# burlachenkok/flpytorch

Hardware: AMD Instinct MI355X
Metric: gradient-codec encode+reduce GB/s (device-resident), [N,D] fp32; % HBM peak (higher is better)
Workload: dtype f32; 1 GPU; C3 topk:1% N=1024/GPU D=10000000; codec=topk:1%, clients_per_gpu=1024, clients_total=1024, D=10000000, K=100000, rows_alloc=contiguous, parallelism=client-shard dp1

## Files before the change

flpytorch_amd/csrc/select.hip:

```cpp
#include <stdlib.h>

#include <atomic>
#include <map>
#include <mutex>
#include <vector>

#include "chunks.hpp"
#include "randk_tree.hpp"

namespace flc {

constexpr uint32_t ALL = 0xFFFFFFFFu;
constexpr uint32_t F_OVERFLOW = 1u, F_SHORT = 2u, F_TIES = 4u, F_EXACT = 8u;
constexpr uint32_t F_RESIDENT = 16u;
constexpr uint32_t F_REPAIR = 32u;
constexpr int SMAX = 16384;
constexpr int HBINS = 2048;
constexpr uint32_t TIECAP = HBINS;
constexpr int CS_SH = 64;
constexpr int64_t CS_FEW = 16;
constexpr int CS_ST = 8;
constexpr int CS_LCAP = 2048;
constexpr int RS_U = 16;
#ifndef FLC_RS_NG
#define FLC_RS_NG 4
#endif
constexpr int RS_NG = FLC_RS_NG;
constexpr int RS_NG_MAX = 16;
static_assert(RS_NG >= 1 && RS_NG <= RS_NG_MAX, "FLC_RS_NG: 1..16 groups");
constexpr int RS_GLOB = 0, RS_GEN = 32, RS_GAVE = 64, RS_CCNT = 96, RS_CDONE = 112, RS_GRP = 128;
constexpr int RS_XGRP = RS_GRP + 32 * RS_NG_MAX;
constexpr int RS_ABV = RS_XGRP + 32 * RS_NG_MAX;
constexpr int RS_CAP = 2048;
constexpr int RS_SS = 8192;
#ifndef FLC_RS_SR
#define FLC_RS_SR 1
#endif
constexpr int RS_SR = FLC_RS_SR;
#ifndef FLC_RS_STPOL
#define FLC_RS_STPOL 2
#endif
#ifndef FLC_RS_GACQ
#define FLC_RS_GACQ 1
#endif
#ifndef FLC_RS_POLLAB
#define FLC_RS_POLLAB 1
#endif
#ifndef FLC_RS_DONE
#define FLC_RS_DONE 1
#endif
#ifndef FLC_RS_RANKFIRST
#define FLC_RS_RANKFIRST 0
#endif
#ifndef FLC_RS_PROBE_NOCOUNT
#define FLC_RS_PROBE_NOCOUNT 0
#endif
#ifndef FLC_RS_G0REL
#define FLC_RS_G0REL 1
#endif
#ifndef FLC_RS_FENCE
#define FLC_RS_FENCE 0
#endif
#ifndef FLC_RS_SPEC
#define FLC_RS_SPEC 1
#endif
constexpr int RS_HREP = RS_ABV + 32 * RS_NG_MAX;
constexpr int RS_HSPEC = RS_HREP + 3 * RS_NG * HBINS;
constexpr int RS_CLIST = RS_HSPEC + 3 * RS_NG * HBINS;
constexpr int RS_TCNT = RS_CLIST + 2 * RS_CAP;
constexpr int RS_GMAX = 1024;
constexpr int RS_CS = 4;
constexpr int RS_CNUM = RS_TCNT + 2 * RS_GMAX;
constexpr int RS_CREG = RS_CNUM + RS_GMAX;
#ifdef FLC_RS_PRINT
constexpr int RS_PROBE = RS_CREG + 2 * RS_CS * RS_GMAX;
constexpr int RS_CTL = RS_PROBE + 4096;
#else
constexpr int RS_CTL = RS_CREG + 2 * RS_CS * RS_GMAX;
#endif
#ifndef FLC_RS_SPECST
#define FLC_RS_SPECST 0
#endif
#ifndef FLC_CS_LIST
#define FLC_CS_LIST 1
#endif
#ifndef FLC_CS_TWO_MAXD
#define FLC_CS_TWO_MAXD (int64_t(64) << 20)
#endif

struct SelWs {
    uint2* tab;
    uint32_t* ent_idx;
    float* ent_val;
    uint32_t* rowcnt;
    uint32_t* flags;
    uint32_t* thr;
    uint32_t* prefix;
    uint32_t* krem;
    uint32_t* tieprefix;
    uint32_t* tiecut;
    uint32_t* hist;
    uint32_t* worklist;
    uint32_t* nwork;
    uint32_t* cursor;
    uint32_t* cstate;
    uint64_t* clist;
    uint32_t* carrive;
    uint32_t* shcnt;
    uint32_t* zm;
    float* part;
    int64_t cap;
    uint32_t tie_hi;
};

__device__ __host__ inline uint32_t tie_pref(uint32_t ix, uint32_t hi) { return hi ? ix : ~ix; }
__device__ __host__ inline uint32_t tie_all(uint32_t hi) { return hi ? 0u : 0xFFFFFFFFu; }


__device__ inline void lds_bar() {
    asm volatile("s_waitcnt lgkmcnt(0)" ::: "memory");
    __builtin_amdgcn_s_barrier();
    asm volatile("" ::: "memory");
}
template <bool RAW>
__device__ inline void blk_bar() {
    if (RAW) lds_bar();
    else __syncthreads();
}
template <bool RAW = false>
__device__ inline void hist_find_at(const uint32_t* h, uint32_t k, uint32_t& bin, uint32_t& above,
                                    uint32_t* scratch , int t, bool own) {
    uint32_t local[8];
    uint32_t s = 0;
#pragma unroll
    for (int q = 0; q < 8; ++q) { local[q] = own ? h[HBINS - 1 - (t * 8 + q)] : 0u; s += local[q]; }
    if (t == 0) { scratch[256] = 0; scratch[257] = 0; }
    const int lane = t & 63, w = t >> 6;
    uint32_t inc = s;
#pragma unroll
    for (int off = 1; off < 64; off <<= 1) {
        const uint32_t v = __shfl_up(inc, off, 64);
        inc += lane >= off ? v : 0u;
    }
    if (own && lane == 63) scratch[w] = inc;
    blk_bar<RAW>();
    uint32_t before = 0;
    if (own)
        for (int q = 0; q < w; ++q) before += scratch[q];
    uint32_t incl = own ? before + inc : 0u, excl = incl - s;
    if (own && excl < k && incl >= k) {
        uint32_t run = excl;
#pragma unroll
        for (int q = 0; q < 8; ++q) {
            if (run + local[q] >= k) {
                scratch[256] = (uint32_t)(HBINS - 1 - (t * 8 + q));
                scratch[257] = run;
                break;
            }
            run += local[q];
        }
    }
    blk_bar<RAW>();
    bin = scratch[256];
    above = scratch[257];
    blk_bar<RAW>();
}
template <int NB>
__device__ inline void hist_find_n(const uint32_t* h, uint32_t k, uint32_t& bin, uint32_t& above, bool& found,
                                   uint32_t* scratch ) {
    constexpr int PER = NB / 256;
    static_assert(NB % 256 == 0, "256 threads scan NB / 256 bins each");
    const int t = (int)threadIdx.x;
    const bool own = t < 256;
    uint32_t local[PER];
    uint32_t s = 0;
#pragma unroll
    for (int q = 0; q < PER; ++q) { local[q] = own ? h[NB - 1 - (t * PER + q)] : 0u; s += local[q]; }
    if (t == 0) { scratch[256] = 0; scratch[257] = 0; scratch[258] = 0; }
    const int lane = t & 63, w = t >> 6;
    uint32_t inc = s;
#pragma unroll
    for (int off = 1; off < 64; off <<= 1) {
        const uint32_t v = __shfl_up(inc, off, 64);
        inc += lane >= off ? v : 0u;
    }
    if (own && lane == 63) scratch[w] = inc;
    __syncthreads();
    uint32_t before = 0;
    if (own)
        for (int q = 0; q < w; ++q) before += scratch[q];
    const uint32_t incl = own ? before + inc : 0u, excl = incl - s;
    if (own && excl < k && incl >= k) {
        uint32_t run = excl;
#pragma unroll
        for (int q = 0; q < PER; ++q) {
            if (run + local[q] >= k) {
                scratch[256] = (uint32_t)(NB - 1 - (t * PER + q));
                scratch[257] = run;
                scratch[258] = 1;
                break;
            }
            run += local[q];
        }
    }
    __syncthreads();
    bin = scratch[256];
    above = scratch[257];
    found = scratch[258] != 0u;
    __syncthreads();
}
template <bool RAW = false>
__device__ inline void hist_find(const uint32_t* h, uint32_t k, uint32_t& bin, uint32_t& above,
                                 uint32_t* scratch ) {
    hist_find_at<RAW>(h, k, bin, above, scratch, (int)threadIdx.x, threadIdx.x < 256);
}
__device__ inline void hist_find2(const uint32_t* ha, uint32_t ka, uint32_t& bina, uint32_t& abovea, uint32_t* sa,
                                  const uint32_t* hb, uint32_t kb, uint32_t& binb, uint32_t& aboveb, uint32_t* sb) {
    const bool second = threadIdx.x >= 256;
    uint32_t bin, above;
    hist_find_at(second ? hb : ha, second ? kb : ka, bin, above, second ? sb : sa, (int)(threadIdx.x & 255u),
                 threadIdx.x < 512);
    bina = sa[256]; abovea = sa[257];
    binb = sb[256]; aboveb = sb[257];
    __syncthreads();
}

__device__ inline uint32_t pass_shift(int p) { return p == 0 ? 20u : (p == 1 ? 9u : 0u); }
__device__ inline uint32_t pass_bits(int p) { return p == 2 ? 9u : 11u; }
__device__ inline bool key_in_prefix(uint32_t key, int p, uint32_t prefix) {
    if (p == 0) return true;
    uint32_t sh = pass_shift(p) + pass_bits(p);
    return (key >> sh) == prefix;
}
__device__ inline uint32_t key_bin(uint32_t key, int p) {
    return (key >> pass_shift(p)) & ((1u << pass_bits(p)) - 1u);
}

template <int NT, bool DUAL>
__global__ __launch_bounds__(NT) void k_topk_sample(RowSrc rows, int64_t n, int64_t d, int64_t K, SelWs ws, int few,
                                                    int64_t r_off) {
    __shared__ uint32_t keys[SMAX];
    __shared__ uint32_t h[HBINS], h2[DUAL ? HBINS : 1];
    __shared__ uint32_t scratch[260], scratch2[DUAL ? 260 : 1];
    const int64_t row = r_off + blockIdx.x;
    if (row >= n) return;
    const float* r = rows.row(row);
    int S;
    if (d <= SMAX) {
        S = (int)d;
        for (int i = threadIdx.x; i < S; i += NT) keys[i] = mag_key(r[i]);
    } else {
        const int P = SMAX / 256;
        S = SMAX;
        constexpr int GR = NT / 256, PU = 32 / GR;
        const int e = threadIdx.x & 255, g0 = threadIdx.x >> 8;
        for (int p0 = 0; p0 < P; p0 += 32) {
            float x[PU];
#pragma unroll
            for (int u = 0; u < PU; ++u) x[u] = r[((int64_t)(p0 + u * GR + g0) * (d - 256)) / (P - 1) + e];
#pragma unroll
            for (int u = 0; u < PU; ++u) keys[(p0 + u * GR + g0) * 256 + e] = mag_key(x[u]);
        }
    }
    const int NP = S == d ? 3 : 2;
    uint32_t rank;
    if (S == d) {
        rank = (uint32_t)K;
    } else {
        double ks = (double)K * (double)S / (double)d;
        double rr = ks + 4.0 * sqrt(ks) + 8.0;
        rank = (uint32_t)min((double)S, ceil(rr));
    }
    static_assert(!DUAL || NT >= 512, "hist_find2 takes 512 threads");
    auto rank_key = [&](uint32_t r) {
        uint32_t prefix = 0, krem = r;
        for (int p = 0; p < NP; ++p) {
            for (int i = threadIdx.x; i < HBINS; i += NT) h[i] = 0;
            __syncthreads();
            for (int i = threadIdx.x; i < S; i += NT) {
                uint32_t k = keys[i];
                if (key_in_prefix(k, p, prefix)) atomicAdd(&h[key_bin(k, p)], 1u);
            }
            __syncthreads();
            uint32_t bin, above;
            hist_find(h, krem, bin, above, scratch);
            prefix = (prefix << pass_bits(p)) | bin;
            krem -= above;
            __syncthreads();
        }
        return NP == 3 ? prefix : prefix << 9;
    };
    auto rank_keys = [&](uint32_t ra, uint32_t rb, uint32_t& ka, uint32_t& kb) {
        if constexpr (!DUAL) {
            ka = rank_key(ra);
            kb = rb == ra ? ka : rank_key(rb);
            return;
        }
        uint32_t pa = 0, pb = 0, ma = ra, mb = rb;
        for (int p = 0; p < NP; ++p) {
            const bool same = pa == pb;
            for (int i = threadIdx.x; i < HBINS; i += NT) { h[i] = 0; h2[i] = 0; }
            __syncthreads();
            for (int i = threadIdx.x; i < S; i += NT) {
                const uint32_t k = keys[i];
                if (key_in_prefix(k, p, pa)) atomicAdd(&h[key_bin(k, p)], 1u);
                if (!same && key_in_prefix(k, p, pb)) atomicAdd(&h2[key_bin(k, p)], 1u);
            }
            __syncthreads();
            uint32_t ba, aa, bb, ab;
            hist_find2(h, ma, ba, aa, scratch, same ? h : h2, mb, bb, ab, scratch2);
            pa = (pa << pass_bits(p)) | ba;
            ma -= aa;
            pb = (pb << pass_bits(p)) | bb;
            mb -= ab;
        }
        ka = NP == 3 ? pa : pa << 9;
        kb = NP == 3 ? pb : pb << 9;
    };
    uint32_t tkey, kest;
    rank_keys(rank, S == d ? rank : (uint32_t)max(1.0, min((double)S, (double)K * (double)S / (double)d)), tkey, kest);
    if (threadIdx.x == 0) {
        ws.thr[row] = (rank >= (uint32_t)S && S != d) ? 0u : tkey;
        ws.prefix[row] = kest;
        ws.flags[row] = 0;
        ws.rowcnt[(row) * RCS] = 0;
        if (few) { ws.cstate[row * CS_ST + 3] = 0; ws.cstate[row * CS_ST + 5] = 0; ws.carrive[row * RCS] = 0; }
    }
    if (few && threadIdx.x < CS_SH) ws.shcnt[(row * CS_SH + threadIdx.x) * RCS] = 0;
    if (few)
        for (int i = threadIdx.x; i < HBINS; i += NT) ws.hist[row * HBINS + i] = 0;
}

#ifndef FLC_CS_NT
#define FLC_CS_NT 1
#endif
__device__ inline float4 cs_ld(const float4* p) {
#if FLC_CS_NT
    typedef float v4f __attribute__((ext_vector_type(4)));
    const v4f v = __builtin_nontemporal_load(reinterpret_cast<const v4f*>(p));
    return make_float4(v.x, v.y, v.z, v.w);
#else
    return *p;
#endif
}
template <int NT>
__device__ void cand_select_row(int64_t row, int64_t K, SelWs ws, uint32_t* h, uint32_t* scratch) {
    {
        if (ws.flags[row]) return;
        const uint32_t cnt = ws.rowcnt[(row) * RCS];
        if (cnt < (uint32_t)K) {
            if (threadIdx.x == 0) ws.flags[row] |= F_SHORT;
            return;
        }
        const uint32_t T = ws.thr[row];
        const uint32_t span = ws.prefix[row] - T;
        int s = 0;
        while (s < 21 && (((uint64_t)span * 4u) >> s) >= (uint64_t)HBINS) ++s;
        const float* vals = ws.ent_val + row * ws.cap;
        const float4* v4 = reinterpret_cast<const float4*>(vals);
        const uint32_t n4 = cnt >> 2;
        uint32_t prefix = 0, krem = (uint32_t)K, last = 0;
        bool first = true, fail = false;
        int sh = s;
        while (true) {
            const int s1 = first ? sh : max(0, sh - 11);
            const uint32_t mask = first ? 0xFFFFFFFFu : ((1u << (sh - s1)) - 1u);
            for (int i = threadIdx.x; i < HBINS; i += NT) h[i] = 0;
            __syncthreads();
            auto add = [&](float x) {
                const uint32_t dk = mag_key(x) - T;
                if (first) atomicAdd(&h[min(dk >> s1, (uint32_t)(HBINS - 1))], 1u);
                else if ((dk >> sh) == prefix) atomicAdd(&h[(dk >> s1) & mask], 1u);
            };
            uint32_t i = threadIdx.x;
            for (; i + 7 * NT < n4; i += 8 * NT) {
                float4 q[8];
#pragma unroll
                for (int u = 0; u < 8; ++u) q[u] = cs_ld(v4 + i + u * NT);
#pragma unroll
                for (int u = 0; u < 8; ++u) { add(q[u].x); add(q[u].y); add(q[u].z); add(q[u].w); }
            }
            for (; i < n4; i += NT) {
                const float4 q = v4[i];
                add(q.x); add(q.y); add(q.z); add(q.w);
            }
            for (uint32_t i = n4 * 4 + threadIdx.x; i < cnt; i += NT) add(vals[i]);
            __syncthreads();
            uint32_t bin, above;
            hist_find(h, krem, bin, above, scratch);
            last = h[bin];
            if (first && bin == HBINS - 1) { fail = true; break; }
            prefix = first ? bin : ((prefix << (sh - s1)) | bin);
            krem -= above;
            sh = s1;
            first = false;
            __syncthreads();
            if (sh == 0) break;
        }
        __syncthreads();
        const uint32_t thr = T + prefix;
        bool ties = !fail && last > krem;
        if (ties && last > TIECAP) { fail = true; ties = false; }
        if (ties) {
            uint32_t* tix = h;
            if (threadIdx.x == 0) scratch[0] = 0;
            __syncthreads();
            const uint32_t* idxs = ws.ent_idx + row * ws.cap;
            for (uint32_t i = threadIdx.x; i < n4; i += NT) {
                const float4 q = v4[i];
                const float qv[4] = {q.x, q.y, q.z, q.w};
#pragma unroll
                for (int u = 0; u < 4; ++u)
                    if (mag_key(qv[u]) == thr) tix[atomicAdd(&scratch[0], 1u)] = idxs[i * 4 + u];
            }
            for (uint32_t i = n4 * 4 + threadIdx.x; i < cnt; i += NT) {
                if (mag_key(vals[i]) == thr) tix[atomicAdd(&scratch[0], 1u)] = idxs[i];
            }
            __syncthreads();
            const uint32_t m = scratch[0];
            for (uint32_t a = threadIdx.x; a < m; a += NT) {
                const uint32_t ia = tix[a];
                uint32_t rank = 0;
                for (uint32_t b = 0; b < m; ++b) rank += tie_pref(tix[b], ws.tie_hi) > tie_pref(ia, ws.tie_hi) ? 1u : 0u;
                if (rank == krem - 1) ws.tiecut[row] = ia;
            }
        }
        if (threadIdx.x == 0) {
            if (fail) {
                ws.flags[row] |= F_SHORT;
            } else {
                ws.thr[row] = thr;
                ws.krem[row] = krem;
                if (ties) ws.flags[row] |= F_TIES;
            }
        }
        __syncthreads();
    }
}

template <int NT>
__global__ __launch_bounds__(NT) void k_cand_select(int64_t r0, int64_t rn, int64_t K, SelWs ws) {
    __shared__ uint32_t h[HBINS];
    __shared__ uint32_t scratch[260];
    for (int64_t row = r0 + blockIdx.x; row < r0 + rn; row += gridDim.x) {
        cand_select_row<NT>(row, K, ws, h, scratch);
        __syncthreads();
    }
}

constexpr int CS_NT = 256;
__global__ __launch_bounds__(CS_NT) void k_cs_pass(int64_t K, SelWs ws, int final_pass) {
    __shared__ uint32_t h[HBINS];
    __shared__ uint32_t scratch[260];
    __shared__ uint32_t last_wg;
    __shared__ uint64_t lst[FLC_CS_LIST ? CS_LCAP : 1];
    const int64_t row = blockIdx.y;
    const uint32_t B = gridDim.x, b = blockIdx.x;
    uint32_t* cs = ws.cstate + row * CS_ST;
    const uint32_t stage = cs[3];
    if (stage >= 2u) return;
    const uint32_t* shc = ws.shcnt + row * CS_SH * RCS;
    uint32_t cnt = 0;
    for (int k = 0; k < CS_SH; ++k) cnt += shc[k * RCS];
    const uint32_t mycnt = shc[b * RCS];
    const bool first = stage == 0u;
    if (first && (ws.flags[row] != 0u || cnt < (uint32_t)K)) {
        if (b == 0 && threadIdx.x == 0) {
            if (ws.flags[row] == 0u) ws.flags[row] = F_SHORT;
            cs[3] = 2u;
        }
        return;
    }
    const uint32_t T = ws.thr[row];
    uint32_t sh, prefix, krem;
    if (first) {
        const uint32_t span = ws.prefix[row] - T;
        uint32_t s0 = 0;
        while (s0 < 21 && (((uint64_t)span * 4u) >> s0) >= (uint64_t)HBINS) ++s0;
        sh = s0; prefix = 0; krem = (uint32_t)K;
    } else {
        sh = cs[0]; prefix = cs[1]; krem = cs[2];
    }
    const uint32_t s1 = first ? sh : (sh > 11u ? sh - 11u : 0u);
    const uint32_t mask = first ? 0xFFFFFFFFu : ((1u << (sh - s1)) - 1u);
    const int64_t segcap = (ws.cap / CS_SH) & ~int64_t(3);
    if (FLC_CS_LIST && !first && cs[4] <= (uint32_t)CS_LCAP) {
        if (threadIdx.x == 0) scratch[0] = 0;
        __syncthreads();
        const float* sv = ws.ent_val + row * ws.cap + b * segcap;
        const uint32_t* si = ws.ent_idx + row * ws.cap + b * segcap;
        for (uint32_t e = threadIdx.x; e < mycnt; e += CS_NT) {
            const uint32_t key = mag_key(sv[e]);
            if (((key - T) >> sh) == prefix) {
                const uint32_t slot = atomicAdd(&scratch[0], 1u);
                if (slot < (uint32_t)CS_LCAP) lst[slot] = ((uint64_t)key << 32) | (uint64_t)tie_pref(si[e], ws.tie_hi);
            }
        }
        __syncthreads();
        const uint32_t nl = min(scratch[0], (uint32_t)CS_LCAP);
        if (threadIdx.x == 0) scratch[1] = nl ? atomicAdd(&cs[5], nl) : 0u;
        __syncthreads();
        uint64_t* gl = ws.clist + row * CS_LCAP;
        const uint32_t gb = scratch[1];
        for (uint32_t i = threadIdx.x; i < nl; i += CS_NT)
            if (gb + i < (uint32_t)CS_LCAP) gl[gb + i] = lst[i];
        asm volatile("s_waitcnt vmcnt(0)" ::: "memory");
        __syncthreads();
        if (threadIdx.x == 0) {
            __builtin_amdgcn_fence(__ATOMIC_RELEASE, "agent");
            last_wg = atomicAdd(&ws.carrive[row * RCS], 1u) == B - 1u ? 1u : 0u;
        }
        __syncthreads();
        if (!last_wg) return;
        __builtin_amdgcn_fence(__ATOMIC_ACQUIRE, "agent");
        const uint32_t m = __hip_atomic_load(&cs[5], __ATOMIC_RELAXED, __HIP_MEMORY_SCOPE_AGENT);
        const bool ok = m == cs[4] && m >= krem && krem >= 1u;
        const uint32_t mm = min(m, (uint32_t)CS_LCAP);
        for (uint32_t i = threadIdx.x; i < mm; i += CS_NT)
            lst[i] = __hip_atomic_load(&gl[i], __ATOMIC_RELAXED, __HIP_MEMORY_SCOPE_AGENT);
        if (threadIdx.x == 0) { scratch[0] = 0; scratch[1] = 0; scratch[2] = 0; scratch[3] = 0; }
        __syncthreads();
        if (ok)
            for (uint32_t i = threadIdx.x; i < mm; i += CS_NT) {
                const uint64_t me = lst[i];
                uint32_t rank = 0;
                for (uint32_t j = 0; j < mm; ++j) rank += lst[j] > me ? 1u : 0u;
                if (rank == krem - 1u) { scratch[0] = (uint32_t)(me >> 32); scratch[1] = tie_pref((uint32_t)me, ws.tie_hi); }
            }
        __syncthreads();
        const uint32_t kth = scratch[0];
        if (ok)
            for (uint32_t i = threadIdx.x; i < mm; i += CS_NT) {
                const uint32_t key = (uint32_t)(lst[i] >> 32);
                if (key > kth) atomicAdd(&scratch[2], 1u);
                else if (key == kth) atomicAdd(&scratch[3], 1u);
            }
        __syncthreads();
        if (threadIdx.x == 0) {
            atomicExch(&ws.carrive[row * RCS], 0u);
            if (!ok) {
                ws.flags[row] |= F_SHORT;
            } else {
                const uint32_t gt = scratch[2], eq = scratch[3];
                ws.thr[row] = kth;
                ws.krem[row] = krem - gt;
                if (gt + eq > krem) { ws.tiecut[row] = scratch[1]; ws.flags[row] |= F_TIES; }
            }
            cs[3] = 2u;
        }
        return;
    }
    for (int i = threadIdx.x; i < HBINS; i += CS_NT) h[i] = 0;
    __syncthreads();
    auto add = [&](float x) {
        const uint32_t dk = mag_key(x) - T;
        if (first) atomicAdd(&h[min(dk >> s1, (uint32_t)(HBINS - 1))], 1u);
        else if ((dk >> sh) == prefix) atomicAdd(&h[(dk >> s1) & mask], 1u);
    };
    const float* vals = ws.ent_val + row * ws.cap + b * segcap;
    const float4* v4 = reinterpret_cast<const float4*>(vals);
    const uint32_t n4 = mycnt >> 2, q1 = n4;
    uint32_t i = threadIdx.x;
    for (; i + 3 * CS_NT < q1; i += 4 * CS_NT) {
        float4 q[4];
#pragma unroll
        for (int u = 0; u < 4; ++u) q[u] = cs_ld(v4 + i + u * CS_NT);
#pragma unroll
        for (int u = 0; u < 4; ++u) { add(q[u].x); add(q[u].y); add(q[u].z); add(q[u].w); }
    }
    for (; i < q1; i += CS_NT) {
        const float4 q = cs_ld(v4 + i);
        add(q.x); add(q.y); add(q.z); add(q.w);
    }
    for (uint32_t t = n4 * 4 + threadIdx.x; t < mycnt; t += CS_NT) add(vals[t]);
    __syncthreads();
    uint32_t* gh = ws.hist + row * HBINS;
    for (int t = threadIdx.x; t < HBINS; t += CS_NT)
        if (h[t]) atomicAdd(gh + t, h[t]);
    asm volatile("s_waitcnt vmcnt(0)" ::: "memory");
    __syncthreads();
    if (threadIdx.x == 0) {
        __builtin_amdgcn_fence(__ATOMIC_RELEASE, "agent");
        asm volatile("s_waitcnt vmcnt(0)" ::: "memory");
        last_wg = atomicAdd(&ws.carrive[row * RCS], 1u) == B - 1u ? 1u : 0u;
    }
    __syncthreads();
    if (!last_wg) return;
    for (int t = threadIdx.x; t < HBINS; t += CS_NT) h[t] = atomicExch(gh + t, 0u);
    __syncthreads();
    uint32_t bin, above;
    hist_find(h, krem, bin, above, scratch);
    const uint32_t last = h[bin];
    const uint32_t np = first ? bin : ((prefix << (sh - s1)) | bin);
    const uint32_t nk = krem - above;
    const bool clamp = first && bin == HBINS - 1;
    bool ties = !clamp && s1 == 0u && last > nk, tie_fail = ties && last > TIECAP;
    if (ties && !tie_fail) {
        static_assert(CS_NT == 4 * CS_SH, "tie gather: 4 threads per shard");
        __syncthreads();
        uint32_t* tix = h;
        if (threadIdx.x == 0) scratch[0] = 0;
        __syncthreads();
        const uint32_t thr = T + np;
        const int k = threadIdx.x >> 2;
        const uint32_t sub = threadIdx.x & 3u, c = shc[k * RCS], c4 = c >> 2;
        const float* sv = ws.ent_val + row * ws.cap + k * segcap;
        const uint32_t* si = ws.ent_idx + row * ws.cap + k * segcap;
        const float4* s4 = reinterpret_cast<const float4*>(sv);
        auto test = [&](float x, uint32_t pos) {
            if (mag_key(x) == thr) {
                const uint32_t slot = atomicAdd(&scratch[0], 1u);
                if (slot < TIECAP) tix[slot] = si[pos];
            }
        };
        uint32_t j = sub;
        for (; j + 28u < c4; j += 32u) {
            float4 q[8];
#pragma unroll
            for (int u = 0; u < 8; ++u) q[u] = cs_ld(s4 + j + 4u * u);
#pragma unroll
            for (int u = 0; u < 8; ++u) {
                const uint32_t p4 = (j + 4u * u) * 4u;
                test(q[u].x, p4); test(q[u].y, p4 + 1u); test(q[u].z, p4 + 2u); test(q[u].w, p4 + 3u);
            }
        }
        for (; j < c4; j += 4u) {
            const float4 q = cs_ld(s4 + j);
            test(q.x, j * 4u); test(q.y, j * 4u + 1u); test(q.z, j * 4u + 2u); test(q.w, j * 4u + 3u);
        }
        for (uint32_t t = c4 * 4u + sub; t < c; t += 4u) test(sv[t], t);
        __syncthreads();
        const uint32_t m = scratch[0];
        if (m != last) tie_fail = true;
        else
            for (uint32_t a = threadIdx.x; a < m; a += CS_NT) {
                const uint32_t ia = tix[a];
                uint32_t rank = 0;
                for (uint32_t bb = 0; bb < m; ++bb) rank += tie_pref(tix[bb], ws.tie_hi) > tie_pref(ia, ws.tie_hi) ? 1u : 0u;
                if (rank == nk - 1u) ws.tiecut[row] = ia;
            }
    }
    if (threadIdx.x == 0) {
        atomicExch(&ws.carrive[row * RCS], 0u);
        if (clamp) {
            ws.flags[row] |= F_SHORT;
            cs[3] = 2u;
        } else if (s1 == 0u) {
            if (tie_fail) ws.flags[row] |= F_SHORT;
            else {
                ws.thr[row] = T + np;
                ws.krem[row] = nk;
                if (ties) ws.flags[row] |= F_TIES;
            }
            cs[3] = 2u;
        } else if (final_pass) {
            ws.flags[row] |= F_SHORT;
            cs[3] = 2u;
        } else {
            cs[0] = s1; cs[1] = np; cs[2] = nk; cs[3] = 1u; cs[4] = last;
        }
    }
}

template <bool EXACT, bool VEC>
__global__ __launch_bounds__(256) void k_topk_filter(RowSrc rows, int64_t n, int64_t d, SelWs ws) {
    const int64_t C = nchunks(d);
    const int64_t bpr = (C + 3) / 4;
    const int lane = threadIdx.x & 63, wv = threadIdx.x >> 6;
    const int64_t nrows = EXACT ? (int64_t)(*ws.nwork) : n;
    const int64_t items = nrows * bpr;
    for (int64_t it = blockIdx.x; it < items; it += gridDim.x) {
        const int64_t li = it / bpr;
        const int64_t row = EXACT ? (int64_t)ws.worklist[li] : li;
        const int64_t c = (it % bpr) * 4 + wv;
        if (!EXACT && ws.flags[row]) continue;
        if (c >= C) continue;
        const float* r = rows.row(row);
        const int64_t j0 = c * CHUNK;
        const uint32_t T = ws.thr[row];
        float v[16][4];
#pragma unroll
        for (int t = 0; t < 16; ++t) {
            const int64_t j = j0 + (int64_t)(t * 64 + lane) * 4;
            if (VEC && j + 3 < d) {
                float4 f = *reinterpret_cast<const float4*>(r + j);
                v[t][0] = f.x; v[t][1] = f.y; v[t][2] = f.z; v[t][3] = f.w;
            } else {
#pragma unroll
                for (int q = 0; q < 4; ++q) v[t][q] = (j + q < d) ? r[j + q] : 0.f;
            }
        }
        uint32_t tie_base = 0, tie_need = ALL, tie_from = 0;
        if (EXACT) {
            tie_base = ws.tieprefix[c * n + row];
            tie_need = ws.krem[row];
            if (ws.tie_hi) { const uint32_t tot = ws.tiecut[row]; tie_from = tot - tie_need; tie_need = tot; }
        }
        uint32_t cnt = 0;
        uint32_t tie_run = tie_base;
#pragma unroll
        for (int t = 0; t < 16; ++t) {
            const int64_t jb = j0 + (int64_t)(t * 64 + lane) * 4;
            bool gt[4], eq[4];
#pragma unroll
            for (int q = 0; q < 4; ++q) {
                const uint32_t k = mag_key(v[t][q]);
                const bool inb = (jb + q) < d;
                gt[q] = inb && (EXACT ? k > T : k >= T);
                eq[q] = inb && EXACT && k == T;
            }
            if (EXACT) {
                uint64_t m[4];
#pragma unroll
                for (int q = 0; q < 4; ++q) m[q] = __ballot(eq[q]);
                const uint64_t lt = (lane == 0) ? 0ull : (~0ull >> (64 - lane));
                uint32_t before = __popcll(m[0] & lt) + __popcll(m[1] & lt) + __popcll(m[2] & lt) + __popcll(m[3] & lt);
                uint32_t inlane = 0;
#pragma unroll
                for (int q = 0; q < 4; ++q) {
                    if (eq[q]) { const uint32_t tr = tie_run + before + inlane; gt[q] = tr >= tie_from && tr < tie_need; }
                    inlane += eq[q] ? 1u : 0u;
                }
                tie_run += __popcll(m[0]) + __popcll(m[1]) + __popcll(m[2]) + __popcll(m[3]);
            }
#pragma unroll
            for (int q = 0; q < 4; ++q) cnt += gt[q] ? 1u : 0u;
        }
        cnt = wave_sum(cnt);
        uint32_t base = 0;
        if (lane == 0) base = atomicAdd(&ws.rowcnt[(row) * RCS], cnt);
        base = __shfl(base, 0, WAVE);
        const bool fits = (int64_t)base + cnt <= ws.cap;
        if (lane == 0) {
            ws.tab[c * n + row] = make_uint2(base, fits ? cnt : 0u);
            if (!fits) atomicOr(&ws.flags[row], F_OVERFLOW);
        }
        if (!fits || cnt == 0) continue;
        uint32_t run = base;
        tie_run = tie_base;
        uint32_t* oi = ws.ent_idx + row * ws.cap;
        float* ov = ws.ent_val + row * ws.cap;
#pragma unroll
        for (int t = 0; t < 16; ++t) {
            const int64_t jb = j0 + (int64_t)(t * 64 + lane) * 4;
            bool gt[4], eq[4];
#pragma unroll
            for (int q = 0; q < 4; ++q) {
                const uint32_t k = mag_key(v[t][q]);
                const bool inb = (jb + q) < d;
                gt[q] = inb && (EXACT ? k > T : k >= T);
                eq[q] = inb && EXACT && k == T;
            }
            if (EXACT) {
                uint64_t m[4];
#pragma unroll
                for (int q = 0; q < 4; ++q) m[q] = __ballot(eq[q]);
                const uint64_t lt = (lane == 0) ? 0ull : (~0ull >> (64 - lane));
                uint32_t before = __popcll(m[0] & lt) + __popcll(m[1] & lt) + __popcll(m[2] & lt) + __popcll(m[3] & lt);
                uint32_t inlane = 0;
#pragma unroll
                for (int q = 0; q < 4; ++q) {
                    if (eq[q]) { const uint32_t tr = tie_run + before + inlane; gt[q] = tr >= tie_from && tr < tie_need; }
                    inlane += eq[q] ? 1u : 0u;
                }
                tie_run += __popcll(m[0]) + __popcll(m[1]) + __popcll(m[2]) + __popcll(m[3]);
            }
#pragma unroll
            for (int q = 0; q < 4; ++q) {
                const uint64_t m = __ballot(gt[q]);
                if (gt[q]) {
                    const uint32_t pos = run + (uint32_t)__popcll(m & ((lane == 0) ? 0ull : (~0ull >> (64 - lane))));
                    oi[pos] = (uint32_t)(jb + q);
                    ov[pos] = v[t][q];
                }
                run += (uint32_t)__popcll(m);
            }
        }
    }
}

constexpr int GCAP = 512;
static_assert(GCAP % 64 == 0, "copy-out runs in whole wave slots");


#ifndef FLC_TK_STPOL
#define FLC_TK_STPOL 0
#endif
#ifndef FLC_TK_COPY4
#define FLC_TK_COPY4 1
#endif
#ifndef FLC_TK_PROBE
#define FLC_TK_PROBE 0
#endif

template <int POL = FLC_TK_STPOL>
__device__ inline void tk_copy_out(const uint32_t* si, const uint32_t* sv, const SelWs& ws, int64_t n, int64_t row,
                                   uint32_t pos, uint32_t tot, bool fits, int lane, int64_t wslot) {
    int64_t at = row * ws.cap + pos;
    if (FLC_TK_PROBE == 4) at = (wslot % max((n * ws.cap) >> 10, (int64_t)1)) << 10;
    const uint32_t nrec = (fits && FLC_TK_PROBE != 2) ? tot * 4u : 0u;
    const auto di = __builtin_amdgcn_make_buffer_rsrc(ws.ent_idx + at, (short)0, (int)nrec, 0x00020000);
    const auto dv = __builtin_amdgcn_make_buffer_rsrc(ws.ent_val + at, (short)0, (int)nrec, 0x00020000);
    typedef unsigned int u4v __attribute__((ext_vector_type(4)));
    const uint32_t nq = min(tot, (uint32_t)GCAP) >> 2;
#pragma unroll
    for (int k = 0; k < GCAP / 256; ++k) {
        const uint32_t q = (uint32_t)(k * 64 + lane);
        const uint4 a = reinterpret_cast<const uint4*>(si)[q];
        const uint4 b = reinterpret_cast<const uint4*>(sv)[q];
        const uint32_t off = q < nq ? q * 16u : 0x7FFFFFF0u;
        __builtin_amdgcn_raw_buffer_store_b128(__builtin_bit_cast(u4v, a), di, off, 0, POL);
        __builtin_amdgcn_raw_buffer_store_b128(__builtin_bit_cast(u4v, b), dv, off, 0, POL);
    }
    const uint32_t e = nq * 4u + (uint32_t)(lane & 3);
    const uint32_t off = lane < 3 ? e * 4u : 0x7FFFFFF0u;
    __builtin_amdgcn_raw_buffer_store_b32(si[e], di, off, 0, POL);
    __builtin_amdgcn_raw_buffer_store_b32(sv[e], dv, off, 0, POL);
}

template <int RING, int FGS, int LONE = 0>
#ifndef FLC_TK_RING
#define FLC_TK_RING 16
#endif
#ifndef FLC_TK_WPE
#define FLC_TK_WPE 1
#endif
__global__ __launch_bounds__(256) __attribute__((amdgpu_waves_per_eu(FLC_TK_WPE))) void k_topk_filter_fast(RowSrc rows, int64_t n, int64_t r0, int64_t rn, int64_t rb, int64_t d, SelWs ws, int shards,
                                                                                                float* __restrict__ zout) {
    static_assert(16 % RING == 0, "ring must divide the 16 loads of a chunk");
    constexpr int SROW = GCAP + 64;
    static_assert((SROW * 4) % 256 == 0, "value block offset in 256-byte units");
    __shared__ __attribute__((aligned(16))) uint32_t st[2][4][2 * SROW];
    const int lane = threadIdx.x & 63;
    const int wv = __builtin_amdgcn_readfirstlane(threadIdx.x >> 6);
    const int64_t C = nchunks(d);
    const int64_t G = (C + FGS - 1) / FGS;
    const int64_t items = rn * G;
    const int64_t stride = (int64_t)gridDim.x * 4;
    int64_t it = (int64_t)blockIdx.x * 4 + wv;
    if (it >= items) return;
    float4 ring[RING];
    auto item_at = [&](int64_t t, int64_t& r, int64_t& cc) {
        const int64_t blk = t / (rb * G), rem = t - blk * rb * G;
        const int64_t bn = min(rb, rn - blk * rb);
        const int64_t g = rem / bn;
        r = r0 + blk * rb + (rem - g * bn);
        cc = g * FGS;
    };
    int64_t row, c;
    item_at(it, row, c);
    auto rs = chunk_rsrc(rows.row_s(row), c * CHUNK, d);
#pragma unroll
    for (int L = 0; L < RING - 1; ++L) {
        ring[L] = load_q(rs, lane, L);
        __builtin_amdgcn_sched_barrier(0);
    }
    const int64_t segcap = shards > 1 ? (ws.cap / shards) & ~int64_t(3) : ws.cap;
    bool pv = false;
    int64_t prow = 0, pc0 = 0, pseg = 0;
    uint64_t pcc = 0;
    uint32_t ptot = 0, pres = 0;
    int par = 0;
    auto finish = [&](int pb) {
        uint32_t base = 0;
        bool fits = ptot <= GCAP;
        if (fits && ptot) {
            base = __shfl(pres, 0, WAVE);
            fits = (int64_t)base + ptot <= segcap;
            base += (uint32_t)(pseg * segcap);
        }
        if (lane < FGS && pc0 + lane < C) {
            uint32_t off = 0, cc = 0;
#pragma unroll
            for (int u = 0; u < FGS; ++u) {
                const uint32_t cu = (uint32_t)(pcc >> (16 * u)) & 0xFFFFu;
                off += u < lane ? cu : 0u;
                cc = u == lane ? cu : cc;
            }
            ws.tab[(pc0 + lane) * n + prow] = make_uint2(base + off, fits ? cc : 0u);
        }
        if (!fits && lane == 0) atomicOr(&ws.flags[prow], F_OVERFLOW);
#if FLC_TK_COPY4
        tk_copy_out(st[pb][wv], st[pb][wv] + SROW, ws, n, prow, base, ptot, fits, lane, (int64_t)blockIdx.x * 4 + wv);
#else
        if (fits && FLC_TK_PROBE != 2) {
            const uint32_t* si = st[pb][wv];
            const float* sv = reinterpret_cast<const float*>(st[pb][wv] + SROW);
            uint32_t* oi = ws.ent_idx + prow * ws.cap + base;
            float* ov = ws.ent_val + prow * ws.cap + base;
#pragma unroll
            for (int k = 0; k < GCAP / 64; ++k) {
                const uint32_t e = (uint32_t)(k * 64 + lane);
                if (e < ptot) { oi[e] = si[e]; ov[e] = sv[e]; }
            }
        }
#endif
    };
    while (it < items) {
        const uint32_t T = max(sload(ws.thr + row), 1u);
        const int64_t nit = it + stride;
        const uint32_t sla = __builtin_amdgcn_readfirstlane((uint32_t)(size_t)(__attribute__((address_space(3))) uint32_t*)st[par][wv]);
        uint32_t cnt = 0;
        uint64_t ccp = 0;
        const int64_t cg0 = c;
        int64_t nrow = row, nc = c;
#pragma unroll
        for (int sub = 0; sub < FGS; ++sub, ++c) {
            const int64_t j0 = c * CHUNK;
            __amdgpu_buffer_rsrc_t rsn;
            if (sub + 1 < FGS) {
                rsn = chunk_rsrc(rows.row_s(row), j0 + CHUNK, d);
            } else if (nit < items) {
                item_at(nit, nrow, nc);
                rsn = chunk_rsrc(rows.row_s(nrow), nc * CHUNK, d);
            } else {
                rsn = __builtin_amdgcn_make_buffer_rsrc(const_cast<float*>(rows.row_s(row)), (short)0, 0, 0x00020000);
            }
            const uint32_t cnt0 = cnt;
            __amdgpu_buffer_rsrc_t ro;
            if constexpr (LONE != 0) ro = chunk_rsrc(zout, j0, d);
            uint32_t lb = (uint32_t)j0 + (uint32_t)lane * 4u;
            asm volatile("" : "+v"(lb));
#pragma unroll
            for (int L = 0; L < 16; ++L) {
                const int P = L + RING - 1;
                ring[P % RING] = P < 16 ? load_q(rs, lane, P) : load_q(rsn, lane, P - 16);
                const float4 x = ring[L % RING];
                if constexpr (LONE != 0) {
                    typedef unsigned int u4v __attribute__((ext_vector_type(4)));
                    const u4v z = {0u, 0u, 0u, 0u};
                    __builtin_amdgcn_raw_buffer_store_b128(z, ro, lane * 16, L * 1024, 0);
                }
                const uint32_t jl = lb + (uint32_t)(L * 256);
                const float vq[4] = {x.x, x.y, x.z, x.w};
#pragma unroll
                for (int q = 0; q < 4; ++q) {
                    if (FLC_TK_PROBE == 3) { cnt += __float_as_uint(vq[q]) == 0x7F800001u ? 1u : 0u; continue; }
                    const bool f = mag_key(vq[q]) >= T;
                    const uint64_t m = __ballot(f);
                    if (FLC_TK_PROBE != 1 && f) {
                        const uint32_t pre = __builtin_amdgcn_mbcnt_hi((uint32_t)(m >> 32), __builtin_amdgcn_mbcnt_lo((uint32_t)m, 0u));
                        uint32_t sb = sla + min(cnt, (uint32_t)GCAP) * 4u;
                        asm volatile("" : "+s"(sb));
                        asm volatile("ds_write2st64_b32 %0, %1, %2 offset1:%3" ::"v"(sb + pre * 4u),
                                     "v"(jl + q), "v"(__float_as_uint(vq[q])), "i"(SROW * 4 / 256) : "memory");
                    }
                    cnt += (uint32_t)__popcll(m);
                }
            }
            ccp |= (uint64_t)min(cnt - cnt0, 0xFFFFu) << (16 * (c - cg0));
            rs = rsn;
        }
        if (pv) finish(par ^ 1);
        uint32_t res = 0;
        const int64_t shard = shards > 1 ? (cg0 / FGS) % shards : 0;
        if (cnt && cnt <= GCAP && lane == 0)
            res = atomicAdd(shards > 1 ? &ws.shcnt[(row * shards + shard) * RCS] : &ws.rowcnt[(row) * RCS], cnt);
        pv = true; prow = row; pc0 = cg0; pcc = ccp; ptot = cnt; pres = res; pseg = shard;
        __builtin_amdgcn_fence(__ATOMIC_SEQ_CST, "wavefront");
        par ^= 1;
        it = nit;
        row = nrow;
        c = nc;
    }
    __builtin_amdgcn_fence(__ATOMIC_SEQ_CST, "wavefront");
    finish(par ^ 1);
}

#ifndef FLC_TK_WG
#define FLC_TK_WG 1
#endif
#ifndef FLC_TK_WG_NL
#define FLC_TK_WG_NL 4
#endif
#ifndef FLC_TK_WG_RING
#define FLC_TK_WG_RING FLC_TK_RING
#endif
#ifndef FLC_TK_WG_STPOL
#define FLC_TK_WG_STPOL 17
#endif
#ifndef FLC_TK_WG_WPE
#define FLC_TK_WG_WPE 4
#endif
__device__ inline uint32_t lds_addr(const void* p) {
    return (uint32_t)(size_t)(const __attribute__((address_space(3))) void*)p;
}
__device__ inline uint32_t lds_peek(uint32_t addr) {
    uint32_t v;
    asm volatile("ds_read_b32 %0, %1\n\ts_waitcnt lgkmcnt(0)" : "=&v"(v) : "v"(addr) : "memory");
    return __builtin_amdgcn_readfirstlane(v);
}
template <int RING, int NL>
__global__ __launch_bounds__((NL + 1) * 64) __attribute__((amdgpu_waves_per_eu(FLC_TK_WG_WPE))) void k_topk_filter_fast_wg(RowSrc rows, int64_t n, int64_t r0, int64_t rn, int64_t rb, int64_t d,
                                                                        SelWs ws) {
    static_assert(16 % RING == 0, "ring must divide the 16 loads of a chunk");
    constexpr int FGS = 4;
    constexpr int SROW = GCAP + 64;
    __shared__ __attribute__((aligned(16))) uint32_t st[2][NL][2 * SROW];
    __shared__ __attribute__((aligned(16))) uint32_t hs[2][NL][4];
    __shared__ uint32_t fr[2];
    const int lane = threadIdx.x & 63;
    const int wv = __builtin_amdgcn_readfirstlane(threadIdx.x >> 6);
    if (threadIdx.x < 2 * NL * 4) (&hs[0][0][0])[threadIdx.x] = 0;
    if (threadIdx.x < 2) fr[threadIdx.x] = 0;
    __syncthreads();
    const int64_t C = nchunks(d);
    const int64_t G = (C + FGS * NL - 1) / (FGS * NL);
    const int64_t items = rn * G;
    const int64_t stride = gridDim.x;
    int64_t it = blockIdx.x;
    if (it >= items) return;
    auto item_at = [&](int64_t t, int64_t& r, int64_t& cc) {
        const int64_t blk = t / (rb * G), rem = t - blk * rb * G;
        const int64_t bn = min(rb, rn - blk * rb);
        const int64_t g = rem / bn;
        r = r0 + blk * rb + (rem - g * bn);
        cc = g * (FGS * NL);
    };
    if (wv == NL) {
        for (uint32_t k = 0; it < items; it += stride, ++k) {
            const int b = k & 1;
            int64_t row, c0;
            item_at(it, row, c0);
            const uint32_t fa = lds_addr(&hs[b][min(lane, NL - 1)][3]);
            for (;;) {
                uint32_t f;
                asm volatile("ds_read_b32 %0, %1\n\ts_waitcnt lgkmcnt(0)" : "=&v"(f) : "v"(fa) : "memory");
                if (__ballot(f != k + 1) == 0) break;
                __builtin_amdgcn_s_sleep(4);
            }
            uint32_t pre[NL], tot[NL], sum = 0;
            uint64_t cc[NL];
            bool allfit = true;
#pragma unroll
            for (int w = 0; w < NL; ++w) {
                const uint4 h = *reinterpret_cast<const uint4*>(hs[b][w]);
                cc[w] = (uint64_t)h.x | ((uint64_t)h.y << 32);
                tot[w] = h.z;
                pre[w] = sum;
                sum += tot[w] <= GCAP ? tot[w] : 0u;
                allfit = allfit && tot[w] <= GCAP;
            }
            uint32_t base = 0;
            bool fits = true;
            if (sum) {
                uint32_t res = 0;
                if (lane == 0) res = atomicAdd(&ws.rowcnt[row * RCS], sum);
                base = __shfl(res, 0, WAVE);
                fits = (int64_t)base + sum <= ws.cap;
            }
            if (lane < FGS * NL && c0 + lane < C) {
                uint32_t off = 0, cu = 0;
                bool gf = false;
#pragma unroll
                for (int w = 0; w < NL; ++w)
                    if ((lane >> 2) == w) {
                        off = pre[w];
                        gf = tot[w] <= GCAP;
#pragma unroll
                        for (int u = 0; u < FGS; ++u) {
                            const uint32_t x = (uint32_t)(cc[w] >> (16 * u)) & 0xFFFFu;
                            off += u < (lane & 3) ? x : 0u;
                            cu = u == (lane & 3) ? x : cu;
                        }
                    }
                ws.tab[(c0 + lane) * n + row] = make_uint2(base + off, fits && gf ? cu : 0u);
            }
            if (!(fits && allfit) && lane == 0) atomicOr(&ws.flags[row], F_OVERFLOW);
#pragma unroll
            for (int w = 0; w < NL; ++w)
                tk_copy_out<FLC_TK_WG_STPOL>(st[b][w], st[b][w] + SROW, ws, n, row, base + pre[w], tot[w], fits && tot[w] <= GCAP, lane,
                            (int64_t)blockIdx.x * NL + w);
            asm volatile("s_waitcnt lgkmcnt(0)\n\tds_write_b32 %0, %1" ::"v"(lds_addr(&fr[b])), "v"(k + 1) : "memory");
        }
        return;
    }
    float4 ring[RING];
    int64_t row, c;
    item_at(it, row, c);
    c += wv * FGS;
    auto rs = chunk_rsrc(rows.row_s(row), c * CHUNK, d);
#pragma unroll
    for (int L = 0; L < RING - 1; ++L) {
        ring[L] = load_q(rs, lane, L);
        __builtin_amdgcn_sched_barrier(0);
    }
    for (uint32_t k = 0; it < items; ++k) {
        const int b = k & 1;
        if (k >= 2) {
            const uint32_t fa = lds_addr(&fr[b]);
            while (lds_peek(fa) != k - 1) __builtin_amdgcn_s_sleep(2);
        }
        const uint32_t T = max(sload(ws.thr + row), 1u);
        const int64_t nit = it + stride;
        const uint32_t sla = __builtin_amdgcn_readfirstlane(lds_addr(st[b][wv]));
        uint32_t cnt = 0;
        uint64_t ccp = 0;
        const int64_t cg0 = c;
        int64_t nrow = row, nc = c;
#pragma unroll
        for (int sub = 0; sub < FGS; ++sub, ++c) {
            const int64_t j0 = c * CHUNK;
            __amdgpu_buffer_rsrc_t rsn;
            if (sub + 1 < FGS) {
                rsn = chunk_rsrc(rows.row_s(row), j0 + CHUNK, d);
            } else if (nit < items) {
                item_at(nit, nrow, nc);
                nc += wv * FGS;
                rsn = chunk_rsrc(rows.row_s(nrow), nc * CHUNK, d);
            } else {
                rsn = __builtin_amdgcn_make_buffer_rsrc(const_cast<float*>(rows.row_s(row)), (short)0, 0, 0x00020000);
            }
            const uint32_t cnt0 = cnt;
            uint32_t lb = (uint32_t)j0 + (uint32_t)lane * 4u;
            asm volatile("" : "+v"(lb));
#pragma unroll
            for (int L = 0; L < 16; ++L) {
                const int P = L + RING - 1;
                ring[P % RING] = P < 16 ? load_q(rs, lane, P) : load_q(rsn, lane, P - 16);
                const float4 x = ring[L % RING];
                const uint32_t jl = lb + (uint32_t)(L * 256);
                const float vq[4] = {x.x, x.y, x.z, x.w};
#pragma unroll
                for (int q = 0; q < 4; ++q) {
                    const bool f = mag_key(vq[q]) >= T;
                    const uint64_t m = __ballot(f);
                    if (f) {
                        const uint32_t pre = __builtin_amdgcn_mbcnt_hi((uint32_t)(m >> 32), __builtin_amdgcn_mbcnt_lo((uint32_t)m, 0u));
                        uint32_t sb = sla + min(cnt, (uint32_t)GCAP) * 4u;
                        asm volatile("" : "+s"(sb));
                        asm volatile("ds_write2st64_b32 %0, %1, %2 offset1:%3" ::"v"(sb + pre * 4u),
                                     "v"(jl + q), "v"(__float_as_uint(vq[q])), "i"(SROW * 4 / 256) : "memory");
                    }
                    cnt += (uint32_t)__popcll(m);
                }
            }
            ccp |= (uint64_t)min(cnt - cnt0, 0xFFFFu) << (16 * (c - cg0));
            rs = rsn;
        }
        if (lane == 0)
            asm volatile("ds_write_b64 %0, %1\n\tds_write_b32 %0, %2 offset:8\n\tds_write_b32 %0, %3 offset:12"
                         ::"v"(lds_addr(hs[b][wv])), "v"(ccp), "v"(cnt), "v"(k + 1) : "memory");
        it = nit;
        row = nrow;
        c = nc;
    }
}

template <bool FULLROW>
__global__ __launch_bounds__(256) void k_radix_hist(RowSrc rows, int64_t n, int64_t d, int p, SelWs ws) {
    __shared__ uint32_t h[HBINS];
    constexpr int64_t BLK = 65536;
    const int64_t nrows = FULLROW ? (int64_t)(*ws.nwork) : n;
    const int64_t maxlen = FULLROW ? d : ws.cap;
    const int64_t bpr = (maxlen + BLK - 1) / BLK;
    const int64_t items = nrows * bpr;
    for (int64_t it = blockIdx.x; it < items; it += gridDim.x) {
        const int64_t li = it / bpr;
        const int64_t row = FULLROW ? (int64_t)ws.worklist[li] : li;
        if (!FULLROW && ws.flags[row]) continue;
        const int64_t len = FULLROW ? d : (int64_t)ws.rowcnt[(row) * RCS];
        const int64_t b0 = (it % bpr) * BLK;
        if (b0 >= len) continue;
        const int64_t b1 = min(len, b0 + BLK);
        for (int i = threadIdx.x; i < HBINS; i += 256) h[i] = 0;
        __syncthreads();
        const uint32_t prefix = ws.prefix[row];
        const float* src = FULLROW ? rows.row(row) : (ws.ent_val + row * ws.cap);
        for (int64_t j = b0 + threadIdx.x; j < b1; j += 256) {
            const uint32_t k = mag_key(src[j]);
            if (key_in_prefix(k, p, prefix)) atomicAdd(&h[key_bin(k, p)], 1u);
        }
        __syncthreads();
        uint32_t* gh = ws.hist + row * HBINS;
        for (int i = threadIdx.x; i < HBINS; i += 256)
            if (h[i]) atomicAdd(&gh[i], h[i]);
        __syncthreads();
    }
}

template <bool FULLROW>
__global__ __launch_bounds__(256) void k_radix_select(int64_t n, int p, int64_t K, SelWs ws) {
    __shared__ uint32_t scratch[260];
    const int64_t nrows = FULLROW ? (int64_t)(*ws.nwork) : n;
    for (int64_t li = blockIdx.x; li < nrows; li += gridDim.x) {
        const int64_t row = FULLROW ? (int64_t)ws.worklist[li] : li;
        if (!FULLROW && ws.flags[row]) continue;
        uint32_t* gh = ws.hist + row * HBINS;
        if (!FULLROW && p == 0 && ws.rowcnt[(row) * RCS] < (uint32_t)K) {
            for (int i = threadIdx.x; i < HBINS; i += 256) gh[i] = 0;
            if (threadIdx.x == 0) ws.flags[row] |= F_SHORT;
            continue;
        }
        const uint32_t k = (p == 0) ? (uint32_t)K : ws.krem[row];
        uint32_t bin, above;
        hist_find(gh, k, bin, above, scratch);
        const uint32_t ties_here = gh[bin];
        __syncthreads();
        for (int i = threadIdx.x; i < HBINS; i += 256) gh[i] = 0;
        if (threadIdx.x == 0) {
            const uint32_t pre = (p == 0) ? 0u : ws.prefix[row];
            ws.prefix[row] = (pre << pass_bits(p)) | bin;
            ws.krem[row] = k - above;
            if (p == 2) {
                ws.thr[row] = ws.prefix[row];
                if (FULLROW) ws.tiecut[row] = ties_here;
                if (ties_here > k - above) ws.flags[row] |= (FULLROW ? F_TIES | F_EXACT : F_TIES);
                else if (FULLROW) ws.flags[row] |= F_EXACT;
            }
        }
        __syncthreads();
    }
}

__global__ void k_build_worklist(int64_t n, int64_t K, int64_t d, SelWs ws, int force_all) {
    __shared__ uint32_t cnt;
    if (threadIdx.x == 0) cnt = 0;
    __syncthreads();
    for (int64_t row = threadIdx.x; row < n; row += blockDim.x) {
        uint32_t f = ws.flags[row];
        if (force_all || (f & (F_OVERFLOW | F_SHORT))) {
            uint32_t pos = atomicAdd(&cnt, 1u);
            ws.worklist[pos] = (uint32_t)row;
            ws.flags[row] = F_EXACT;
            ws.rowcnt[(row) * RCS] = 0;
            ws.prefix[row] = 0;
        }
    }
    __syncthreads();
    if (threadIdx.x == 0) *ws.nwork = cnt;
}

constexpr int EX_NT = 1024;
constexpr int EX_U = 8;

template <int NT = EX_NT>
__device__ inline uint32_t ex_scan(uint32_t v, uint32_t* wsum , uint32_t& total) {
    const int lane = threadIdx.x & 63, wv = threadIdx.x >> 6;
    uint32_t inc = v;
#pragma unroll
    for (int o = 1; o < 64; o <<= 1) {
        const uint32_t t = __shfl_up(inc, o, 64);
        inc += lane >= o ? t : 0u;
    }
    if (lane == 63) wsum[wv] = inc;
    __syncthreads();
    uint32_t before = 0, tot = 0;
#pragma unroll
    for (int k = 0; k < NT / 64; ++k) {
        const uint32_t x = wsum[k];
        before += k < wv ? x : 0u;
        tot += x;
    }
    __syncthreads();
    total = tot;
    return before + inc - v;
}

template <bool VEC, int NT = EX_NT>
__device__ void exact_row(RowSrc rows, int64_t n, int64_t row, int64_t d, int64_t K, SelWs ws, uint32_t* h,
                          uint32_t* scratch, uint32_t* wsum) {
    const int t = threadIdx.x;
    const int64_t C = nchunks(d);
    {
        const float* r = rows.row(row);
        uint32_t prefix = 0, krem = (uint32_t)K, ties_tot = 0;
        for (int p = 0; p < 3; ++p) {
            for (int i = t; i < HBINS; i += NT) h[i] = 0;
            __syncthreads();
            auto add = [&](uint32_t k) { if (key_in_prefix(k, p, prefix)) atomicAdd(&h[key_bin(k, p)], 1u); };
            int64_t j = 0;
            if (VEC) {
                const float4* r4 = reinterpret_cast<const float4*>(r);
                const int64_t g4 = d / 4;
                int64_t g = t;
                for (; g + (EX_U - 1) * NT < g4; g += EX_U * NT) {
                    float4 q[EX_U];
#pragma unroll
                    for (int u = 0; u < EX_U; ++u) q[u] = ld_row4(r4 + g + u * NT);
#pragma unroll
                    for (int u = 0; u < EX_U; ++u) {
                        add(mag_key(q[u].x)); add(mag_key(q[u].y)); add(mag_key(q[u].z)); add(mag_key(q[u].w));
                    }
                }
                for (; g < g4; g += NT) {
                    const float4 q = ld_row4(r4 + g);
                    add(mag_key(q.x)); add(mag_key(q.y)); add(mag_key(q.z)); add(mag_key(q.w));
                }
                j = g4 * 4;
            }
            for (int64_t jj = j + t; jj < d; jj += NT) add(mag_key(r[jj]));
            __syncthreads();
            uint32_t bin, above;
            hist_find(h, krem, bin, above, scratch);
            prefix = (prefix << pass_bits(p)) | bin;
            krem -= above;
            if (p == 2) ties_tot = h[bin];
            __syncthreads();
        }
        const uint32_t thr = prefix;
        const uint32_t tie_from = ws.tie_hi ? ties_tot - krem : 0u, tie_to = ws.tie_hi ? ties_tot : krem;
        uint32_t* oi = ws.ent_idx + row * ws.cap;
        float* ov = ws.ent_val + row * ws.cap;
        static_assert(CHUNK % (NT * 4) == 0, "exact_row: NT * 4 must divide CHUNK");
        constexpr int SUBS = CHUNK / (NT * 4);
        uint32_t base = 0, tie_run = 0, cbase = 0;
        for (int64_t cs = 0; cs < C * SUBS; ++cs) {
            const int64_t c = cs / SUBS;
            const int sb = (int)(cs % SUBS);
            if (sb == 0) cbase = base;
            const int64_t j0 = c * CHUNK + (int64_t)sb * (NT * 4) + (int64_t)t * 4;
            float v[4];
            if (VEC && j0 + 3 < d) {
                const float4 q = ld_row4(reinterpret_cast<const float4*>(r + j0));
                v[0] = q.x; v[1] = q.y; v[2] = q.z; v[3] = q.w;
            } else {
#pragma unroll
                for (int q = 0; q < 4; ++q) v[q] = (j0 + q < d) ? r[j0 + q] : 0.f;
            }
            bool gt[4], eq[4];
            uint32_t ne = 0;
#pragma unroll
            for (int q = 0; q < 4; ++q) {
                const bool in = j0 + q < d;
                const uint32_t k = mag_key(v[q]);
                gt[q] = in && k > thr;
                eq[q] = in && k == thr;
                ne += eq[q] ? 1u : 0u;
            }
            uint32_t etot;
            uint32_t erank = tie_run + ex_scan<NT>(ne, wsum, etot);
            uint32_t na = 0;
            bool adm[4];
#pragma unroll
            for (int q = 0; q < 4; ++q) {
                adm[q] = gt[q] || (eq[q] && erank >= tie_from && erank < tie_to);
                erank += eq[q] ? 1u : 0u;
                na += adm[q] ? 1u : 0u;
            }
            uint32_t atot;
            uint32_t pos = base + ex_scan<NT>(na, wsum, atot);
#pragma unroll
            for (int q = 0; q < 4; ++q)
                if (adm[q]) { oi[pos] = (uint32_t)(j0 + q); ov[pos] = v[q]; ++pos; }
            base += atot;
            tie_run += etot;
            if (sb == SUBS - 1 && t == 0) ws.tab[c * n + row] = make_uint2(cbase, base - cbase);
        }
        if (t == 0) {
            ws.thr[row] = thr;
            ws.krem[row] = krem;
            ws.rowcnt[row * RCS] = base;
            ws.flags[row] = F_EXACT | (ws.flags[row] & (F_OVERFLOW | F_SHORT));
        }
        __syncthreads();
    }
}

template <bool VEC>
__global__ __launch_bounds__(EX_NT) void k_topk_exact_rows(RowSrc rows, int64_t n, int64_t r0, int64_t rn, int64_t d, int64_t K, SelWs ws) {
    __shared__ uint32_t h[HBINS];
    __shared__ uint32_t scratch[260];
    __shared__ uint32_t wsum[EX_NT / 64];
    for (int64_t row = r0 + blockIdx.x; row < r0 + rn; row += gridDim.x) {
        if (!(ws.flags[row] & (F_OVERFLOW | F_SHORT))) continue;
        exact_row<VEC>(rows, n, row, d, K, ws, h, scratch, wsum);
    }
}

template <int NT, bool VEC>
__global__ __launch_bounds__(NT) void k_cand_select_x(RowSrc rows, int64_t n, int64_t r0, int64_t rn, int64_t d, int64_t K,
                                                      SelWs ws) {
    __shared__ uint32_t h[HBINS];
    __shared__ uint32_t scratch[260];
    __shared__ uint32_t wsum[NT / 64];
    __shared__ uint32_t failed;
    for (int64_t row = r0 + blockIdx.x; row < r0 + rn; row += gridDim.x) {
        cand_select_row<NT>(row, K, ws, h, scratch);
        __syncthreads();
        if (threadIdx.x == 0) failed = __atomic_load_n(&ws.flags[row], __ATOMIC_RELAXED) & (F_OVERFLOW | F_SHORT);
        __syncthreads();
        if (failed) exact_row<VEC, NT>(rows, n, row, d, K, ws, h, scratch, wsum);
        __syncthreads();
    }
}

__global__ __launch_bounds__(256) void k_tie_count(RowSrc rows, int64_t n, int64_t d, SelWs ws) {
    const int64_t C = nchunks(d);
    const int lane = threadIdx.x & 63, wv = threadIdx.x >> 6;
    const int64_t nrows = *ws.nwork;
    const int64_t bpr = (C + 3) / 4;
    for (int64_t it = blockIdx.x; it < nrows * bpr; it += gridDim.x) {
        const int64_t row = ws.worklist[it / bpr];
        const int64_t c = (it % bpr) * 4 + wv;
        if (c >= C) continue;
        uint32_t cnt = 0;
        if (ws.flags[row] & F_TIES) {
            const uint32_t T = ws.thr[row];
            const float* r = rows.row(row);
            const int64_t j1 = min(d, (c + 1) * (int64_t)CHUNK);
            for (int64_t j = c * CHUNK + lane; j < j1; j += 64) cnt += (mag_key(r[j]) == T) ? 1u : 0u;
            cnt = wave_sum(cnt);
        }
        if (lane == 0) ws.tieprefix[c * n + row] = cnt;
    }
}

__global__ __launch_bounds__(256) void k_tie_scan(int64_t n, int64_t d, SelWs ws) {
    constexpr bool EXACT = true;
    __shared__ uint32_t part[256];
    const int64_t C = nchunks(d);
    const int64_t nrows = EXACT ? (int64_t)(*ws.nwork) : n;
    const int t = threadIdx.x;
    const int64_t per = (C + 255) / 256;
    for (int64_t li = blockIdx.x; li < nrows; li += gridDim.x) {
        const int64_t row = EXACT ? (int64_t)ws.worklist[li] : li;
        if (!EXACT && (ws.flags[row] & (F_TIES | F_EXACT)) != F_TIES) continue;
        const int64_t c0 = t * per, c1 = min(C, c0 + per);
        uint32_t sum = 0;
        for (int64_t c = c0; c < c1; ++c) sum += ws.tieprefix[c * n + row];
        part[t] = sum;
        __syncthreads();
        for (int off = 1; off < 256; off <<= 1) {
            const uint32_t v = (t >= off) ? part[t - off] : 0u;
            __syncthreads();
            part[t] += v;
            __syncthreads();
        }
        uint32_t run = part[t] - sum;
        for (int64_t c = c0; c < c1; ++c) {
            const uint32_t v = ws.tieprefix[c * n + row];
            ws.tieprefix[c * n + row] = run;
            run += v;
        }
        __syncthreads();
    }
}

constexpr int RK_T = 1024;
constexpr int RK_SB = 256;
constexpr int RK_TILE = 8192;

__host__ __device__ inline int64_t rk_spc(int64_t C) { return (C + RK_SB - 1) / RK_SB; }

template <class Emit>
__device__ inline void randk_walk(const flc_pattern& pat, int64_t row, int64_t K, int64_t ldi, int tid, Emit emit) {
    for (int64_t t = tid; t < K; t += RK_T) emit(t, (uint32_t)pat.d_randk_idx[row * ldi + t]);
}

template <bool FINAL>
__global__ __launch_bounds__(RK_T) void k_randk_coarse(RowSrc rows, int64_t n, int64_t d, int64_t K, flc_pattern pat,
                                                       int64_t ldi, float scale, SelWs ws) {
    __shared__ uint32_t cnt[RK_SB], tcnt[RK_SB], toff[RK_SB], gbase[RK_SB];
    __shared__ uint32_t tile[RK_TILE];
    const int64_t row = blockIdx.x;
    const int64_t C = nchunks(d), spc = rk_spc(C);
    const int tid = threadIdx.x;
    if (tid < RK_SB) cnt[tid] = 0;
    __syncthreads();
    uint32_t* jbuf = reinterpret_cast<uint32_t*>(ws.ent_val + row * ws.cap);
    randk_walk(pat, row, K, ldi, tid, [&](int64_t t, uint32_t j) {
        jbuf[t] = j;
        atomicAdd(&cnt[(j >> CHUNK_SHIFT) / spc], 1u);
    });
    __syncthreads();
    if (tid < 64) {
        uint32_t v[RK_SB / 64], loc = 0;
#pragma unroll
        for (int q = 0; q < RK_SB / 64; ++q) { v[q] = cnt[tid * (RK_SB / 64) + q]; loc += v[q]; }
        uint32_t incl = loc;
#pragma unroll
        for (int o = 1; o < 64; o <<= 1) {
            const uint32_t u = __shfl_up(incl, o, WAVE);
            if (tid >= o) incl += u;
        }
        uint32_t run = incl - loc;
#pragma unroll
        for (int q = 0; q < RK_SB / 64; ++q) {
            const int b = tid * (RK_SB / 64) + q;
            if (FINAL) {
                if (b < C) ws.tab[(int64_t)b * n + row] = make_uint2(run, v[q]);
            } else {
                ws.cursor[row * RK_SB + b] = run;
            }
            cnt[b] = run;
            run += v[q];
        }
    }
    __syncthreads();
    uint32_t* oi = ws.ent_idx + row * ws.cap;
    constexpr int Q = RK_TILE / RK_T;
    for (int64_t t0 = 0; t0 < K; t0 += RK_TILE) {
        const int m = (int)min<int64_t>(RK_TILE, K - t0);
        if (tid < RK_SB) tcnt[tid] = 0;
        __syncthreads();
        uint32_t jj[Q], rnk[Q];
#pragma unroll
        for (int q = 0; q < Q; ++q) {
            const int k = tid + q * RK_T;
            if (k < m) {
                jj[q] = jbuf[t0 + k];
                rnk[q] = atomicAdd(&tcnt[(jj[q] >> CHUNK_SHIFT) / spc], 1u);
            }
        }
        __syncthreads();
        if (tid < 64) {
            uint32_t v[RK_SB / 64], loc = 0;
#pragma unroll
            for (int q = 0; q < RK_SB / 64; ++q) { v[q] = tcnt[tid * (RK_SB / 64) + q]; loc += v[q]; }
            uint32_t incl = loc;
#pragma unroll
            for (int o = 1; o < 64; o <<= 1) {
                const uint32_t u = __shfl_up(incl, o, WAVE);
                if (tid >= o) incl += u;
            }
            uint32_t run = incl - loc;
#pragma unroll
            for (int q = 0; q < RK_SB / 64; ++q) {
                const int b = tid * (RK_SB / 64) + q;
                toff[b] = run;
                gbase[b] = cnt[b];
                cnt[b] += v[q];
                run += v[q];
            }
        }
        __syncthreads();
#pragma unroll
        for (int q = 0; q < Q; ++q) {
            const int k = tid + q * RK_T;
            if (k < m) tile[toff[(jj[q] >> CHUNK_SHIFT) / spc] + rnk[q]] = jj[q];
        }
        __syncthreads();
#pragma unroll
        for (int q = 0; q < Q; ++q) {
            const int k = tid + q * RK_T;
            if (k < m) {
                const uint32_t j = tile[k];
                const uint32_t b = (j >> CHUNK_SHIFT) / spc;
                oi[gbase[b] + (uint32_t)k - toff[b]] = j;
            }
        }
        __syncthreads();
    }
    if (tid == 0) {
        ws.thr[row] = 0;
        ws.flags[row] = F_EXACT;
        ws.rowcnt[row * RCS] = (uint32_t)K;
    }
    if (FINAL) {
        __syncthreads();
        const float* r = rows.row(row);
        float* val = ws.ent_val + row * ws.cap;
        for (int64_t t = tid; t < K; t += RK_T) val[t] = scale * r[oi[t]];
    }
}

constexpr int RK_FT = 8192, RK_FTHR = 512;
__global__ __launch_bounds__(RK_FTHR) void k_randk_fine(RowSrc rows, int64_t n, int64_t d, int64_t K, float scale,
                                                        SelWs ws) {
    extern __shared__ uint32_t fc[];
    __shared__ uint32_t wsum[RK_FTHR / 64];
    __shared__ uint32_t tile[RK_FT];
    const int64_t row = blockIdx.y, b = blockIdx.x;
    const int64_t C = nchunks(d), spc = rk_spc(C);
    const int64_t cb0 = b * spc, cb1 = min(C, cb0 + spc);
    const int tid = threadIdx.x;
    if (cb0 >= C) return;
    const uint32_t s0 = ws.cursor[row * RK_SB + b];
    const uint32_t s1 = (b + 1 < RK_SB) ? ws.cursor[row * RK_SB + b + 1] : (uint32_t)K;
    const int64_t nc = cb1 - cb0;
    const bool in_lds = s1 - s0 <= (uint32_t)RK_FT;
    for (int64_t c = tid; c < nc; c += RK_FTHR) fc[c] = 0;
    __syncthreads();
    uint32_t* idx = ws.ent_idx + row * ws.cap;
    uint32_t* tmp = reinterpret_cast<uint32_t*>(ws.ent_val + row * ws.cap);
    constexpr int Q = RK_FT / RK_FTHR;
    uint32_t jj[Q], rnk[Q];
    if (in_lds) {
#pragma unroll
        for (int q = 0; q < Q; ++q) {
            const uint32_t t = s0 + tid + q * RK_FTHR;
            if (t < s1) {
                jj[q] = idx[t];
                rnk[q] = atomicAdd(&fc[(jj[q] >> CHUNK_SHIFT) - cb0], 1u);
            }
        }
    } else {
        for (uint32_t t = s0 + tid; t < s1; t += RK_FTHR) {
            const uint32_t j = idx[t];
            tmp[t] = j;
            atomicAdd(&fc[(j >> CHUNK_SHIFT) - cb0], 1u);
        }
    }
    __syncthreads();
    const int64_t per = (nc + RK_FTHR - 1) / RK_FTHR;
    const int64_t q0 = min<int64_t>(nc, tid * per), q1 = min<int64_t>(nc, q0 + per);
    uint32_t loc = 0;
    for (int64_t c = q0; c < q1; ++c) loc += fc[c];
    uint32_t incl = loc;
#pragma unroll
    for (int o = 1; o < 64; o <<= 1) {
        const uint32_t u = __shfl_up(incl, o, WAVE);
        if ((tid & 63) >= o) incl += u;
    }
    if ((tid & 63) == 63) wsum[tid >> 6] = incl;
    __syncthreads();
    uint32_t run = incl - loc;
    for (int w = 0; w < (tid >> 6); ++w) run += wsum[w];
    for (int64_t c = q0; c < q1; ++c) {
        const uint32_t v = fc[c];
        ws.tab[(cb0 + c) * n + row] = make_uint2(s0 + run, v);
        fc[c] = run;
        run += v;
    }
    __syncthreads();
    const float* r = rows.row(row);
    float* val = ws.ent_val + row * ws.cap;
    if (in_lds) {
#pragma unroll
        for (int q = 0; q < Q; ++q) {
            const uint32_t t = s0 + tid + q * RK_FTHR;
            if (t < s1) tile[fc[(jj[q] >> CHUNK_SHIFT) - cb0] + rnk[q]] = jj[q];
        }
        __syncthreads();
        for (uint32_t k = tid; k < s1 - s0; k += RK_FTHR) {
            const uint32_t j = tile[k];
            idx[s0 + k] = j;
            val[s0 + k] = scale * r[j];
        }
        return;
    }
    for (uint32_t t = s0 + tid; t < s1; t += RK_FTHR) {
        const uint32_t j = tmp[t];
        idx[s0 + atomicAdd(&fc[(j >> CHUNK_SHIFT) - cb0], 1u)] = j;
    }
    __syncthreads();
    for (uint32_t t = s0 + tid; t < s1; t += RK_FTHR) val[t] = scale * r[idx[t]];
}

#ifndef FLC_CA_PROBE
#define FLC_CA_PROBE 0
#endif
#ifndef FLC_CA_AP1
#define FLC_CA_AP1 4
#endif
#ifndef FLC_CA_WPB1
#define FLC_CA_WPB1 0
#endif
#ifndef FLC_CA_AP
#define FLC_CA_AP 8
#endif
constexpr int AP = FLC_CA_AP;

struct RowMeta {
    uint2 te;
    uint32_t thr, cut, mode;
    float w;
};

__device__ inline RowMeta load_meta(const SelWs& ws, int64_t c, int64_t n, int64_t r, const float* w, int64_t rend = -1) {
    RowMeta m;
    m.te = make_uint2(0, 0);
    m.thr = 0; m.cut = 0u; m.mode = 0; m.w = 1.f;
    if (r < (rend < 0 ? n : rend)) {
        m.te = ws.tab[c * n + r];
        m.thr = ws.thr[r];
        const uint32_t f = ws.flags[r];
        m.mode = (f & F_EXACT) ? 2u : ((f & F_TIES) ? 1u : 0u);
        if (m.mode == 1u) m.cut = tie_pref(ws.tiecut[r], ws.tie_hi);
        if (m.mode == 2u) m.thr = 0u;
        if (w) m.w = w[r];
    }
    return m;
}


template <int TS>
__device__ void resolve_neg_zero(float* tl, uint32_t* rm, const SelWs& ws, int64_t c, int64_t n, uint32_t cbase,
                                 int64_t len, const float* w, int lane) {
    constexpr int NW = TS / 32;
    constexpr int WL = (NW + 63) / 64;
    bool any = false;
    for (int k = 0; k < TS / 64; ++k) {
        const int64_t i = (int64_t)k * 64 + lane;
        const uint64_t b = __ballot(i < len && __float_as_uint(tl[i]) == 0x80000000u);
        if (lane == 0) { rm[2 * k] = (uint32_t)b; rm[2 * k + 1] = (uint32_t)(b >> 32); }
        any |= b != 0ull;
    }
    if (!any) return;
    uint32_t z0[WL], zc[WL];
#pragma unroll
    for (int j = 0; j < WL; ++j) {
        const int k = lane + 64 * j;
        z0[j] = k < NW ? rm[k] : 0u;
        zc[j] = z0[j];
    }
    for (int64_t r = 0; r < n; ++r) {
        if (w && (__float_as_uint(w[r]) >> 31)) continue;
#pragma unroll
        for (int j = 0; j < WL; ++j) if (lane + 64 * j < NW) rm[lane + 64 * j] = 0u;
        const RowMeta m = load_meta(ws, c, n, r, w);
        const uint32_t mode = m.mode, T = m.thr, cut = m.cut;
        for (uint32_t e = (uint32_t)lane; e < m.te.y; e += 64) {
            const uint32_t ix = ws.ent_idx[r * ws.cap + m.te.x + e];
            const uint32_t key = mag_key(ws.ent_val[r * ws.cap + m.te.x + e]);
            const uint32_t loc = ix - cbase;
            if (loc < (uint32_t)TS && (mode == 2u || key > T || (key == T && tie_pref(ix, ws.tie_hi) >= cut)))
                atomicOr(&rm[loc >> 5], 1u << (loc & 31));
        }
        bool left = false;
#pragma unroll
        for (int j = 0; j < WL; ++j) {
            if (lane + 64 * j < NW) zc[j] &= rm[lane + 64 * j];
            left |= zc[j] != 0u;
        }
        if (__ballot(left) == 0ull) break;
    }
#pragma unroll
    for (int j = 0; j < WL; ++j) {
        uint32_t dead = z0[j] & ~zc[j];
        while (dead) {
            const int b = __builtin_ctz(dead);
            dead &= dead - 1u;
            tl[(lane + 64 * j) * 32 + b] = 0.f;
        }
    }
}

template <int TS>
__device__ void resolve_neg_zero_g(float* tl, uint32_t* rm, const SelWs& ws, int64_t c, int64_t n, uint32_t cbase,
                                   int64_t len, const float* w, int lane) {
    constexpr int NW = TS / 32;
    constexpr int WL = (NW + 63) / 64;
    uint32_t z0[WL], zc[WL];
#pragma unroll
    for (int j = 0; j < WL; ++j) z0[j] = 0u;
    bool any = false;
#pragma unroll 4
    for (int k = 0; k < TS / 64; ++k) {
        const int64_t i = (int64_t)k * 64 + lane;
        const uint64_t b = __ballot(i < len && __float_as_uint(tl[i]) == 0x80000000u);
        const int w0 = 2 * k, w1 = 2 * k + 1;
#pragma unroll
        for (int j = 0; j < WL; ++j) {
            if (lane == (w0 & 63) && (w0 >> 6) == j) z0[j] = (uint32_t)b;
            if (lane == (w1 & 63) && (w1 >> 6) == j) z0[j] = (uint32_t)(b >> 32);
        }
        any |= b != 0ull;
    }
    if (!any) return;
#pragma unroll
    for (int j = 0; j < WL; ++j) zc[j] = z0[j];
    for (int64_t r = 0; r < n; ++r) {
        if (w && (__float_as_uint(w[r]) >> 31)) continue;
#pragma unroll
        for (int j = 0; j < WL; ++j) if (lane + 64 * j < NW) rm[lane + 64 * j] = 0u;
        __threadfence_block();
        const RowMeta m = load_meta(ws, c, n, r, w);
        const uint32_t mode = m.mode, T = m.thr, cut = m.cut;
        for (uint32_t e = (uint32_t)lane; e < m.te.y; e += 64) {
            const uint32_t ix = ws.ent_idx[r * ws.cap + m.te.x + e];
            const uint32_t key = mag_key(ws.ent_val[r * ws.cap + m.te.x + e]);
            const uint32_t loc = ix - cbase;
            if (loc < (uint32_t)TS && (mode == 2u || key > T || (key == T && tie_pref(ix, ws.tie_hi) >= cut)))
                atomicOr(&rm[loc >> 5], 1u << (loc & 31));
        }
        __threadfence_block();
        bool left = false;
#pragma unroll
        for (int j = 0; j < WL; ++j) {
            if (lane + 64 * j < NW) zc[j] &= atomicOr(&rm[lane + 64 * j], 0u);
            left |= zc[j] != 0u;
        }
        if (__ballot(left) == 0ull) break;
    }
#pragma unroll
    for (int j = 0; j < WL; ++j) {
        uint32_t dead = z0[j] & ~zc[j];
        while (dead) {
            const int b = __builtin_ctz(dead);
            dead &= dead - 1u;
            tl[(lane + 64 * j) * 32 + b] = 0.f;
        }
    }
}

template <bool ASSIGN, int TS, bool W, int WPB, int AP = AP>
__device__ __forceinline__ void chunk_accum_body(int64_t n, int64_t d, SelWs ws, const float* __restrict__ w, float wt,
                                                 float* __restrict__ out, int64_t r0, int64_t rend, int first, int last,
                                                 float (*tile)[TS], uint32_t (*zmask)[WPB == 1 ? 1 : TS / 32]) {
    if (rend < 0) rend = n;
    constexpr int PARTS = CHUNK / TS;
    const int lane = threadIdx.x & 63;
    const int wv = WPB == 1 ? 0 : __builtin_amdgcn_readfirstlane(threadIdx.x >> 6);
    const int64_t C = nchunks(d);
    float* tl = tile[wv];
    const int64_t nb = (rend - r0 + 63) / 64;
    for (int64_t t = (int64_t)blockIdx.x * WPB + wv; t < C * PARTS; t += (int64_t)gridDim.x * WPB) {
        const int64_t c = t / PARTS;
        const uint32_t cbase = (uint32_t)(c * CHUNK + (t % PARTS) * TS);
        if (FLC_TILE_V4 && !ASSIGN && !first && (int64_t)cbase + TS <= d) {
            const float4* p4 = reinterpret_cast<const float4*>(ws.part + cbase);
#pragma unroll
            for (int k0 = 0; k0 < TS / 256; k0 += 8) {
                float4 v[8];
#pragma unroll
                for (int k = 0; k < 8; ++k) v[k] = k0 + k < TS / 256 ? p4[(k0 + k) * 64 + lane] : make_float4(0.f, 0.f, 0.f, 0.f);
#pragma unroll
                for (int k = 0; k < 8; ++k)
                    if (k0 + k < TS / 256) reinterpret_cast<float4*>(tl)[(k0 + k) * 64 + lane] = v[k];
            }
        } else {
            for (int i = lane; i < TS; i += 64)
                tl[i] = ASSIGN ? 0.f : (first || (int64_t)cbase + i >= d ? -0.f : ws.part[cbase + i]);
        }
        RowMeta cur = load_meta(ws, c, n, r0 + lane, w, rend), nxt;
        uint32_t ri[AP][2];
        float rv[AP][2];
        auto fetch = [&](const RowMeta& m, int q, int64_t row, int slot) {
            const uint32_t off = __builtin_amdgcn_readlane(m.te.x, q), cnt = __builtin_amdgcn_readlane(m.te.y, q);
            const auto di = list_rsrc(ws.ent_idx + row * ws.cap + off, cnt);
            const auto dv = list_rsrc(ws.ent_val + row * ws.cap + off, cnt);
#pragma unroll
            for (int h = 0; h < 2; ++h) {
                const uint32_t e = (uint32_t)lane + 64u * h;
                const uint32_t x = __builtin_amdgcn_raw_buffer_load_b32(di, lane * 4, h * 256, 0);
                ri[slot][h] = e < cnt ? x : 0xFFFFFFFFu;
                rv[slot][h] = __uint_as_float(__builtin_amdgcn_raw_buffer_load_b32(dv, lane * 4, h * 256, 0));
            }
        };
        const uint32_t txm = ws.tie_hi ? 0u : 0xFFFFFFFFu;
        auto fold = [&](uint32_t ix, float vv, uint32_t T, uint32_t cut, uint32_t mode, float wi) {
            (void)mode;
            const uint32_t loc = ix - cbase;
            const uint64_t a = ((uint64_t)mag_key(vv) << 32) | (uint64_t)(ix ^ txm);
            const uint64_t b = ((uint64_t)T << 32) | (uint64_t)cut;
            if (FLC_CA_PROBE == 1) {
                if (loc < (uint32_t)TS && a >= b && vv == 1.2345f) tl[0] = vv;
                return;
            }
            if (loc < (uint32_t)TS && a >= b) {
                if (ASSIGN) tl[loc] = vv;
                else tl[loc] = W ? tl[loc] + wi * vv : tl[loc] + vv;
            }
        };
#pragma unroll
        for (int q = 0; q < AP; ++q) fetch(cur, q, r0 + q, q);
        for (int64_t b = 0; b < nb; ++b) {
            const int64_t i0 = r0 + b * 64;
            nxt = load_meta(ws, c, n, i0 + 64 + lane, w, rend);
            if (__builtin_expect(__ballot(cur.te.y > 128u) == 0ull, 1)) {
#pragma unroll
                for (int q = 0; q < 64; ++q) {
                    const int slot = q % AP;
                    const uint32_t T = __builtin_amdgcn_readlane(cur.thr, q);
                    const uint32_t cut = __builtin_amdgcn_readlane(cur.cut, q);
                    const uint32_t mode = 0u;
                    const float wi = W ? __uint_as_float(__builtin_amdgcn_readlane(__float_as_uint(cur.w), q)) : 1.f;
                    fold(ri[slot][0], rv[slot][0], T, cut, mode, wi);
                    if (__builtin_amdgcn_readlane(cur.te.y, q) > 64u) fold(ri[slot][1], rv[slot][1], T, cut, mode, wi);
                    if (q + AP < 64) fetch(cur, q + AP, i0 + q + AP, slot);
                    else fetch(nxt, q + AP - 64, i0 + q + AP, slot);
                }
            } else {
                for (int q = 0; q < 64; ++q) {
                    const int slot = q % AP;
                    const uint32_t T = __shfl(cur.thr, q, WAVE), cut = __shfl(cur.cut, q, WAVE);
                    const uint32_t mode = __shfl(cur.mode, q, WAVE), cnt = __shfl(cur.te.y, q, WAVE);
                    const uint32_t off = __shfl(cur.te.x, q, WAVE);
                    const float wi = W ? __shfl(cur.w, q, WAVE) : 1.f;
                    uint32_t i_0 = 0, i_1 = 0;
                    float v_0 = 0.f, v_1 = 0.f;
#pragma unroll
                    for (int z = 0; z < AP; ++z)
                        if (z == slot) { i_0 = ri[z][0]; i_1 = ri[z][1]; v_0 = rv[z][0]; v_1 = rv[z][1]; }
                    fold(i_0, v_0, T, cut, mode, wi);
                    fold(i_1, v_1, T, cut, mode, wi);
                    const int64_t row = i0 + q;
                    for (uint32_t e = 128u + lane; e < cnt; e += 64)
                        fold(ws.ent_idx[row * ws.cap + off + e], ws.ent_val[row * ws.cap + off + e], T, cut, mode, wi);
                    const RowMeta& m = (q + AP < 64) ? cur : nxt;
                    const int qq = (q + AP) & 63;
                    const uint32_t offn = __shfl(m.te.x, qq, WAVE), cntn = __shfl(m.te.y, qq, WAVE);
                    const int64_t rown = i0 + q + AP;
                    uint32_t xi[2];
                    float xv[2];
#pragma unroll
                    for (int h = 0; h < 2; ++h) {
                        const uint32_t e = (uint32_t)lane + 64u * h;
                        xi[h] = e < cntn ? ws.ent_idx[rown * ws.cap + offn + e] : 0xFFFFFFFFu;
                        xv[h] = e < cntn ? ws.ent_val[rown * ws.cap + offn + e] : 0.f;
                    }
#pragma unroll
                    for (int z = 0; z < AP; ++z)
                        if (z == slot) { ri[z][0] = xi[0]; ri[z][1] = xi[1]; rv[z][0] = xv[0]; rv[z][1] = xv[1]; }
                }
            }
            cur = nxt;
        }
        const int64_t len = min((int64_t)TS, d - (int64_t)cbase);
        if (!last) {
            for (int64_t i = lane; i < len; i += 64) ws.part[cbase + i] = tl[i];
            continue;
        }
        if (!ASSIGN) {
            if (WPB == 1) resolve_neg_zero_g<TS>(tl, ws.zm + t * (TS / 32), ws, c, n, cbase, len, w, lane);
            else resolve_neg_zero<TS>(tl, zmask[wv], ws, c, n, cbase, len, w, lane);
        }
        for (int64_t i = lane; i < len; i += 64) out[cbase + i] = ASSIGN ? tl[i] : tl[i] / wt;
    }
}

template <bool ASSIGN, int TS = CHUNK, bool W = true>
__global__ __launch_bounds__(256) void k_chunk_accum(int64_t n, int64_t d, SelWs ws, const float* __restrict__ w, float wt,
                                                     float* __restrict__ out, int64_t r0 = 0, int64_t rend = -1,
                                                     int first = 1, int last = 1) {
    __shared__ __attribute__((aligned(16))) float tile[4][TS];
    __shared__ uint32_t zmask[4][TS / 32];
    chunk_accum_body<ASSIGN, TS, W, 4>(n, d, ws, w, wt, out, r0, rend, first, last, tile, zmask);
}

template <bool W>
__global__ __launch_bounds__(64) void k_chunk_accum1(
        int64_t n, int64_t d, SelWs ws, const float* __restrict__ w, float wt, float* __restrict__ out, int64_t r0,
        int64_t rend, int first, int last) {
    extern __shared__ __attribute__((aligned(16))) float dyn_tile[];
    chunk_accum_body<false, CHUNK, W, 1, FLC_CA_AP1>(n, d, ws, w, wt, out, r0, rend, first, last,
                                         reinterpret_cast<float (*)[CHUNK]>(dyn_tile), nullptr);
}

struct RkdWs {
    uint32_t* cnt;
    uint64_t* ckey;
};

constexpr int RKC_NT = 1024;
constexpr int64_t RKC_BINS = 32768;

__global__ __launch_bounds__(256) void k_randk_ckeys(int64_t n, uint64_t seed, int64_t client0, uint64_t* __restrict__ ckey) {
    const int64_t row = (int64_t)blockIdx.x * 256 + threadIdx.x;
    if (row < n) ckey[row] = client_key(seed, client0 + row);
}

__global__ __launch_bounds__(RKC_NT) void k_randk_counts(int64_t n, int64_t d, int64_t K, uint64_t seed, int64_t client0,
                                                         RkdWs ws) {
    __shared__ uint32_t bins[RKC_BINS / 2];
    const int64_t row = blockIdx.y;
    const int tid = threadIdx.x;
    const int64_t C = nchunks(d);
    const int64_t c0 = (int64_t)blockIdx.x * RKC_BINS, nc = min(C, c0 + RKC_BINS) - c0;
    const uint64_t ck = client_key(seed, client0 + row);
    for (int64_t i = tid; i < (nc + 1) / 2; i += RKC_NT) bins[i] = 0;
    __syncthreads();
    const rktree::RowPerm P(ck, (uint64_t)d);
    int64_t t = tid;
    bool live = t < K;
    uint64_t x = (uint64_t)t;
    while (__ballot(live) != 0ull) {
        const uint64_t v = P.once(x);
        if (live) {
            if (v < (uint64_t)d) {
                const int64_t c = (int64_t)(v >> CHUNK_SHIFT) - c0;
                if ((uint64_t)c < (uint64_t)nc) atomicAdd(&bins[c >> 1], 1u << (16 * (c & 1)));
                t += RKC_NT;
                live = t < K;
                x = (uint64_t)t;
            } else {
                x = v;
            }
        }
    }
    __syncthreads();
    if (blockIdx.x == 0 && tid == 0) ws.ckey[row] = ck;
    for (int64_t c = tid; c < nc; c += RKC_NT) ws.cnt[(c0 + c) * n + row] = (bins[c >> 1] >> (16 * (c & 1))) & 0xFFFFu;
}

__global__ __launch_bounds__(256) void k_randk_tab(int64_t n, int64_t d, int64_t K, const uint32_t* __restrict__ cnt,
                                                   SelWs ls) {
    __shared__ uint32_t part[256];
    const int64_t row = blockIdx.x;
    const int tid = threadIdx.x;
    const int64_t C = nchunks(d), per = (C + 255) / 256;
    const int64_t c0 = min(C, tid * per), c1 = min(C, c0 + per);
    uint32_t loc = 0;
    for (int64_t c = c0; c < c1; ++c) loc += cnt[c * n + row];
    part[tid] = loc;
    __syncthreads();
    for (int off = 1; off < 256; off <<= 1) {
        const uint32_t v = tid >= off ? part[tid - off] : 0u;
        __syncthreads();
        part[tid] += v;
        __syncthreads();
    }
    uint32_t run = part[tid] - loc;
    for (int64_t c = c0; c < c1; ++c) {
        const uint32_t m = cnt[c * n + row];
        ls.tab[c * n + row] = make_uint2(run, m);
        run += m;
    }
    if (tid == 0) {
        ls.thr[row] = 0;
        ls.flags[row] = F_EXACT;
        ls.rowcnt[row * RCS] = (uint32_t)K;
    }
}

constexpr int RKG_CPW = 4;
__global__ __launch_bounds__(256) void k_randk_gen(RowSrc rows, int64_t n, int64_t d, const uint64_t* __restrict__ ckey,
                                                   float scale, SelWs ws) {
    const int lane = threadIdx.x & 63;
    const int wv = __builtin_amdgcn_readfirstlane(threadIdx.x >> 6);
    const int64_t C = nchunks(d);
    for (int64_t row = blockIdx.y; row < n; row += gridDim.y) {
        const uint64_t k = ckey[row];
        const float* r = rows.row_s(row);
        uint32_t* oi = ws.ent_idx + row * ws.cap;
        float* ov = ws.ent_val + row * ws.cap;
        for (int64_t c0 = ((int64_t)blockIdx.x * 4 + wv) * RKG_CPW; c0 < C; c0 += (int64_t)gridDim.x * 4 * RKG_CPW) {
            uint2 te[RKG_CPW];
            uint32_t col[RKG_CPW];
            float v[RKG_CPW];
#pragma unroll
            for (int q = 0; q < RKG_CPW; ++q) {
                const int64_t c = c0 + q;
                te[q] = c < C ? ws.tab[c * n + row] : make_uint2(0u, 0u);
                const uint32_t clen = (uint32_t)min((int64_t)CHUNK, d - c * CHUNK);
                const rktree::ChunkPerm P(k, c, clen);
                col[q] = (uint32_t)lane < te[q].y ? P((uint32_t)lane) : 0u;
                v[q] = (uint32_t)lane < te[q].y ? r[c * CHUNK + col[q]] : 0.f;
            }
#pragma unroll
            for (int q = 0; q < RKG_CPW; ++q) {
                const int64_t c = c0 + q;
                if ((uint32_t)lane < te[q].y) {
                    oi[te[q].x + lane] = (uint32_t)(c * CHUNK + col[q]);
                    ov[te[q].x + lane] = scale * v[q];
                }
                if (te[q].y > 64u) {
                    const uint32_t clen = (uint32_t)min((int64_t)CHUNK, d - c * CHUNK);
                    const rktree::ChunkPerm P(k, c, clen);
                    for (uint32_t t = 64u + lane; t < te[q].y; t += 64) {
                        const uint32_t cc = P(t);
                        oi[te[q].x + t] = (uint32_t)(c * CHUNK + cc);
                        ov[te[q].x + t] = scale * r[c * CHUNK + cc];
                    }
                }
            }
        }
    }
}

__device__ inline uint64_t join64(uint32_t hi, uint32_t lo) { return ((uint64_t)hi << 32) | (uint64_t)lo; }

struct RkMeta {
    uint32_t m;
    uint32_t klo, khi;
    uint32_t plo, phi;
    float w;
};

__device__ inline RkMeta rk_meta(RowSrc rows, const uint32_t* cnt, const uint64_t* ckey, const float* w, int64_t c,
                                 int64_t n, int64_t r, uint32_t clen) {
    RkMeta m{0u, 0u, 0u, 0u, 0u, 1.f};
    if (r < n) {
        m.m = min(cnt[c * n + r], clen);
        const uint64_t k = ckey[r];
        m.klo = (uint32_t)k;
        m.khi = (uint32_t)(k >> 32);
        const uintptr_t p = (uintptr_t)rows.row(r);
        m.plo = (uint32_t)p;
        m.phi = (uint32_t)((uint64_t)p >> 32);
        if (w) m.w = w[r];
    }
    return m;
}


#ifndef FLC_RK_AP
#define FLC_RK_AP 8
#endif
constexpr int RK_AP = FLC_RK_AP;
template <int TS>
__global__ __launch_bounds__(256) void k_randk_fold(RowSrc rows, int64_t n, int64_t d, const uint32_t* __restrict__ cnt,
                                                    const uint64_t* __restrict__ ckey, float scale,
                                                    const float* __restrict__ w, float wt, float* __restrict__ out) {
    constexpr int PARTS = CHUNK / TS;
    constexpr uint32_t NOCOL = 0xFFFFu;
    __shared__ __attribute__((aligned(16))) float tile[4][TS];
    __shared__ uint32_t zmask[4][TS / 32];
    const int lane = threadIdx.x & 63;
    const int wv = __builtin_amdgcn_readfirstlane(threadIdx.x >> 6);
    const int64_t C = nchunks(d);
    float* tl = tile[wv];
    const int64_t nb = (n + 63) / 64;
    for (int64_t t = (int64_t)blockIdx.x * 4 + wv; t < C * PARTS; t += (int64_t)gridDim.x * 4) {
        const int64_t c = t / PARTS;
        const uint32_t pbase = (uint32_t)((t % PARTS) * TS);
        const int64_t cbase = c * CHUNK;
        const uint32_t clen = (uint32_t)min((int64_t)CHUNK, d - cbase);
        for (int i = lane; i < TS; i += 64) tl[i] = -0.f;
        constexpr int AP = RK_AP;
        uint32_t ro[AP];
        float rv[AP];
        auto fetch = [&](const RkMeta& mt, int q, int slot) {
            const uint32_t m = __builtin_amdgcn_readlane(mt.m, q);
            const uint64_t k = join64((uint32_t)__builtin_amdgcn_readlane(mt.khi, q), (uint32_t)__builtin_amdgcn_readlane(mt.klo, q));
            const float* rp = (const float*)join64((uint32_t)__builtin_amdgcn_readlane(mt.phi, q),
                                                   (uint32_t)__builtin_amdgcn_readlane(mt.plo, q));
            const rktree::ChunkPerm P(k, c, clen);
            uint32_t col = (uint32_t)lane < m ? P((uint32_t)lane) : NOCOL;
            if (PARTS > 1 && col - pbase >= (uint32_t)TS) col = NOCOL;
            const auto rs = chunk_rsrc(rp ? rp : rows.base, cbase, d);
            ro[slot] = col - pbase;
            rv[slot] = __uint_as_float(__builtin_amdgcn_raw_buffer_load_b32(rs, (int)(col * 4u), 0, 0));
        };
        auto fold = [&](int slot, float wi) {
            const uint32_t loc = ro[slot];
            if (loc < (uint32_t)TS) tl[loc] = tl[loc] + wi * (scale * rv[slot]);
        };
        RkMeta cur = rk_meta(rows, cnt, ckey, w, c, n, lane, clen), nxt;
#pragma unroll
        for (int q = 0; q < AP; ++q) fetch(cur, q, q);
        for (int64_t b = 0; b < nb; ++b) {
            const int64_t i0 = b * 64;
            nxt = rk_meta(rows, cnt, ckey, w, c, n, i0 + 64 + lane, clen);
            if (__builtin_expect(__ballot(cur.m > 64u) == 0ull, 1)) {
#pragma unroll
                for (int q = 0; q < 64; ++q) {
                    const int slot = q % AP;
                    fold(slot, __uint_as_float(__builtin_amdgcn_readlane(__float_as_uint(cur.w), q)));
                    if (q + AP < 64) fetch(cur, q + AP, slot);
                    else fetch(nxt, q + AP - 64, slot);
                }
            } else {
                for (int q = 0; q < 64; ++q) {
                    const int slot = q % AP;
                    const float wi = __shfl(cur.w, q, WAVE);
                    uint32_t lo = NOCOL;
                    float vv = 0.f;
#pragma unroll
                    for (int z = 0; z < AP; ++z)
                        if (z == slot) { lo = ro[z]; vv = rv[z]; }
                    if (lo < (uint32_t)TS) tl[lo] = tl[lo] + wi * (scale * vv);
                    const uint32_t m = __shfl(cur.m, q, WAVE);
                    if (m > 64u) {
                        const int64_t row = i0 + q;
                        const rktree::ChunkPerm P(ckey[row], c, clen);
                        const float* rp = rows.row(row);
                        for (uint32_t e = 64u + lane; e < m; e += 64) {
                            const uint32_t col = P(e), l2 = col - pbase;
                            if (l2 < (uint32_t)TS) tl[l2] = tl[l2] + wi * (scale * rp[cbase + col]);
                        }
                    }
                    const RkMeta& mt = (q + AP < 64) ? cur : nxt;
                    const int qq = (q + AP) & 63;
                    const uint32_t mn = __shfl(mt.m, qq, WAVE);
                    const uint64_t kn = join64((uint32_t)__shfl(mt.khi, qq, WAVE), (uint32_t)__shfl(mt.klo, qq, WAVE));
                    const float* rpn = (const float*)join64((uint32_t)__shfl(mt.phi, qq, WAVE), (uint32_t)__shfl(mt.plo, qq, WAVE));
                    const rktree::ChunkPerm Pn(kn, c, clen);
                    const uint32_t col = (uint32_t)lane < mn ? Pn((uint32_t)lane) : NOCOL;
                    const float xv = col < clen ? rpn[cbase + col] : 0.f;
#pragma unroll
                    for (int z = 0; z < AP; ++z)
                        if (z == slot) { ro[z] = col - pbase; rv[z] = xv; }
                }
            }
            cur = nxt;
        }
        const int64_t len = min((int64_t)TS, (int64_t)clen - (int64_t)pbase);
        rk_resolve_neg_zero<TS>(tl, zmask[wv], cnt, ckey, c, n, pbase, clen, len, w, lane);
        for (int64_t i = lane; i < len; i += 64) out[cbase + pbase + i] = tl[i] / wt;
    }
}

__global__ __launch_bounds__(256) void k_randk_scatter_dev(const float* __restrict__ x, int64_t d, const uint32_t* cnt,
                                                           const uint64_t* ckey, float scale, float* __restrict__ out) {
    const int lane = threadIdx.x & 63;
    const int64_t C = nchunks(d);
    const uint64_t k = ckey[0];
    for (int64_t c = ((int64_t)blockIdx.x * 256 + threadIdx.x) / 64; c < C; c += (int64_t)gridDim.x * 4) {
        const int64_t cbase = c * CHUNK;
        const uint32_t clen = (uint32_t)min((int64_t)CHUNK, d - cbase);
        const rktree::ChunkPerm P(k, c, clen);
        const uint32_t m = min(cnt[c], clen);
        for (uint32_t t = (uint32_t)lane; t < m; t += 64) {
            const int64_t j = cbase + P(t);
            out[j] = scale * x[j];
        }
    }
}

__global__ __launch_bounds__(256) void k_assign_scatter(SelWs ws, float* __restrict__ out, int sharded) {
    const uint32_t T = ws.thr[0], f = ws.flags[0];
    const uint32_t mode = (f & F_EXACT) ? 2u : ((f & F_TIES) ? 1u : 0u);
    const uint32_t cut = mode == 1u ? tie_pref(ws.tiecut[0], ws.tie_hi) : 0u;
    const bool shd = sharded && mode != 2u;
    const int64_t segcap = (ws.cap / CS_SH) & ~int64_t(3);
    for (int sh = shd ? (int)blockIdx.x : 0; sh < (shd ? CS_SH : 1); sh += shd ? (int)gridDim.x : 1) {
        const uint32_t cnt = shd ? ws.shcnt[sh * RCS] : ws.rowcnt[0];
        const int64_t o = shd ? sh * segcap : 0;
        for (uint32_t e = (shd ? 0u : blockIdx.x * 256u) + threadIdx.x; e < cnt; e += shd ? 256u : gridDim.x * 256u) {
            const uint32_t ix = ws.ent_idx[o + e];
            const float v = ws.ent_val[o + e];
            const uint32_t key = mag_key(v);
            if (mode == 2u || key > T || (key == T && tie_pref(ix, ws.tie_hi) >= cut)) out[ix] = v;
        }
    }
}

template <bool VEC>
__global__ __launch_bounds__(EX_NT) void k_assign_finish(RowSrc rows, int64_t d, int64_t K, SelWs ws, float* __restrict__ out) {
    __shared__ uint32_t h[HBINS];
    __shared__ uint32_t scratch[260];
    __shared__ uint32_t wsum[EX_NT / 64];
    if (ws.flags[0] & (F_OVERFLOW | F_SHORT)) {
        if (blockIdx.x != 0) return;
        exact_row<VEC>(rows, 1, 0, d, K, ws, h, scratch, wsum);
        __threadfence_block();
        const uint32_t cnt = ws.rowcnt[0];
        for (uint32_t e = threadIdx.x; e < cnt; e += EX_NT) out[ws.ent_idx[e]] = ws.ent_val[e];
        return;
    }
    const uint32_t T = ws.thr[0], f = ws.flags[0];
    const uint32_t cut = (f & F_TIES) ? tie_pref(ws.tiecut[0], ws.tie_hi) : 0u;
    const int64_t segcap = (ws.cap / CS_SH) & ~int64_t(3);
    for (int sh = (int)blockIdx.x; sh < CS_SH; sh += (int)gridDim.x) {
        const uint32_t cnt = ws.shcnt[sh * RCS];
        const int64_t o = sh * segcap;
        for (uint32_t e = threadIdx.x; e < cnt; e += EX_NT) {
            const uint32_t ix = ws.ent_idx[o + e];
            const float v = ws.ent_val[o + e];
            const uint32_t key = mag_key(v);
            if (key > T || (key == T && tie_pref(ix, ws.tie_hi) >= cut)) out[ix] = v;
        }
    }
}

constexpr int RS_NT = 1024;
#ifndef FLC_RS_SPIN
#define FLC_RS_SPIN 10000000ull
#endif

struct RsTree {
    uint32_t* ctl;
    uint32_t grp, gsz, ngr;
};
__device__ inline uint64_t rs_digit(uint32_t bin, uint32_t above, uint32_t last) {
    return (uint64_t)bin | ((uint64_t)above << 11) | ((uint64_t)last << 35);
}
__device__ inline uint32_t rs_gen(const RsTree& tr) {
    return (uint32_t)__hip_atomic_load(reinterpret_cast<const uint64_t*>(tr.ctl + RS_GEN), __ATOMIC_RELAXED, __HIP_MEMORY_SCOPE_AGENT) & 7u;
}
__device__ inline bool rs_arrive(const RsTree& tr, uint32_t* flag_s, uint32_t* gen_s, uint32_t gen) {
    asm volatile("s_waitcnt vmcnt(0)" ::: "memory");
    __syncthreads();
    if (threadIdx.x == 0) {
        *gen_s = gen;
        if (FLC_RS_FENCE) __builtin_amdgcn_fence(__ATOMIC_RELEASE, "agent");
        uint32_t last = 0;
        uint32_t* gc = tr.ctl + RS_GRP + 32 * tr.grp;
#if FLC_RS_FENCE
        if (__hip_atomic_fetch_add(gc, 1u, __ATOMIC_RELAXED, __HIP_MEMORY_SCOPE_AGENT) == tr.gsz - 1u) {
            if (FLC_RS_GACQ) __builtin_amdgcn_fence(__ATOMIC_ACQUIRE, "agent");
            __hip_atomic_store(gc, 0u, __ATOMIC_RELAXED, __HIP_MEMORY_SCOPE_AGENT);
            __builtin_amdgcn_fence(__ATOMIC_RELEASE, "agent");
            if (__hip_atomic_fetch_add(tr.ctl + RS_GLOB, 1u, __ATOMIC_RELAXED, __HIP_MEMORY_SCOPE_AGENT) == tr.ngr - 1u) {
                __hip_atomic_store(tr.ctl + RS_GLOB, 0u, __ATOMIC_RELAXED, __HIP_MEMORY_SCOPE_AGENT);
                last = 1;
                __builtin_amdgcn_fence(__ATOMIC_ACQUIRE, "agent");
            }
        }
#else
        const uint32_t o = __hip_atomic_fetch_add(gc, 1u, __ATOMIC_RELAXED, __HIP_MEMORY_SCOPE_AGENT);
        if ((o + 1u) % tr.gsz == 0u) {
            __hip_atomic_fetch_add(gc, 0u - tr.gsz, __ATOMIC_RELAXED, __HIP_MEMORY_SCOPE_AGENT);
            const uint32_t og = __hip_atomic_fetch_add(tr.ctl + RS_GLOB, 1u, __ATOMIC_RELAXED, __HIP_MEMORY_SCOPE_AGENT);
            if ((og + 1u) % tr.ngr == 0u) {
                __hip_atomic_fetch_add(tr.ctl + RS_GLOB, 0u - tr.ngr, __ATOMIC_RELAXED, __HIP_MEMORY_SCOPE_AGENT);
                last = 1;
            }
        }
        __builtin_amdgcn_fence(__ATOMIC_ACQUIRE, "wavefront");
#endif
        *flag_s = last;
    }
    __syncthreads();
    return *flag_s != 0u;
}
__device__ inline void rs_release(const RsTree& tr, const uint32_t* gen_s, uint64_t payload) {
    asm volatile("s_waitcnt vmcnt(0)" ::: "memory");
    __syncthreads();
    if (threadIdx.x == 0) {
        if (FLC_RS_FENCE) __builtin_amdgcn_fence(__ATOMIC_RELEASE, "agent");
        __hip_atomic_store(reinterpret_cast<uint64_t*>(tr.ctl + RS_GEN), (uint64_t)((*gen_s + 1u) & 7u) | (payload << 3),
                           __ATOMIC_RELAXED, __HIP_MEMORY_SCOPE_AGENT);
    }
}
__device__ inline bool rs_wait(const RsTree& tr, const uint32_t* gen_s, uint32_t* res_s, uint32_t* ok_s,
                               uint32_t* rep_s, uint64_t spin, uint32_t seq, bool raw_bar = false) {
    if (threadIdx.x == 0) {
        const uint64_t* rw = reinterpret_cast<const uint64_t*>(tr.ctl + RS_GEN);
        uint32_t* ab = tr.ctl + RS_GAVE;
        const uint64_t t0 = (uint64_t)wall_clock64();
        uint64_t w;
        uint32_t ok = 1;
        for (uint32_t it = 0;; ++it) {
            w = __hip_atomic_load(rw, __ATOMIC_RELAXED, __HIP_MEMORY_SCOPE_AGENT);
            const uint32_t a = (it % FLC_RS_POLLAB) == FLC_RS_POLLAB - 1
                                   ? __hip_atomic_load(ab, __ATOMIC_RELAXED, __HIP_MEMORY_SCOPE_AGENT) : 0u;
            if (((uint32_t)w & 7u) != *gen_s) break;
            if (a == seq) { ok = 0; break; }
            __builtin_amdgcn_s_sleep(1);
            if ((uint64_t)wall_clock64() - t0 > spin) {
                if (__hip_atomic_exchange(ab, seq, __ATOMIC_RELAXED, __HIP_MEMORY_SCOPE_AGENT) != seq) *rep_s = 1;
                ok = 0;
                break;
            }
        }
        if (FLC_RS_FENCE || !ok) __builtin_amdgcn_fence(__ATOMIC_ACQUIRE, "agent");
        else __builtin_amdgcn_fence(__ATOMIC_ACQUIRE, "wavefront");
        res_s[0] = (uint32_t)(w >> 3);
        res_s[1] = (uint32_t)(w >> 35);
        *ok_s = ok;
    }
    if (raw_bar) {
        asm volatile("s_waitcnt lgkmcnt(0)" ::: "memory");
        __builtin_amdgcn_s_barrier();
        asm volatile("" ::: "memory");
    } else {
        __syncthreads();
    }
    return *ok_s != 0u;
}

__device__ inline void rs_repair(const float* x, uint32_t d, uint32_t K, uint32_t tie_hi, uint32_t* st_thr,
                                 uint32_t* st_krem, uint32_t* st_tiecut, uint32_t* st_flags, float* out,
                                 uint32_t* ctl, uint32_t* h, uint32_t* scratch, uint32_t* wsum) {
    typedef unsigned int u4v __attribute__((ext_vector_type(4)));
    constexpr uint32_t RU4 = 4;
    const uint32_t t = threadIdx.x;
    for (uint32_t i = t; i < (uint32_t)RS_CTL; i += RS_NT)
        if (i < (uint32_t)RS_XGRP || i >= (uint32_t)(RS_XGRP + 32 * RS_NG_MAX))
            __hip_atomic_store(ctl + i, 0u, __ATOMIC_RELAXED, __HIP_MEMORY_SCOPE_AGENT);
    const auto rx = __builtin_amdgcn_make_buffer_rsrc(const_cast<float*>(x), (short)0, (int)(d * 4u), 0x00020000);
    const auto ro = __builtin_amdgcn_make_buffer_rsrc(out, (short)0, (int)(d * 4u), 0x00020000);
    const uint32_t d4 = (d + 3u) / 4u;
    uint32_t prefix = 0, krem = K, ties = 0;
    for (int p = 0; p < 3; ++p) {
        for (uint32_t i = t; i < (uint32_t)HBINS; i += RS_NT) h[i] = 0;
        __syncthreads();
        for (uint32_t f0 = t; f0 < d4; f0 += RU4 * RS_NT) {
            u4v q[RU4];
#pragma unroll
            for (uint32_t u = 0; u < RU4; ++u)
                q[u] = __builtin_amdgcn_raw_buffer_load_b128(rx, (f0 + u * RS_NT) * 16u, 0, 0);
#pragma unroll
            for (uint32_t u = 0; u < RU4; ++u)
#pragma unroll
                for (uint32_t e = 0; e < 4; ++e) {
                    const uint32_t k = q[u][e] & 0x7FFFFFFFu;
                    if ((f0 + u * RS_NT) * 4u + e < d && key_in_prefix(k, p, prefix)) atomicAdd(&h[key_bin(k, p)], 1u);
                }
        }
        __syncthreads();
        uint32_t bin, above;
        hist_find(h, krem, bin, above, scratch);
        prefix = (prefix << pass_bits(p)) | bin;
        krem -= above;
        if (p == 2) ties = h[bin];
        __syncthreads();
    }
    const uint32_t thr = prefix;
    const bool cut = ties > krem;
    const uint32_t from = tie_hi ? ties - krem : 0u, to = tie_hi ? ties : krem;
    uint32_t run = 0;
    for (uint32_t b = 0; b < d4; b += RS_NT) {
        const uint32_t f = b + t;
        const u4v q = __builtin_amdgcn_raw_buffer_load_b128(rx, f * 16u, 0, 0);
        uint32_t ne = 0;
#pragma unroll
        for (uint32_t e = 0; e < 4; ++e) ne += (f * 4u + e < d && (q[e] & 0x7FFFFFFFu) == thr) ? 1u : 0u;
        uint32_t tot;
        uint32_t r = run + ex_scan<RS_NT>(ne, wsum, tot);
        u4v o;
#pragma unroll
        for (uint32_t e = 0; e < 4; ++e) {
            const uint32_t k = q[e] & 0x7FFFFFFFu;
            const bool eq = f * 4u + e < d && k == thr;
            const bool keep = k > thr || (eq && (!cut || (r >= from && r < to)));
            r += eq ? 1u : 0u;
            o[e] = keep ? q[e] : 0u;
        }
        if (f < d4) __builtin_amdgcn_raw_buffer_store_b128(o, ro, f * 16u, 0, 0);
        run += tot;
    }
    if (t == 0) {
        *st_thr = thr;
        *st_krem = krem;
        *st_tiecut = 0;
        *st_flags = F_RESIDENT | F_REPAIR | (cut ? F_TIES : 0u);
    }
}

#ifdef FLC_RS_PRINT
#ifndef FLC_RS_TLK
#define FLC_RS_TLK 0, 4, 1, 2, 3, 10, 12
#endif
#define RS_STAMP(i) do { if (threadIdx.x == 0) stamp[i] = (uint64_t)wall_clock64(); } while (0)
#else
#define RS_STAMP(i) do { } while (0)
#endif
template <int RU>
__global__ __launch_bounds__(RS_NT) void k_lone_resident(RowSrc rows, int64_t d, int64_t K, SelWs ws,
                                                          float* __restrict__ out, int e4, uint32_t* __restrict__ ctl,
                                                          uint32_t seq, uint64_t spin, uint32_t xbase) {
    __shared__ uint32_t h[HBINS];
    __shared__ uint32_t scratch[260];
    __shared__ uint32_t wsum[RS_NT / 64];
    __shared__ uint32_t flag_s, gen_s, ok_s, lcnt_s;
    __shared__ uint64_t lst[RS_CAP];
    const uint32_t G = gridDim.x, g = blockIdx.x, t = threadIdx.x;
#ifdef FLC_RS_PRINT
    uint64_t stamp[18] = {0};
    if (g == 0 && t == 0 && (seq & 15u) == 0u && G <= 256u) {
        const uint64_t* pr = reinterpret_cast<const uint64_t*>(ctl + RS_PROBE);
        const int ks[7] = {FLC_RS_TLK};
        uint64_t s0 = ~0ull;
        for (uint32_t i = 0; i < G; ++i) { const uint64_t v = pr[i]; s0 = v < s0 ? v : s0; }
        uint32_t mg = 0;
        for (uint32_t i = 0; i < G; ++i) if (pr[7 * 256 + i]) mg = i;
        printf("rs_tl G=%u merger %u (x10ns from the first start): ", G, mg);
        for (int k = 0; k < 7; ++k) {
            uint64_t mn = ~0ull, mx = 0, sum = 0;
            for (uint32_t i = 0; i < G; ++i) {
                const uint64_t v = pr[k * 256 + i] - s0;
                mn = v < mn ? v : mn; mx = v > mx ? v : mx; sum += v;
            }
            printf("s%d %llu/%llu/%llu ", ks[k], mn, sum / G, mx);
        }
        printf("\n");
    }
#endif
    RS_STAMP(0);
    RsTree tr;
    tr.ctl = ctl;
    tr.grp = g % RS_NG;
    tr.ngr = min(G, (uint32_t)RS_NG);
    tr.gsz = (G - tr.grp + RS_NG - 1) / RS_NG;
    auto count_out = [&]() {
        if (t == 0 && !FLC_RS_FENCE) asm volatile("s_waitcnt vmcnt(0)" ::: "memory");
        if (t == 0 && !FLC_RS_PROBE_NOCOUNT)
            __hip_atomic_fetch_add(ctl + RS_XGRP + 32 * tr.grp, 1u, __ATOMIC_RELAXED, __HIP_MEMORY_SCOPE_AGENT);
    };
    struct RsExit {
        const float* x;
        float* out;
        uint32_t* ctl;
        uint32_t *thr, *krem, *tiecut, *flags;
        uint32_t d, K, tie_hi, seq, G, xbase;
        uint64_t spin;
    };
    __shared__ RsExit ex_s;
    __shared__ uint32_t rep_s;
    if (t == 0) {
        rep_s = 0;
        lcnt_s = 0;
        ex_s = RsExit{rows.row_s(0), out, ctl, ws.thr, ws.krem, ws.tiecut, ws.flags, (uint32_t)d, (uint32_t)K, ws.tie_hi, seq,
                      G, xbase, spin};
    }
    const uint32_t nb = (uint32_t)(d * 4);
    auto out_rsrc = [&]() {
        const uint64_t op = reinterpret_cast<uint64_t>(ex_s.out);
        const uint32_t lo = __builtin_amdgcn_readfirstlane((uint32_t)op), hi = __builtin_amdgcn_readfirstlane((uint32_t)(op >> 32));
        const uint32_t nbx = __builtin_amdgcn_readfirstlane(ex_s.d * 4u);
        return __builtin_amdgcn_make_buffer_rsrc(reinterpret_cast<float*>(((uint64_t)hi << 32) | lo), (short)0, (int)nbx, 0x00020000);
    };
    const uint32_t f0 = g * (uint32_t)e4 * RS_NT + t;
    const int64_t d4 = (d + 3) / 4;
    const int uv = (int)min((int64_t)e4, max((int64_t)0, (d4 - (int64_t)f0 + RS_NT - 1) / RS_NT));
    const uint32_t pad = (uint32_t)((4 - (d & 3)) & 3);
    const uint32_t padg = (uint32_t)((d / 4) / ((int64_t)e4 * RS_NT));
    const uint32_t voff = f0 * 16u;
    const bool spec = FLC_RS_SPEC && d >= 4 * (int64_t)RS_SS;
    const uint64_t gen_word = __hip_atomic_load(reinterpret_cast<const uint64_t*>(ctl + RS_GEN), __ATOMIC_RELAXED, __HIP_MEMORY_SCOPE_AGENT);
    const int64_t spos = spec ? (int64_t)(t >> 5) * (d - 256) / 31 + (int64_t)(t & 31) * 8 : 0;
    const auto rsm = __builtin_amdgcn_make_buffer_rsrc(const_cast<float*>(rows.row_s(0)), (short)0, spec ? (int)nb : 0, 0x00020000);
    const auto sa = __builtin_amdgcn_raw_buffer_load_b128(rsm, (uint32_t)(spos * 4), 0, 0);
    const auto sb = __builtin_amdgcn_raw_buffer_load_b128(rsm, (uint32_t)(spos * 4 + 16), 0, 0);
    const int64_t gb = (int64_t)g * e4 * RS_NT * 4;
    const auto rxg = __builtin_amdgcn_make_buffer_rsrc(const_cast<float*>(rows.row_s(0)) + gb, (short)0,
                                                       (int)(min((int64_t)e4 * RS_NT * 4, d - gb) * 4), 0x00020000);
    float4 v[RU];
#pragma unroll
    for (int u = 0; u < RU; ++u) {
        const auto q = __builtin_amdgcn_raw_buffer_load_b128(rxg, t * 16u, u * RS_NT * 16, FLC_LOADPOL);
        v[u] = make_float4(__uint_as_float(q[0]), __uint_as_float(q[1]), __uint_as_float(q[2]), __uint_as_float(q[3]));
    }
#ifdef FLC_RS_PRINT
    if (t < 64) {
        asm volatile("s_waitcnt vmcnt(0)" ::: "memory");
        RS_STAMP(4);
    }
#endif
#if defined(FLC_RS_EXIT) && FLC_RS_EXIT == 3
    {
        typedef unsigned int u4v __attribute__((ext_vector_type(4)));
        const uint64_t op = reinterpret_cast<uint64_t>(out);
        const auto rq = __builtin_amdgcn_make_buffer_rsrc(reinterpret_cast<float*>(op), (short)0, (int)nb, 0x00020000);
#pragma unroll
        for (int u = 0; u < RU; ++u)
            if (u < uv) {
                const u4v ov = {__float_as_uint(v[u].x), __float_as_uint(v[u].y), __float_as_uint(v[u].z), __float_as_uint(v[u].w)};
                __builtin_amdgcn_raw_buffer_store_b128(ov, rq, voff, u * RS_NT * 16, FLC_RS_STPOL);
            }
        return;
    }
#endif
#if defined(FLC_RS_EXIT) && FLC_RS_EXIT == 1
    {
        uint32_t a = 0;
#pragma unroll
        for (int u = 0; u < RU; ++u) a |= __float_as_uint(v[u].x);
        if (a == 0x7FFFFFFFu) out[0] = 1.f;
        return;
    }
#endif
    uint32_t prefix = 0, krem = (uint32_t)K, last = 0, bar = 0;
    bool cand = false;
    uint32_t bs = 0;
    int p0 = 0;
    uint32_t winm = 0;
    bool sst = false;
    typedef unsigned int u4v __attribute__((ext_vector_type(4)));
    if (spec) {
        __shared__ uint32_t h1[3 * HBINS];
        __shared__ uint32_t hs[RS_SR * (HBINS + 1)];
        const uint32_t gen = (uint32_t)gen_word & 7u;
        for (int i = t; i < RS_SR * (HBINS + 1); i += RS_NT) hs[i] = 0;
        for (int i = t; i < 3 * HBINS; i += RS_NT) h1[i] = 0;
        lds_bar();
        {
            uint32_t* hr = hs + (t % RS_SR) * (HBINS + 1);
#pragma unroll
            for (int q = 0; q < 4; ++q) {
                atomicAdd(&hr[(sa[q] & 0x7FFFFFFFu) >> 20], 1u);
                atomicAdd(&hr[(sb[q] & 0x7FFFFFFFu) >> 20], 1u);
            }
        }
        lds_bar();
        for (int i = t; i < HBINS; i += RS_NT) {
            uint32_t c = 0;
#pragma unroll
            for (int r = 0; r < RS_SR; ++r) c += hs[r * (HBINS + 1) + i];
            h[i] = c;
        }
        lds_bar();
        RS_STAMP(5);
#if defined(FLC_RS_EXIT) && FLC_RS_EXIT == 2
        if (h[t] == 0x7FFFFFFFu) out[0] = 1.f;
        return;
#endif
        uint32_t ab;
        const uint32_t rs = (uint32_t)min((int64_t)RS_SS, max((int64_t)1, (K * RS_SS + d / 2) / d));
        hist_find<true>(h, rs, bs, ab, scratch);
        lds_bar();
        RS_STAMP(6);
        uint32_t km = 0x7FFFFFFFu;
        asm volatile("" : "+s"(km));
        const uint32_t wlo = (bs - 1u) << 20, whi = (bs + 2u) << 20;
        uint32_t abv = 0;
#pragma unroll
        for (int u = 0; u < RU; ++u) {
            if (u < uv) {
                const float e[4] = {v[u].x, v[u].y, v[u].z, v[u].w};
#pragma unroll
                for (int q = 0; q < 4; ++q) {
                    const uint32_t k = __float_as_uint(e[q]) & km;
                    const uint32_t dd = k - wlo;
                    abv += (uint32_t)__popcll(__ballot(k >= whi));
                    if (dd < (3u << 20)) {
                        atomicAdd(&h1[dd >> 9], 1u);
                        winm |= 1u << u;
                    }
                }
            }
        }
        RS_STAMP(7);
        if (t == 0) scratch[0] = 0;
        __syncthreads();
        if ((t & 63) == 0 && abv) atomicAdd(&scratch[0], abv);
        __syncthreads();
        RS_STAMP(1);
#if defined(FLC_RS_EXIT) && FLC_RS_EXIT == 4
        if (scratch[0] == 0x7FFFFFFFu) out[0] = 1.f;
        return;
#endif
        auto spec_store = [&]() {
            if (!FLC_RS_SPECST) return;
            const auto ro = out_rsrc();
            int uvx = uv;
            uint32_t wmx = winm;
            asm volatile("" : "+v"(uvx), "+v"(wmx));
#pragma unroll
            for (int u = 0; u < RU; ++u) {
                if (u < uvx && !((wmx >> u) & 1u)) {
                    const float e[4] = {v[u].x, v[u].y, v[u].z, v[u].w};
                    uint32_t o[4];
#pragma unroll
                    for (int q = 0; q < 4; ++q) o[q] = (mag_key(e[q]) >> 20) > bs + 1u ? __float_as_uint(e[q]) : 0u;
                    const u4v ov = {o[0], o[1], o[2], o[3]};
                    __builtin_amdgcn_raw_buffer_store_b128(ov, ro, voff + (uint32_t)(u * RS_NT * 16), 0, FLC_RS_STPOL);
                }
            }
        };
        uint32_t* gs = ctl + RS_HSPEC + tr.grp * 3 * HBINS;
        for (int i = t; i < 3 * HBINS; i += RS_NT)
            if (h1[i]) __hip_atomic_fetch_add(gs + i, h1[i], __ATOMIC_RELAXED, __HIP_MEMORY_SCOPE_AGENT);
        if (t == 0 && scratch[0]) __hip_atomic_fetch_add(ctl + RS_ABV + 32 * tr.grp, scratch[0], __ATOMIC_RELAXED, __HIP_MEMORY_SCOPE_AGENT);
        ++bar;
        if (FLC_RS_SPECST && t < 64) winm = 0xFFFFu;
        const bool mg_ = rs_arrive(tr, &flag_s, &gen_s, gen);
#if defined(FLC_RS_EXIT) && FLC_RS_EXIT == 5
        return;
#endif
        if (mg_) {
            RS_STAMP(2);
#ifdef FLC_RS_PRINT
            stamp[13] = 1;
#endif
            uint32_t* s0 = ctl + RS_HSPEC;
            constexpr int ML = RS_NG * 3 * HBINS / RS_NT;
            uint32_t mv[ML];
#pragma unroll
            for (int j = 0; j < ML; ++j) mv[j] = __hip_atomic_load(s0 + t + j * RS_NT, __ATOMIC_RELAXED, __HIP_MEMORY_SCOPE_AGENT);
            const uint32_t ar = t < RS_NG ? __hip_atomic_load(ctl + RS_ABV + 32 * t, __ATOMIC_RELAXED, __HIP_MEMORY_SCOPE_AGENT) : 0u;
            for (int i = t; i < 3 * HBINS; i += RS_NT) h1[i] = 0;
            __syncthreads();
#pragma unroll
            for (int j = 0; j < ML; ++j) {
                const int i = (t + j * RS_NT) % (3 * HBINS);
                if (mv[j]) atomicAdd(&h1[i], mv[j]);
            }
            if (t < 64) {
                const uint32_t a4 = wave_sum(ar);
                if (t == 0) scratch[259] = a4;
            }
            __syncthreads();
            if (t < 2) {
                if (bs + (uint32_t)t == 1u) h1[t * HBINS] -= pad;
            }
            __syncthreads();
            const uint32_t A = scratch[259];
            uint32_t bb = 0, ab = 0;
            bool found = false;
            if (A < (uint32_t)K) hist_find_n<3 * HBINS>(h1, (uint32_t)K - A, bb, ab, found, scratch);
            uint64_t pl = 0;
            if (found) {
                const uint32_t w0 = bb / HBINS, b1 = bb % HBINS, b0 = bs - 1u + w0;
                pl = 1ull | ((uint64_t)((b0 << 11) | b1) << 1) | ((uint64_t)((uint32_t)K - A - ab) << 23) |
                     ((uint64_t)min(h1[bb], 16383u) << 47);
            }
            rs_release(tr, &gen_s, pl);
            if (t == 0) { scratch[0] = (uint32_t)pl; scratch[1] = (uint32_t)(pl >> 32); }
            RS_STAMP(3);
            spec_store();
            if (t < RS_NG) __hip_atomic_store(ctl + RS_ABV + 32 * t, 0u, __ATOMIC_RELAXED, __HIP_MEMORY_SCOPE_AGENT);
            for (int i = t; i < 3 * RS_NG * HBINS; i += RS_NT)
                __hip_atomic_store(s0 + i, 0u, __ATOMIC_RELAXED, __HIP_MEMORY_SCOPE_AGENT);
        } else {
            RS_STAMP(2);
            spec_store();
            if (!rs_wait(tr, &gen_s, scratch, &ok_s, &rep_s, spin, seq, true)) goto leave;
        }
        asm volatile("s_waitcnt lgkmcnt(0)" ::: "memory");
        __builtin_amdgcn_s_barrier();
        const uint64_t pl = ((uint64_t)scratch[1] << 32) | scratch[0];
        asm volatile("s_waitcnt lgkmcnt(0)" ::: "memory");
        __builtin_amdgcn_s_barrier();
        if (pl & 1u) {
            prefix = (uint32_t)(pl >> 1) & 0x3FFFFFu;
            krem = (uint32_t)(pl >> 23) & 0xFFFFFFu;
            last = (uint32_t)(pl >> 47);
            p0 = 2;
            cand = last <= (uint32_t)RS_CAP;
            sst = FLC_RS_SPECST;
        }
#if defined(FLC_RS_EXIT) && FLC_RS_EXIT == 6
        return;
#endif
        RS_STAMP(3);
    }
    for (int p = p0; p < 3 && !cand; ++p) {
        const uint32_t gen = (p == 0 && !spec) ? ((uint32_t)gen_word & 7u) : (t == 0 ? rs_gen(tr) : 0u);
        for (int i = t; i < HBINS; i += RS_NT) h[i] = 0;
        __syncthreads();
        uint32_t km = 0x7FFFFFFFu;
        asm volatile("" : "+s"(km));
#pragma unroll
        for (int u = 0; u < RU; ++u) {
            if (u < uv) {
                const float e[4] = {v[u].x, v[u].y, v[u].z, v[u].w};
#pragma unroll
                for (int q = 0; q < 4; ++q) {
                    const uint32_t k = __float_as_uint(e[q]) & km;
                    if (key_in_prefix(k, p, prefix)) atomicAdd(&h[key_bin(k, p)], 1u);
                }
            }
        }
        __syncthreads();
        RS_STAMP(1 + 3 * p);
        uint32_t* gh = ctl + RS_HREP + (p * RS_NG + tr.grp) * HBINS;
        for (int i = t; i < HBINS; i += RS_NT)
            if (h[i]) __hip_atomic_fetch_add(gh + i, h[i], __ATOMIC_RELAXED, __HIP_MEMORY_SCOPE_AGENT);
        ++bar;
        if (rs_arrive(tr, &flag_s, &gen_s, gen)) {
            RS_STAMP(2 + 3 * p);
            uint32_t* r0 = ctl + RS_HREP + p * RS_NG * HBINS;
            for (int i = t; i < HBINS; i += RS_NT) {
                uint32_t c = 0;
#pragma unroll
                for (int r = 0; r < RS_NG; ++r) c += __hip_atomic_load(r0 + r * HBINS + i, __ATOMIC_RELAXED, __HIP_MEMORY_SCOPE_AGENT);
                h[i] = (i == 0 && prefix == 0u) ? c - pad : c;
            }
            __syncthreads();
            uint32_t bin, above;
            hist_find(h, krem, bin, above, scratch);
            const uint64_t pl = rs_digit(bin, above, h[bin]);
            rs_release(tr, &gen_s, pl);
            if (t == 0) { scratch[0] = (uint32_t)pl; scratch[1] = (uint32_t)(pl >> 32); }
            for (int i = t; i < HBINS; i += RS_NT)
#pragma unroll
                for (int r = 0; r < RS_NG; ++r) __hip_atomic_store(r0 + r * HBINS + i, 0u, __ATOMIC_RELAXED, __HIP_MEMORY_SCOPE_AGENT);
        } else {
            RS_STAMP(2 + 3 * p);
            if (!rs_wait(tr, &gen_s, scratch, &ok_s, &rep_s, spin, seq)) goto leave;
        }
        __syncthreads();
        const uint64_t pl = ((uint64_t)scratch[1] << 32) | scratch[0];
        const uint32_t bin = (uint32_t)pl & 0x7FFu, above = (uint32_t)(pl >> 11) & 0xFFFFFFu;
        last = (uint32_t)(pl >> 35);
        prefix = (prefix << pass_bits(p)) | bin;
        krem -= above;
        __syncthreads();
        RS_STAMP(3 + 3 * p);
        if (p == 1 && last <= (uint32_t)RS_CAP) { cand = true; break; }
    }
    if (cand) {
        const uint32_t P = prefix;
        const uint32_t plo = P << 9;
#pragma unroll
        for (int u = 0; u < RU; ++u) {
            if (u < uv) {
                const float e[4] = {v[u].x, v[u].y, v[u].z, v[u].w};
#pragma unroll
                for (int q = 0; q < 4; ++q) {
                    if (mag_key(e[q]) - plo < 512u) {
                        const uint32_t j = (f0 + u * RS_NT) * 4u + (uint32_t)q;
                        if ((int64_t)j < d) {
                            const uint32_t pp = atomicAdd(&lcnt_s, 1u);
                            if (pp < (uint32_t)RS_CAP) lst[pp] = ((uint64_t)__float_as_uint(e[q]) << 32) | j;
                        }
                    }
                }
            }
        }
        lds_bar();
        const uint32_t ctot = lcnt_s;
        RS_STAMP(9);
        if (FLC_RS_DONE && t < 64 && ctot) {
            uint64_t* cl = reinterpret_cast<uint64_t*>(ctl + RS_CLIST);
            uint32_t ob = 0;
            if (t == 0) ob = __hip_atomic_fetch_add(ctl + RS_CCNT, ctot, __ATOMIC_RELAXED, __HIP_MEMORY_SCOPE_AGENT);
            const uint32_t obase = __shfl(ob, 0, 64);
            const uint32_t nl = min(ctot, (uint32_t)RS_CAP);
            for (uint32_t i = t; i < nl; i += 64)
                if (obase + i < (uint32_t)RS_CAP) __hip_atomic_store(cl + obase + i, lst[i], __ATOMIC_RELAXED, __HIP_MEMORY_SCOPE_AGENT);
            asm volatile("s_waitcnt vmcnt(0)" ::: "memory");
            if (t == 0) __hip_atomic_fetch_add(ctl + RS_CDONE, ctot, __ATOMIC_RELAXED, __HIP_MEMORY_SCOPE_AGENT);
        }
        if (!FLC_RS_DONE && t < 64) {
            uint64_t* cl = reinterpret_cast<uint64_t*>(ctl + RS_CLIST);
            uint64_t* cr = reinterpret_cast<uint64_t*>(ctl + RS_CREG) + (size_t)g * RS_CS;
            uint32_t ob = 0;
            if (ctot > (uint32_t)RS_CS && t == 0)
                ob = __hip_atomic_fetch_add(ctl + RS_CCNT, ctot - (uint32_t)RS_CS, __ATOMIC_RELAXED, __HIP_MEMORY_SCOPE_AGENT);
            const uint32_t obase = __shfl(ob, 0, 64);
            const uint32_t nl = min(ctot, (uint32_t)RS_CAP);
            for (uint32_t i = t; i < nl; i += 64) {
                const uint64_t en = lst[i];
                if (i < (uint32_t)RS_CS) __hip_atomic_store(cr + i, en, __ATOMIC_RELAXED, __HIP_MEMORY_SCOPE_AGENT);
                else if (obase + i - RS_CS < (uint32_t)RS_CAP)
                    __hip_atomic_store(cl + obase + i - RS_CS, en, __ATOMIC_RELAXED, __HIP_MEMORY_SCOPE_AGENT);
            }
            if (t == 0) __hip_atomic_store(ctl + RS_CNUM + g, ctot, __ATOMIC_RELAXED, __HIP_MEMORY_SCOPE_AGENT);
            asm volatile("s_waitcnt vmcnt(0)" ::: "memory");
        }
        auto dense = [&]() {
            const auto ro = out_rsrc();
            int uvx = uv;
            uint32_t wmx = sst ? winm : 0xFFFFu;
            asm volatile("" : "+v"(uvx), "+v"(wmx));
#pragma unroll
            for (int u = 0; u < RU; ++u) {
                if (u < uvx && ((wmx >> u) & 1u)) {
                    const float e[4] = {v[u].x, v[u].y, v[u].z, v[u].w};
                    uint32_t o[4];
                    bool at[4], any = false;
#pragma unroll
                    for (int q = 0; q < 4; ++q) {
                        const uint32_t k = mag_key(e[q]);
                        o[q] = k >= plo + 512u ? __float_as_uint(e[q]) : 0u;
                        at[q] = k - plo < 512u;
                        any |= at[q];
                    }
                    if (!any) {
                        const u4v ov = {o[0], o[1], o[2], o[3]};
                        __builtin_amdgcn_raw_buffer_store_b128(ov, ro, voff, u * RS_NT * 16, FLC_RS_STPOL);
                    } else {
#pragma unroll
                        for (int q = 0; q < 4; ++q)
                            if (!at[q]) __builtin_amdgcn_raw_buffer_store_b32(o[q], ro, voff + 4u * q, u * RS_NT * 16, FLC_RS_STPOL);
                    }
                }
            }
        };
        RS_STAMP(10);
        if (g != G - 1u) {
            count_out();
            lds_bar();
#if defined(FLC_RS_EXIT) && FLC_RS_EXIT == 7
            return;
#endif
            dense();
        } else {
            if (!FLC_RS_RANKFIRST) dense();
            const RsExit ex = ex_s;
            if (t == 0) {
                const uint64_t t0 = (uint64_t)wall_clock64();
                uint32_t okw = 1;
                for (;;) {
                    if (FLC_RS_DONE) {
                        if (__hip_atomic_load(ex.ctl + RS_CDONE, __ATOMIC_RELAXED, __HIP_MEMORY_SCOPE_AGENT) >= last) break;
                    } else {
                        uint32_t out_n = 0;
#pragma unroll
                        for (int r = 0; r < RS_NG; ++r)
                            out_n += __hip_atomic_load(ex.ctl + RS_XGRP + 32 * r, __ATOMIC_RELAXED, __HIP_MEMORY_SCOPE_AGENT);
                        if (out_n - ex.xbase >= ex.G - 1u) break;
                    }
                    __builtin_amdgcn_s_sleep(1);
                    if ((uint64_t)wall_clock64() - t0 > ex.spin) {
                        if (__hip_atomic_exchange(ex.ctl + RS_GAVE, ex.seq, __ATOMIC_RELAXED, __HIP_MEMORY_SCOPE_AGENT) != ex.seq) rep_s = 1;
                        okw = 0;
                        break;
                    }
                }
                __builtin_amdgcn_fence(__ATOMIC_ACQUIRE, "wavefront");
                ok_s = okw;
            }
            __syncthreads();
            if (!ok_s) goto leave;
            __shared__ uint64_t comp[RS_CAP];
            __shared__ uint64_t ent[RS_CAP];
            __shared__ uint64_t kth_s;
            uint32_t m, ns, ovn, mm;
            bool ok;
            if (FLC_RS_DONE) {
                if (t == 0) {
                    scratch[4] = __hip_atomic_load(ex.ctl + RS_CCNT, __ATOMIC_RELAXED, __HIP_MEMORY_SCOPE_AGENT);
                    scratch[5] = __hip_atomic_load(ex.ctl + RS_CDONE, __ATOMIC_RELAXED, __HIP_MEMORY_SCOPE_AGENT);
                }
                __syncthreads();
                m = scratch[4];
                ok = m == last && scratch[5] == last && m >= krem && krem >= 1u && m <= (uint32_t)RS_CAP;
                mm = ok ? m : 0u;
                for (uint32_t i = t; i < mm; i += RS_NT)
                    ent[i] = __hip_atomic_load(reinterpret_cast<const uint64_t*>(ex.ctl + RS_CLIST) + i, __ATOMIC_RELAXED, __HIP_MEMORY_SCOPE_AGENT);
                ovn = 1u;
            } else {
            uint32_t c = 0;
            uint64_t sl[RS_CS];
            if (t < ex.G) {
                c = __hip_atomic_load(ex.ctl + RS_CNUM + t, __ATOMIC_RELAXED, __HIP_MEMORY_SCOPE_AGENT);
                const uint64_t* ct = reinterpret_cast<const uint64_t*>(ex.ctl + RS_CREG) + (size_t)t * RS_CS;
#pragma unroll
                for (int k = 0; k < RS_CS; ++k) sl[k] = __hip_atomic_load(ct + k, __ATOMIC_RELAXED, __HIP_MEMORY_SCOPE_AGENT);
            }
            const uint32_t ov = t == 0 ? __hip_atomic_load(ex.ctl + RS_CCNT, __ATOMIC_RELAXED, __HIP_MEMORY_SCOPE_AGENT) : 0u;
            if (t == 0) scratch[4] = ov;
            const uint32_t cs = min(c, (uint32_t)RS_CS);
            (void)ex_scan<RS_NT>(c, wsum, m);
            const uint32_t sp = ex_scan<RS_NT>(cs, wsum, ns);
            ovn = scratch[4];
            ok = m == last && ovn == m - ns && m >= krem && krem >= 1u && m <= (uint32_t)RS_CAP;
            mm = ok ? m : 0u;
            if (ok) {
#pragma unroll
                for (int k = 0; k < RS_CS; ++k)
                    if ((uint32_t)k < cs) ent[sp + k] = sl[k];
                for (uint32_t i = t; i < ovn; i += RS_NT) ent[ns + i] = __hip_atomic_load(reinterpret_cast<const uint64_t*>(ex.ctl + RS_CLIST) + i, __ATOMIC_RELAXED, __HIP_MEMORY_SCOPE_AGENT);
            }
            }
            if (t == 0) { scratch[2] = 0; scratch[3] = 0; kth_s = ~0ull; }
            __syncthreads();
            for (uint32_t i = t; i < mm; i += RS_NT) {
                const uint64_t en = ent[i];
                comp[i] = ((uint64_t)((uint32_t)(en >> 32) & 0x7FFFFFFFu) << 32) | tie_pref((uint32_t)en, ex.tie_hi);
            }
            __syncthreads();
            for (uint32_t i = t; i < mm; i += RS_NT) {
                const uint64_t me = comp[i];
                uint32_t rank = 0;
                for (uint32_t jj = 0; jj < mm; ++jj) rank += comp[jj] > me ? 1u : 0u;
                if (rank == krem - 1u) kth_s = me;
            }
            __syncthreads();
            const uint64_t kc = kth_s;
            const uint32_t kth = (uint32_t)(kc >> 32);
            for (uint32_t i = t; i < mm; i += RS_NT) {
                const uint64_t me = comp[i];
                const uint64_t en = ent[i];
                ex.out[(uint32_t)en] = me >= kc ? __uint_as_float((uint32_t)(en >> 32)) : 0.f;
                const uint32_t key = (uint32_t)(me >> 32);
                if (key > kth) atomicAdd(&scratch[2], 1u);
                else if (key == kth) atomicAdd(&scratch[3], 1u);
            }
            __syncthreads();
            if (t == 0) {
                if (ovn) __hip_atomic_store(ex.ctl + RS_CCNT, 0u, __ATOMIC_RELAXED, __HIP_MEMORY_SCOPE_AGENT);
                if (FLC_RS_DONE) __hip_atomic_store(ex.ctl + RS_CDONE, 0u, __ATOMIC_RELAXED, __HIP_MEMORY_SCOPE_AGENT);
                const uint32_t gt = scratch[2], eq = scratch[3];
                *ex.thr = kth;
                *ex.krem = krem - gt;
                *ex.tiecut = tie_pref((uint32_t)kc, ex.tie_hi);
                *ex.flags = F_RESIDENT | (gt + eq > krem ? F_TIES : 0u);
                if (!ok && __hip_atomic_exchange(ex.ctl + RS_GAVE, ex.seq, __ATOMIC_RELAXED, __HIP_MEMORY_SCOPE_AGENT) != ex.seq)
                    rep_s = 1;
            }
            if (!ok) goto leave;
            if (t == 0) {
                asm volatile("s_waitcnt vmcnt(0)" ::: "memory");
                __hip_atomic_fetch_add(ex.ctl + RS_XGRP + 32 * (blockIdx.x % RS_NG), 1u, __ATOMIC_RELAXED, __HIP_MEMORY_SCOPE_AGENT);
            }
            if (FLC_RS_RANKFIRST) dense();
        }
        RS_STAMP(11);
    } else {
    const uint32_t thr = prefix;
    const bool tie_cut = last > krem;
    uint64_t tmask = 0;
    if (tie_cut) {
        uint32_t c = 0;
#pragma unroll
        for (int u = 0; u < RU; ++u) {
            if (u < uv) {
                const float e[4] = {v[u].x, v[u].y, v[u].z, v[u].w};
#pragma unroll
                for (int q = 0; q < 4; ++q) c += mag_key(e[q]) == thr ? 1u : 0u;
            }
        }
        uint32_t tot;
        (void)ex_scan<RS_NT>(c, wsum, tot);
        if (thr == 0u && g == padg) tot -= pad;
        uint64_t* tc = reinterpret_cast<uint64_t*>(ctl + RS_TCNT);
        if (t == 0) __hip_atomic_store(tc + g, ((uint64_t)seq << 32) | tot, __ATOMIC_RELEASE, __HIP_MEMORY_SCOPE_AGENT);
        if (tot == 0u) goto store;
        uint32_t part = 0, run = 0;
        int bail = 0;
        const uint64_t t0 = (uint64_t)wall_clock64();
        for (uint32_t i = t; i < g && !bail; i += RS_NT) {
            uint64_t w;
            for (;;) {
                w = __hip_atomic_load(tc + i, __ATOMIC_ACQUIRE, __HIP_MEMORY_SCOPE_AGENT);
                const uint32_t a = __hip_atomic_load(ctl + RS_GAVE, __ATOMIC_RELAXED, __HIP_MEMORY_SCOPE_AGENT);
                if ((uint32_t)(w >> 32) == seq) break;
                if (a == seq) { bail = 1; break; }
                __builtin_amdgcn_s_sleep(1);
                if ((uint64_t)wall_clock64() - t0 > spin) {
                    if (__hip_atomic_exchange(ctl + RS_GAVE, seq, __ATOMIC_RELAXED, __HIP_MEMORY_SCOPE_AGENT) != seq)
                        rep_s = 1;
                    bail = 1;
                    break;
                }
            }
            part += (uint32_t)w;
        }
        if (__syncthreads_or(bail)) goto leave;
        (void)ex_scan<RS_NT>(part, wsum, run);
        const uint32_t tie_from = ws.tie_hi ? last - krem : 0u, tie_to = ws.tie_hi ? last : krem;
#pragma unroll
        for (int u = 0; u < RU; ++u) {
            if (u < e4) {
                const float e[4] = {v[u].x, v[u].y, v[u].z, v[u].w};
                uint32_t ce = 0;
#pragma unroll
                for (int q = 0; q < 4; ++q) ce += (u < uv && mag_key(e[q]) == thr) ? 1u : 0u;
                uint32_t tu;
                uint32_t r = run + ex_scan<RS_NT>(ce, wsum, tu);
                run += tu;
#pragma unroll
                for (int q = 0; q < 4; ++q)
                    if (u < uv && mag_key(e[q]) == thr) {
                        if (r >= tie_from && r < tie_to) tmask |= 1ull << (4 * u + q);
                        ++r;
                    }
            }
        }
    }
store:
    RS_STAMP(10);
    if (g == 0 && t == 0) {
#if FLC_RS_FENCE
        ws.thr[0] = thr;
        ws.krem[0] = krem;
        ws.tiecut[0] = 0;
        ws.flags[0] = F_RESIDENT | (tie_cut ? F_TIES : 0u);
        if (FLC_RS_G0REL) __builtin_amdgcn_fence(__ATOMIC_RELEASE, "agent");
#else
        __hip_atomic_store(ws.thr, thr, __ATOMIC_RELAXED, __HIP_MEMORY_SCOPE_AGENT);
        __hip_atomic_store(ws.krem, krem, __ATOMIC_RELAXED, __HIP_MEMORY_SCOPE_AGENT);
        __hip_atomic_store(ws.tiecut, 0u, __ATOMIC_RELAXED, __HIP_MEMORY_SCOPE_AGENT);
        __hip_atomic_store(ws.flags, F_RESIDENT | (tie_cut ? F_TIES : 0u), __ATOMIC_RELAXED, __HIP_MEMORY_SCOPE_AGENT);
        asm volatile("s_waitcnt vmcnt(0)" ::: "memory");
#endif
    }
    count_out();
    const auto ro = out_rsrc();
    int uvx = uv;
    uint32_t wmx = sst ? winm : 0xFFFFu;
    asm volatile("" : "+v"(uvx), "+v"(wmx));
#pragma unroll
    for (int u = 0; u < RU; ++u) {
        if (u < uvx && ((wmx >> u) & 1u)) {
            const float e[4] = {v[u].x, v[u].y, v[u].z, v[u].w};
            uint32_t o[4];
#pragma unroll
            for (int q = 0; q < 4; ++q) {
                const uint32_t k = mag_key(e[q]);
                const bool keep = k > thr || (k == thr && (!tie_cut || ((tmask >> (4 * u + q)) & 1ull)));
                o[q] = keep ? __float_as_uint(e[q]) : 0u;
            }
            const u4v ov = {o[0], o[1], o[2], o[3]};
            __builtin_amdgcn_raw_buffer_store_b128(ov, ro, voff, u * RS_NT * 16, FLC_RS_STPOL);
        }
    }
    RS_STAMP(11);
    (void)bar;
    }
    goto done;
leave:
    if (t == 0) {
        __builtin_amdgcn_fence(__ATOMIC_RELEASE, "agent");
    }
    if (!rep_s) count_out();
    __syncthreads();
    if (rep_s) {
        const RsExit ex = ex_s;
        if (t == 0) {
            const uint64_t t0 = (uint64_t)wall_clock64();
            for (;;) {
                uint32_t out_n = 0;
                for (int r = 0; r < RS_NG; ++r)
                    out_n += __hip_atomic_load(ex.ctl + RS_XGRP + 32 * r, __ATOMIC_RELAXED, __HIP_MEMORY_SCOPE_AGENT);
                if (out_n - ex.xbase >= ex.G - 1u || (uint64_t)wall_clock64() - t0 >= 64 * ex.spin) break;
                __builtin_amdgcn_s_sleep(8);
            }
            __builtin_amdgcn_fence(__ATOMIC_ACQUIRE, "agent");
        }
        __syncthreads();
        rs_repair(ex.x, ex.d, ex.K, ex.tie_hi, ex.thr, ex.krem, ex.tiecut, ex.flags, ex.out, ex.ctl, h, scratch, wsum);
        __syncthreads();
        if (t == 0) __builtin_amdgcn_fence(__ATOMIC_RELEASE, "agent");
        count_out();
    }
done:;
#ifdef FLC_RS_PRINT
    asm volatile("s_waitcnt vmcnt(0)" ::: "memory");
    __syncthreads();
    RS_STAMP(12);
    if (t == 0 && G <= 256u) {
        uint64_t* pr = reinterpret_cast<uint64_t*>(ex_s.ctl + RS_PROBE);
        const int ks[8] = {FLC_RS_TLK, 13};
        for (int k = 0; k < 8; ++k) __hip_atomic_store(pr + k * 256 + g, stamp[ks[k]], __ATOMIC_RELAXED, __HIP_MEMORY_SCOPE_AGENT);
    }
#endif
}

static int64_t host_chunks(int64_t d) { return (d + CHUNK - 1) / CHUNK; }

int64_t sel_capacity(int codec, int64_t d, int64_t K) {
    if (codec == FLC_RANDK) return std::max<int64_t>(K, 1);
    int64_t cap = 2 * K + 2 * CHUNK;
    cap = std::min<int64_t>(std::max<int64_t>(cap, 1), std::max<int64_t>(d, 1));
    return (cap + 3) & ~int64_t(3);
}

static SelWs carve_sel(void* base, int codec, int64_t n, int64_t d, int64_t K, size_t* bytes) {
    Carver cv(base);
    const int64_t C = std::max<int64_t>(host_chunks(d), 1), nn = std::max<int64_t>(n, 1);
    SelWs s;
    s.tie_hi = 0;
    s.cap = sel_capacity(codec, d, K);
    s.tab = cv.take<uint2>((size_t)C * nn);
    s.ent_idx = cv.take<uint32_t>((size_t)nn * s.cap);
    s.ent_val = cv.take<float>((size_t)nn * s.cap);
    s.rowcnt = cv.take<uint32_t>((size_t)nn * RCS);
    s.flags = cv.take<uint32_t>(nn);
    s.thr = cv.take<uint32_t>(nn);
    s.prefix = cv.take<uint32_t>(nn);
    s.krem = cv.take<uint32_t>(nn);
    s.worklist = cv.take<uint32_t>(nn);
    s.nwork = cv.take<uint32_t>(4);
    s.zm = cv.take<uint32_t>((size_t)C * (CHUNK / 32));
    s.part = codec == FLC_TOPK ? cv.take<float>((size_t)C * CHUNK) : nullptr;
    if (codec == FLC_TOPK) {
        s.tieprefix = cv.take<uint32_t>((size_t)C * nn);
        s.tiecut = cv.take<uint32_t>(nn);
        s.hist = cv.take<uint32_t>((size_t)nn * HBINS);
        s.cursor = nullptr;
        s.cstate = cv.take<uint32_t>((size_t)nn * CS_ST);
        s.clist = cv.take<uint64_t>((size_t)std::min<int64_t>(nn, CS_FEW) * CS_LCAP);
        s.carrive = cv.take<uint32_t>((size_t)nn * RCS);
        s.shcnt = cv.take<uint32_t>((size_t)std::min<int64_t>(nn, CS_FEW) * CS_SH * RCS);
    } else {
        s.tieprefix = nullptr;
        s.tiecut = nullptr;
        s.hist = nullptr;
        s.cursor = cv.take<uint32_t>((size_t)std::max<int64_t>(C, RK_SB) * nn);
        s.cstate = nullptr;
        s.clist = nullptr;
        s.carrive = nullptr;
        s.shcnt = nullptr;
    }
    if (bytes) *bytes = cv.bytes();
    return s;
}

size_t randk_device_workspace(int64_t n, int64_t d);

size_t sel_workspace(const flc_codec_params* prm, int64_t n, int64_t d) {
    size_t b = 0;
    carve_sel(nullptr, prm->codec, n, d, prm->k, &b);
    if (prm->codec == FLC_RANDK) b += randk_device_workspace(n, d);
    return b;
}

static int grid_stride_blocks(int64_t items, int64_t cap = 4096) {
    return (int)std::max<int64_t>(1, std::min<int64_t>(items, cap));
}

static int accum_parts() {
    static const int p = [] {
        const char* e = tuning_env("FLC_ACCUM_PARTS");
        const int v = e ? atoi(e) : 0;
        return (v == 1 || v == 2 || v == 4) ? v : 0;
    }();
    return p;
}

static bool assign_fold() {
    static const bool v = [] { const char* e = tuning_env("FLC_ASSIGN_FOLD"); return e && atoi(e) == 1; }();
    return v;
}

static bool cs_single() {
    static const bool v = [] { const char* e = tuning_env("FLC_CS_SINGLE"); return e && atoi(e) == 1; }();
    return v;
}

#ifndef FLC_LONE_PATH
#define FLC_LONE_PATH 2
#endif
#ifndef FLC_RS_EVREC
#define FLC_RS_EVREC 1
#endif
#ifndef FLC_RS_COOP
#define FLC_RS_COOP 0
#endif
struct RsCtx {
    uint32_t* ctl = nullptr;
    uint32_t seq = 0;
    uint32_t xcum = 0;
    hipStream_t last = nullptr;
    hipEvent_t done = nullptr;
};
static std::mutex g_rs_mu;
static std::map<int, RsCtx> g_rs_ctx;
static std::atomic<int> g_rs_dbg_mult{1};
static std::atomic<long long> g_rs_dbg_spin{0};
int rs_debug(int mult, int64_t spin_ticks) {
    if (mult < 1 || mult > 64 || spin_ticks < 0) { set_error("flc_debug_resident: mult 1..64, spin >= 0"); return FLC_ERR_ARG; }
    g_rs_dbg_mult.store(mult);
    g_rs_dbg_spin.store((long long)spin_ticks);
    return FLC_OK;
}
static int rs_cus() {
    static int cu[64] = {0};
    int dev = 0;
    if (hipGetDevice(&dev) != hipSuccess || dev < 0 || dev >= 64) return 0;
    if (!cu[dev]) {
        int c = 0;
        if (hipDeviceGetAttribute(&c, hipDeviceAttributeMultiprocessorCount, dev) != hipSuccess) return 0;
        cu[dev] = c;
    }
    return cu[dev];
}
static int lone_path() {
    static const int v = [] { const char* e = tuning_env("FLC_LONE_PATH"); return e ? atoi(e) : FLC_LONE_PATH; }();
    return v;
}

static int filter_group() {
    static const int g = [] {
        const char* e = tuning_env("FLC_FILTER_GS");
        return (e && atoi(e) == 2) ? 2 : 4;
    }();
    return g;
}

template <int FGS>
static void launch_filter(RowSrc rows, int64_t n, int64_t r0, int64_t rn, int64_t d, SelWs ws, hipStream_t st,
                          int shards, float* zout = nullptr) {
    const int64_t waves = rn * ((nchunks(d) + FGS - 1) / FGS);
    const int gw = (int)std::max<int64_t>(1, std::min<int64_t>((waves + 3) / 4, 32768));
    static const int64_t rb = [] {
        const char* e = tuning_env("FLC_TK_RB");
        return e ? std::max<int64_t>(1, atoll(e)) : (int64_t)64;
    }();
    ProfScope _pv(FGS == 4 ? "k_topk_filter_g4" : "k_topk_filter_g2", st);
    if constexpr (FGS == 4 && FLC_TK_WG != 0 && FLC_TK_PROBE != 1 && FLC_TK_PROBE != 3) {
        static const bool wg = [] { const char* e = tuning_env("FLC_FILTER_WG"); return !(e && atoi(e) == 0); }();
        if (wg && shards == 1 && !zout) {
            constexpr int NL = FLC_TK_WG_NL;
            const int64_t items = rn * ((nchunks(d) + 4 * NL - 1) / (4 * NL));
            const int gi = (int)std::max<int64_t>(1, std::min<int64_t>(items, 32768));
            static const int64_t rbw = [] {
                const char* e = tuning_env("FLC_TK_RB");
                return e ? std::max<int64_t>(1, atoll(e)) : (int64_t)16;
            }();
            hipLaunchKernelGGL((k_topk_filter_fast_wg<FLC_TK_WG_RING, NL>), dim3(gi), dim3((NL + 1) * 64), 0, st, rows, n, r0,
                               rn, std::min(rbw, std::max<int64_t>(rn, 1)), d, ws);
            return;
        }
    }
    if (zout)
        hipLaunchKernelGGL((k_topk_filter_fast<FLC_TK_RING, FGS, 1>), dim3(gw), dim3(256), 0, st, rows, n, r0, rn,
                           std::min(rb, std::max<int64_t>(rn, 1)), d, ws, shards, zout);
    else
        hipLaunchKernelGGL((k_topk_filter_fast<FLC_TK_RING, FGS>), dim3(gw), dim3(256), 0, st, rows, n, r0, rn,
                           std::min(rb, std::max<int64_t>(rn, 1)), d, ws, shards, (float*)nullptr);
}

#ifndef FLC_TK_SPLIT_SAMPLE
#define FLC_TK_SPLIT_SAMPLE 1
#endif
#ifndef FLC_TK_LASTPCT
#define FLC_TK_LASTPCT 100
#endif
static_assert(FLC_TK_LASTPCT >= 1 && FLC_TK_LASTPCT <= 100, "FLC_TK_LASTPCT: the last row group is 1..100 % of the others");
#ifndef FLC_TK_LAST_TS
#define FLC_TK_LAST_TS 4096
#endif
#ifndef FLC_TK_GFOLD
#define FLC_TK_GFOLD 1
#endif
#ifndef FLC_TK_SIDE_NT
#define FLC_TK_SIDE_NT 512
#endif
#ifndef FLC_TK_EXACT_WG
#define FLC_TK_EXACT_WG 256
#endif
static int tk_tail_groups(const flc_codec_params* prm, int64_t n) {
    static const int g = [] { const char* e = tuning_env("FLC_TK_TAILOV"); return e ? std::max(1, atoi(e)) : 4; }();
    const int hint = (prm->flags >> 8) & 0xFF;
    if (hint) return (int)std::max<int64_t>(1, std::min<int64_t>(hint, n));
    return (int)std::max<int64_t>(1, std::min<int64_t>(g, n / 64));
}
namespace {
struct TkCtx {
    hipStream_t side = nullptr;
    std::vector<hipEvent_t> ev;
};
std::mutex g_tk_mu;
std::map<int, TkCtx> g_tk_ctx;
}

static int launch_chunk_accum(int64_t n, int64_t d, SelWs ws, bool assign, const float* w, float wt, float* out,
                              hipStream_t st);

static RkdWs carve_rkd(void* base, int64_t n, int64_t d, size_t* bytes) {
    Carver cv(base);
    const int64_t C = std::max<int64_t>(host_chunks(d), 1), nn = std::max<int64_t>(n, 1);
    RkdWs s;
    s.cnt = cv.take<uint32_t>((size_t)C * nn);
    s.ckey = cv.take<uint64_t>((size_t)nn);
    if (bytes) *bytes = cv.bytes();
    return s;
}

size_t randk_device_workspace(int64_t n, int64_t d) {
    size_t b = 0;
    carve_rkd(nullptr, n, d, &b);
    return b;
}

static int randk_counts(const flc_codec_params* prm, const flc_pattern* pat, int64_t n, int64_t d, RkdWs ws,
                        hipStream_t st) {
    ProfScope _ps("k_randk_counts", st);
    const int64_t parts = (host_chunks(d) + RKC_BINS - 1) / RKC_BINS;
    hipLaunchKernelGGL(k_randk_counts, dim3((unsigned)parts, (unsigned)n), dim3(RKC_NT), 0, st, n, d, prm->k, prm->seed,
                       pat ? pat->client0 : (int64_t)0, ws);
    FLC_CHECK_LAUNCH("k_randk_counts");
    return FLC_OK;
}

static int randk_counts_or_given(const flc_codec_params* prm, const flc_pattern* pat, int64_t n, int64_t d, RkdWs* rw,
                                 hipStream_t st) {
    if (pat && pat->d_randk_counts) {
        rw->cnt = const_cast<uint32_t*>(pat->d_randk_counts);
        hipLaunchKernelGGL(k_randk_ckeys, dim3((unsigned)((n + 255) / 256)), dim3(256), 0, st, n, prm->seed,
                           pat->client0, rw->ckey);
        FLC_CHECK_LAUNCH("k_randk_ckeys");
        return FLC_OK;
    }
    return randk_counts(prm, pat, n, d, *rw, st);
}

int randk_device_prepare(const flc_codec_params* prm, const flc_pattern* pat, int64_t n, int64_t d, void* wsp,
                         const uint32_t** cnt, const uint64_t** ckey, hipStream_t st) {
    RkdWs rw = carve_rkd(wsp, n, d, nullptr);
    if (int rc = randk_counts_or_given(prm, pat, n, d, &rw, st)) return rc;
    *cnt = rw.cnt;
    *ckey = rw.ckey;
    return FLC_OK;
}

int randk_device_counts(uint64_t seed, int64_t client0, int64_t n, int64_t d, int64_t k, uint32_t* cnt, void* wsp,
                        size_t ws_bytes, hipStream_t st) {
    if (ws_bytes < randk_device_workspace(n, d)) { set_error("randk counts: workspace too small"); return FLC_ERR_WORKSPACE; }
    RkdWs ws = carve_rkd(wsp, n, d, nullptr);
    ws.cnt = cnt;
    flc_codec_params prm{};
    prm.codec = FLC_RANDK;
    prm.k = k;
    prm.seed = seed;
    flc_pattern pat{};
    pat.client0 = client0;
    return randk_counts(&prm, &pat, n, d, ws, st);
}

int randk_device_run(const flc_codec_params* prm, const flc_pattern* pat, RowSrc rows, int64_t n, int64_t d,
                     const float* w, float wt, float* out, void* wsp, size_t ws_bytes, hipStream_t st) {
    size_t lb = 0;
    carve_sel(nullptr, FLC_RANDK, n, d, prm->k, &lb);
    if (ws_bytes < lb + randk_device_workspace(n, d)) { set_error("randk: workspace too small"); return FLC_ERR_WORKSPACE; }
    SelWs sw = carve_sel(wsp, FLC_RANDK, n, d, prm->k, nullptr);
    RkdWs rw = carve_rkd(static_cast<char*>(wsp) + lb, n, d, nullptr);
    const int64_t C = host_chunks(d);
    auto counts = [&]() -> int { return randk_counts_or_given(prm, pat, n, d, &rw, st); };
    if (C >= 1024) {
        if (int rc = counts()) return rc;
        ProfScope _ps("k_randk_fold", st);
        const int ab = grid_stride_blocks((C + 3) / 4, 16384);
        hipLaunchKernelGGL((k_randk_fold<CHUNK>), dim3(ab), dim3(256), 0, st, rows, n, d, rw.cnt, rw.ckey,
                           prm->randk_scale, w, wt, out);
        FLC_CHECK_LAUNCH("k_randk_fold");
        return FLC_OK;
    }
    if (int rc = counts()) return rc;
    hipLaunchKernelGGL(k_randk_tab, dim3((unsigned)n), dim3(256), 0, st, n, d, prm->k, rw.cnt, sw);
    FLC_CHECK_LAUNCH("k_randk_tab");
    {
        ProfScope _ps("k_randk_gen", st);
        const int64_t gx = std::max<int64_t>(1, std::min<int64_t>((C + 4 * RKG_CPW - 1) / (4 * RKG_CPW), 4096));
        hipLaunchKernelGGL(k_randk_gen, dim3((unsigned)gx, (unsigned)std::min<int64_t>(n, 65535)), dim3(256), 0, st, rows,
                           n, d, rw.ckey, prm->randk_scale, sw);
        FLC_CHECK_LAUNCH("k_randk_gen");
    }
    return launch_chunk_accum(n, d, sw, false, w, wt, out, st);
}

static int launch_group_fold(int64_t n, int64_t d, SelWs ws, const float* w, float wt, float* out, int64_t r0, int64_t r1,
                             bool first, bool last, bool exposed, hipStream_t st) {
    const int64_t C = host_chunks(d);
    ProfScope _ps("k_chunk_accum", st);
    if (!exposed) {
        const int ab = grid_stride_blocks(C, 16384);
        if (w) hipLaunchKernelGGL((k_chunk_accum1<true>), dim3(ab), dim3(64), CHUNK * sizeof(float), st, n, d, ws, w, wt, out, r0, r1,
                                  first ? 1 : 0, last ? 1 : 0);
        else hipLaunchKernelGGL((k_chunk_accum1<false>), dim3(ab), dim3(64), CHUNK * sizeof(float), st, n, d, ws, w, wt, out, r0, r1,
                                first ? 1 : 0, last ? 1 : 0);
    } else {
        constexpr int LTS = FLC_TK_LAST_TS;
        const int ab = grid_stride_blocks((C * (CHUNK / LTS) + 3) / 4, 4096);
        if (w) hipLaunchKernelGGL((k_chunk_accum<false, LTS, true>), dim3(ab), dim3(256), 0, st, n, d, ws, w, wt, out, r0, r1,
                                  first ? 1 : 0, last ? 1 : 0);
        else hipLaunchKernelGGL((k_chunk_accum<false, LTS, false>), dim3(ab), dim3(256), 0, st, n, d, ws, w, wt, out, r0, r1,
                                first ? 1 : 0, last ? 1 : 0);
    }
    FLC_CHECK_LAUNCH("k_chunk_accum(group)");
    return FLC_OK;
}

static int launch_chunk_accum(int64_t n, int64_t d, SelWs ws, bool assign, const float* w, float wt, float* out,
                              hipStream_t st) {
    const int64_t C = host_chunks(d);
    { ProfScope _ps("k_chunk_accum", st);
    int parts = accum_parts();
    if (parts == 0) parts = C >= 1024 ? 1 : (C >= 256 ? 2 : 4);
    auto go = [&](auto ts, int ab) {
        constexpr int TS = decltype(ts)::value;
        if (assign) hipLaunchKernelGGL((k_chunk_accum<true, TS>), dim3(ab), dim3(256), 0, st, n, d, ws, w, wt, out);
        else if (w) hipLaunchKernelGGL((k_chunk_accum<false, TS, true>), dim3(ab), dim3(256), 0, st, n, d, ws, w, wt, out);
        else hipLaunchKernelGGL((k_chunk_accum<false, TS, false>), dim3(ab), dim3(256), 0, st, n, d, ws, w, wt, out);
    };
    if (parts == 4) go(std::integral_constant<int, CHUNK / 4>{}, grid_stride_blocks((4 * C + 3) / 4, 8192));
    else if (parts == 2) go(std::integral_constant<int, CHUNK / 2>{}, grid_stride_blocks((2 * C + 3) / 4, 8192));
    else if (FLC_CA_WPB1 && !assign) {
        const int ab = grid_stride_blocks(C, 16384);
        if (w) hipLaunchKernelGGL((k_chunk_accum1<true>), dim3(ab), dim3(64), CHUNK * sizeof(float), st, n, d, ws, w, wt, out, (int64_t)0, n, 1, 1);
        else hipLaunchKernelGGL((k_chunk_accum1<false>), dim3(ab), dim3(64), CHUNK * sizeof(float), st, n, d, ws, w, wt, out, (int64_t)0, n, 1, 1);
    } else go(std::integral_constant<int, CHUNK>{}, grid_stride_blocks((C + 3) / 4, 4096));
    }
    FLC_CHECK_LAUNCH("k_chunk_accum");
    return FLC_OK;
}

size_t randk_lists_workspace(int64_t n, int64_t d, int64_t K) {
    size_t b = 0;
    carve_sel(nullptr, FLC_RANDK, n, d, K, &b);
    return b;
}

static int randk_lists_launch(const flc_codec_params* prm, const flc_pattern* pat, RowSrc rows, int64_t n, int64_t d,
                              SelWs ws, hipStream_t st) {
    const int64_t K = prm->k, C = host_chunks(d);
    const int64_t ldi = pat->idx_ld ? pat->idx_ld : K;
    const int64_t spc = rk_spc(C), sb = (C + spc - 1) / spc;
    { ProfScope _ps("k_randk_coarse", st);
    if (spc == 1)
        hipLaunchKernelGGL(k_randk_coarse<true>, dim3((unsigned)n), dim3(RK_T), 0, st, rows, n, d, K, *pat, ldi,
                           prm->randk_scale, ws);
    else
        hipLaunchKernelGGL(k_randk_coarse<false>, dim3((unsigned)n), dim3(RK_T), 0, st, rows, n, d, K, *pat, ldi,
                           prm->randk_scale, ws); }
    FLC_CHECK_LAUNCH("k_randk_coarse");
    if (spc > 1) {
        ProfScope _ps("k_randk_fine", st);
        hipLaunchKernelGGL(k_randk_fine, dim3((unsigned)sb, (unsigned)n), dim3(RK_FTHR), (size_t)spc * sizeof(uint32_t),
                           st, rows, n, d, K, prm->randk_scale, ws);
        FLC_CHECK_LAUNCH("k_randk_fine");
    }
    return FLC_OK;
}

int randk_lists_build(const flc_codec_params* prm, const flc_pattern* pat, RowSrc rows, int64_t n, int64_t d, void* wsp,
                      RkLists* lists, hipStream_t st) {
    SelWs ws = carve_sel(wsp, FLC_RANDK, n, d, prm->k, nullptr);
    lists->tab = ws.tab;
    lists->idx = ws.ent_idx;
    lists->val = ws.ent_val;
    lists->cap = ws.cap;
    return randk_lists_launch(prm, pat, rows, n, d, ws, st);
}

int randk_lists_fold(int64_t n, int64_t d, int64_t K, void* wsp, const float* w, float wt, float* out, hipStream_t st) {
    return launch_chunk_accum(n, d, carve_sel(wsp, FLC_RANDK, n, d, K, nullptr), false, w, wt, out, st);
}

int sel_run(const flc_codec_params* prm, const flc_pattern* pat, RowSrc rows, bool vec, int64_t n, int64_t d,
            bool assign, const float* w, float wt, float* out, void* wsp, size_t ws_bytes, hipStream_t st) {
    const int codec = prm->codec;
    const int64_t K = prm->k;
    if (d == 0) return FLC_OK;
    if (n == 0) { FLC_CHECK_HIP(hipMemsetAsync(out, 0, (size_t)d * sizeof(float), st)); return FLC_OK; }
    if (K < 1 || K > d) { set_error("K=%lld outside [1, D=%lld]", (long long)K, (long long)d); return FLC_ERR_ARG; }
    if (d >= (int64_t)0xFFFFFFFF) { set_error("D too large for 32-bit entry indices"); return FLC_ERR_ARG; }
    if (codec == FLC_RANDK && !(pat && pat->d_randk_idx))
        return randk_device_run(prm, pat, rows, n, d, w, wt, out, wsp, ws_bytes, st);
    size_t need = 0;
    carve_sel(nullptr, codec, n, d, K, &need);
    if (ws_bytes < need) { set_error("select: workspace %zu < %zu", ws_bytes, need); return FLC_ERR_WORKSPACE; }
    SelWs ws = carve_sel(wsp, codec, n, d, K, nullptr);
    if (codec == FLC_TOPK) {
        if (prm->tie != FLC_TIE_LOWEST && prm->tie != FLC_TIE_HIGHEST) { set_error("topk: unknown tie rule %d", prm->tie); return FLC_ERR_ARG; }
        ws.tie_hi = prm->tie == FLC_TIE_HIGHEST ? 1u : 0u;
    }
    const int64_t C = host_chunks(d);
    bool lone_assign = false, gfold = false;
    const bool few = codec == FLC_TOPK && n <= CS_FEW && !cs_single() && sel_capacity(codec, d, K) >= (int64_t)CS_SH * GCAP;
    if (codec == FLC_RANDK) {
        if (int rc = randk_lists_launch(prm, pat, rows, n, d, ws, st)) return rc;
    } else {
        hipStreamCaptureStatus cap = hipStreamCaptureStatusNone;
        if (assign && n == 1 && !assign_fold() && lone_path() == 2) FLC_CHECK_HIP(hipStreamIsCapturing(st, &cap));
        if (assign && n == 1 && !assign_fold() && lone_path() == 2 && cap == hipStreamCaptureStatusNone) {
            const int64_t cus = rs_cus();
            const int mult = std::max(1, g_rs_dbg_mult.load());
            const int64_t G = std::min<int64_t>(cus * mult, (d + RS_NT * 4 - 1) / (RS_NT * 4));
            const int64_t e4 = G > 0 ? (d + G * RS_NT * 4 - 1) / (G * RS_NT * 4) : RS_U + 1;
            if (e4 <= RS_U && d * 4 < ((int64_t)1 << 31)) {
                const int64_t Gu = (d + e4 * RS_NT * 4 - 1) / (e4 * RS_NT * 4);
                const long long dspin = g_rs_dbg_spin.load();
                const uint64_t spin = dspin > 0 ? (uint64_t)dspin : (uint64_t)FLC_RS_SPIN;
                ProfScope _ps("k_lone_resident", st);
                int dev = 0;
                FLC_CHECK_HIP(hipGetDevice(&dev));
                std::lock_guard<std::mutex> lk(g_rs_mu);
                RsCtx& rc = g_rs_ctx[dev];
                if (!rc.ctl) {
                    FLC_CHECK_HIP(hipMalloc(reinterpret_cast<void**>(&rc.ctl), (size_t)RS_CTL * sizeof(uint32_t)));
                    FLC_CHECK_HIP(hipMemsetAsync(rc.ctl, 0, (size_t)RS_CTL * sizeof(uint32_t), st));
                    FLC_CHECK_HIP(hipEventCreateWithFlags(&rc.done, FLC_SYNC_EVENT_FLAGS));
                }
                if (rc.last && rc.last != st) {
                    if (!FLC_RS_EVREC) FLC_CHECK_HIP(hipEventRecord(rc.done, rc.last));
                    FLC_CHECK_HIP(hipStreamWaitEvent(st, rc.done, 0));
                }
                if (++rc.seq == 0u) rc.seq = 1u;
                const int e4i = (int)e4;
                if (FLC_RS_COOP) {
                    RowSrc ra = rows;
                    int64_t da = d, ka = K;
                    SelWs wa = ws;
                    float* oa = out;
                    int ea = e4i;
                    uint32_t* ca = rc.ctl;
                    uint32_t sa = rc.seq;
                    uint64_t pa = spin;
                    uint32_t xa = rc.xcum;
                    void* args[] = {&ra, &da, &ka, &wa, &oa, &ea, &ca, &sa, &pa, &xa};
                    FLC_CHECK_HIP(hipLaunchCooperativeKernel(reinterpret_cast<const void*>(&k_lone_resident<RS_U>), dim3((unsigned)Gu),
                                                             dim3(RS_NT), args, 0, st));
                } else {
                    hipLaunchKernelGGL((k_lone_resident<RS_U>), dim3((unsigned)Gu), dim3(RS_NT), 0, st, rows, d, K, ws, out, e4i,
                                       rc.ctl, rc.seq, spin, rc.xcum);
                }
                FLC_CHECK_LAUNCH("k_lone_resident");
                rc.xcum += (uint32_t)Gu;
                if (FLC_RS_EVREC) FLC_CHECK_HIP(hipEventRecord(rc.done, st));
                rc.last = st;
                return FLC_OK;
            }
        }
        const bool dense_k = K * 16 > d;
        lone_assign = assign && n == 1 && few && !dense_k && !assign_fold();

        if (dense_k) FLC_CHECK_HIP(hipMemsetAsync(ws.hist, 0, (size_t)n * HBINS * sizeof(uint32_t), st));
        const int64_t bpr = (C + 3) / 4;
        if (!dense_k) {
            const int TG = few ? 1 : tk_tail_groups(prm, n);
            gfold = FLC_TK_GFOLD && !few && !assign && !dense_k;
            hipStream_t sside = st;
            TkCtx* cx = nullptr;
            std::unique_lock<std::mutex> lk;
            if (TG > 1) {
                int dev = 0;
                FLC_CHECK_HIP(hipGetDevice(&dev));
                lk = std::unique_lock<std::mutex>(g_tk_mu);
                cx = &g_tk_ctx[dev];
                if (!cx->side) {
                    int lo = 0, hi = 0;
                    FLC_CHECK_HIP(hipDeviceGetStreamPriorityRange(&lo, &hi));
                    FLC_CHECK_HIP(hipStreamCreateWithPriority(&cx->side, hipStreamNonBlocking, hi));
                }
                while ((int)cx->ev.size() < TG + 3) {
                    hipEvent_t e;
                    FLC_CHECK_HIP(hipEventCreateWithFlags(&e, FLC_SYNC_EVENT_FLAGS));
                    cx->ev.push_back(e);
                }
                sside = cx->side;
            }
            const bool split = FLC_TK_SPLIT_SAMPLE && TG > 1;
            const int64_t rs1 = split ? group_row(n, TG, 1, FLC_TK_LASTPCT) : n;
            auto sample = [&](int64_t a, int64_t b, hipStream_t sx) {
                if (b <= a) return;
                ProfScope _ps("k_topk_sample", sx);
                hipLaunchKernelGGL((few ? k_topk_sample<1024, true> : k_topk_sample<1024, false>), dim3((unsigned)(b - a)), dim3(1024), 0, sx,
                                   rows, n, d, K, ws, few ? 1 : 0, a);
            };
            if (split) {
                FLC_CHECK_HIP(hipEventRecord(cx->ev[TG + 1], st));
                FLC_CHECK_HIP(hipStreamWaitEvent(sside, cx->ev[TG + 1], 0));
            }
            sample(0, rs1, st);
            FLC_CHECK_LAUNCH("k_topk_sample");
            if (split) {
                sample(rs1, n, sside);
                FLC_CHECK_LAUNCH("k_topk_sample (side)");
                FLC_CHECK_HIP(hipEventRecord(cx->ev[TG + 2], sside));
            }
            for (int g = 0; g < TG; ++g) {
                const int64_t r0 = group_row(n, TG, g, FLC_TK_LASTPCT), rn = group_row(n, TG, g + 1, FLC_TK_LASTPCT) - r0;
                if (split && g == 1) FLC_CHECK_HIP(hipStreamWaitEvent(st, cx->ev[TG + 2], 0));
                { ProfScope _ps("k_topk_filter", st);
                float* zout = lone_assign ? out : nullptr;
                if (filter_group() == 2 || n * d < ((int64_t)64 << 20)) launch_filter<2>(rows, n, r0, rn, d, ws, st, few ? CS_SH : 1, zout);
                else launch_filter<4>(rows, n, r0, rn, d, ws, st, few ? CS_SH : 1, zout); }
                FLC_CHECK_LAUNCH("k_topk_filter");
                if (TG > 1) {
                    FLC_CHECK_HIP(hipEventRecord(cx->ev[g], st));
                    FLC_CHECK_HIP(hipStreamWaitEvent(sside, cx->ev[g], 0));
                }
                { ProfScope _ps("k_cand_select", sside);
                if (few) {
                    const int np = (FLC_CS_LIST && d <= FLC_CS_TWO_MAXD) ? 2 : 3;
                    for (int p = 0; p < np; ++p)
                        hipLaunchKernelGGL(k_cs_pass, dim3((unsigned)CS_SH, (unsigned)n), dim3(CS_NT), 0, st, K, ws,
                                           p == np - 1 ? 1 : 0);
                } else if (gfold) {
                    const bool big = rn < 128 || g == TG - 1;
                    const int nt = big ? 1024 : FLC_TK_SIDE_NT;
                    const dim3 grid((unsigned)(big ? rn : grid_stride_blocks(rn, 8192)));
                    if (big) {
                        if (vec) hipLaunchKernelGGL((k_cand_select_x<1024, true>), grid, dim3(nt), 0, sside, rows, n, r0, rn, d, K, ws);
                        else hipLaunchKernelGGL((k_cand_select_x<1024, false>), grid, dim3(nt), 0, sside, rows, n, r0, rn, d, K, ws);
                    } else if (FLC_TK_SIDE_NT == 256) {
                        if (vec) hipLaunchKernelGGL((k_cand_select_x<256, true>), grid, dim3(nt), 0, sside, rows, n, r0, rn, d, K, ws);
                        else hipLaunchKernelGGL((k_cand_select_x<256, false>), grid, dim3(nt), 0, sside, rows, n, r0, rn, d, K, ws);
                    } else {
                        if (vec) hipLaunchKernelGGL((k_cand_select_x<512, true>), grid, dim3(nt), 0, sside, rows, n, r0, rn, d, K, ws);
                        else hipLaunchKernelGGL((k_cand_select_x<512, false>), grid, dim3(nt), 0, sside, rows, n, r0, rn, d, K, ws);
                    }
                } else if (rn < 128 || (TG > 1 && g == TG - 1))
                    hipLaunchKernelGGL(k_cand_select<1024>, dim3((unsigned)rn), dim3(1024), 0, sside, r0, rn, K, ws);
                else if (FLC_TK_SIDE_NT == 256)
                    hipLaunchKernelGGL(k_cand_select<256>, dim3(grid_stride_blocks(rn, 8192)), dim3(256), 0, sside, r0, rn, K, ws);
                else hipLaunchKernelGGL(k_cand_select<512>, dim3(grid_stride_blocks(rn, 8192)), dim3(512), 0, sside, r0, rn, K, ws); }
                FLC_CHECK_LAUNCH("k_cand_select");
                if (gfold) {
                    const bool lastg = g == TG - 1;
                    if (int rc = launch_group_fold(n, d, ws, w, wt, out, r0, r0 + rn, g == 0, lastg, lastg || TG == 1, sside))
                        return rc;
                }
            }
            if (!lone_assign && !gfold) {
                ProfScope _ps("k_topk_exact_rows", sside);
                const int eb = grid_stride_blocks(n, FLC_TK_EXACT_WG);
                if (vec) hipLaunchKernelGGL((k_topk_exact_rows<true>), dim3(eb), dim3(EX_NT), 0, sside, rows, n, (int64_t)0, n, d, K, ws);
                else hipLaunchKernelGGL((k_topk_exact_rows<false>), dim3(eb), dim3(EX_NT), 0, sside, rows, n, (int64_t)0, n, d, K, ws);
                FLC_CHECK_LAUNCH("k_topk_exact_rows");
            }
            if (TG > 1) {
                FLC_CHECK_HIP(hipEventRecord(cx->ev[TG], sside));
                FLC_CHECK_HIP(hipStreamWaitEvent(st, cx->ev[TG], 0));
            }
        } else {
            FLC_CHECK_HIP(hipMemsetAsync(ws.flags, 0, (size_t)n * sizeof(uint32_t), st));
        }
        if (dense_k) {
        hipLaunchKernelGGL(k_build_worklist, dim3(1), dim3(1024), 0, st, n, K, d, ws, 1);
        FLC_CHECK_LAUNCH("k_build_worklist");
        const int64_t hb = (d + 65535) / 65536;
        for (int p = 0; p < 3; ++p) {
            { ProfScope _ps("k_radix_hist_full", st);
hipLaunchKernelGGL((k_radix_hist<true>), dim3(grid_stride_blocks(n * hb)), dim3(256), 0, st, rows, n, d, p, ws); }
            FLC_CHECK_LAUNCH("k_radix_hist(full)");
            hipLaunchKernelGGL((k_radix_select<true>), dim3(grid_stride_blocks(n, 1024)), dim3(256), 0, st, n, p, K, ws);
            FLC_CHECK_LAUNCH("k_radix_select(full)");
        }
        hipLaunchKernelGGL(k_tie_count, dim3(grid_stride_blocks(n * bpr, 4096)), dim3(256), 0, st, rows, n, d, ws);
        FLC_CHECK_LAUNCH("k_tie_count");
        hipLaunchKernelGGL(k_tie_scan, dim3(grid_stride_blocks(n, 1024)), dim3(256), 0, st, n, d, ws);
        FLC_CHECK_LAUNCH("k_tie_scan");
        int gb = grid_stride_blocks(n * bpr, 8192);
        { ProfScope _ps("k_topk_filter_exact", st);
if (vec) hipLaunchKernelGGL((k_topk_filter<true, true>), dim3(gb), dim3(256), 0, st, rows, n, d, ws);
        else hipLaunchKernelGGL((k_topk_filter<true, false>), dim3(gb), dim3(256), 0, st, rows, n, d, ws); }
        FLC_CHECK_LAUNCH("k_topk_filter(exact)");
        }
    }
    if (lone_assign) {
        ProfScope _ps("k_assign_finish", st);
        if (vec) hipLaunchKernelGGL((k_assign_finish<true>), dim3(CS_SH), dim3(EX_NT), 0, st, rows, d, K, ws, out);
        else hipLaunchKernelGGL((k_assign_finish<false>), dim3(CS_SH), dim3(EX_NT), 0, st, rows, d, K, ws, out);
        FLC_CHECK_LAUNCH("k_assign_finish");
        return FLC_OK;
    }
    if (gfold) return FLC_OK;
    if (assign && n == 1 && codec == FLC_TOPK && !assign_fold()) {
        FLC_CHECK_HIP(hipMemsetAsync(out, 0, (size_t)d * sizeof(float), st));
        const int sb = (int)std::max<int64_t>(1, std::min<int64_t>((sel_capacity(codec, d, K) + 255) / 256, 2048));
        hipLaunchKernelGGL(k_assign_scatter, dim3(sb), dim3(256), 0, st, ws, out, few ? 1 : 0);
        FLC_CHECK_LAUNCH("k_assign_scatter");
        return FLC_OK;
    }
    return launch_chunk_accum(n, d, ws, assign, w, wt, out, st);
}

int sel_row_flags(const flc_codec_params* prm, int64_t n, int64_t d, const void* wsp, size_t ws_bytes,
                  uint32_t* flags, hipStream_t st) {
    if (prm->codec != FLC_TOPK) { set_error("flc_select_row_flags: TopK only"); return FLC_ERR_ARG; }
    if (n <= 0 || d <= 0) return FLC_OK;
    size_t need = 0;
    carve_sel(nullptr, prm->codec, n, d, prm->k, &need);
    if (ws_bytes < need) { set_error("flc_select_row_flags: workspace %zu < %zu", ws_bytes, need); return FLC_ERR_WORKSPACE; }
    const SelWs ws = carve_sel(const_cast<void*>(wsp), prm->codec, n, d, prm->k, nullptr);
    FLC_CHECK_HIP(hipMemcpyAsync(flags, ws.flags, (size_t)n * sizeof(uint32_t), hipMemcpyDeviceToDevice, st));
    return FLC_OK;
}

__global__ __launch_bounds__(256) void k_unpack_lists(const char* __restrict__ base, int64_t ld,
                                                      const char* const* __restrict__ ptrs, int64_t n, int64_t cap,
                                                      int64_t pcap, SelWs ws) {
    const int64_t row = blockIdx.y;
    const char* p = base ? base + row * ld : ptrs[row];
    const uint32_t cnt = (uint32_t)min<int64_t>(reinterpret_cast<const uint32_t*>(p)[1], min(cap, pcap));
    const uint32_t* pi = reinterpret_cast<const uint32_t*>(p + 16);
    const float* pv = reinterpret_cast<const float*>(p + 16 + ((4 * pcap + 15) & ~int64_t(15)));
    for (int64_t e = (int64_t)blockIdx.x * 256 + threadIdx.x; e < cnt; e += (int64_t)gridDim.x * 256) {
        ws.ent_idx[row * ws.cap + e] = pi[e];
        ws.ent_val[row * ws.cap + e] = pv[e];
    }
    if (blockIdx.x == 0 && threadIdx.x == 0) {
        ws.thr[row] = 0;
        ws.flags[row] = F_EXACT;
        ws.rowcnt[row * RCS] = cnt;
    }
}

__global__ __launch_bounds__(256) void k_unpack_tab(int64_t n, int64_t d, SelWs ws) {
    const int64_t row = blockIdx.y, C = nchunks(d);
    const int64_t c = (int64_t)blockIdx.x * 256 + threadIdx.x;
    if (c >= C) return;
    const uint32_t cnt = ws.rowcnt[row * RCS];
    const uint32_t* idx = ws.ent_idx + row * ws.cap;
    auto lb = [&](uint64_t key) {
        uint32_t lo = 0, hi = cnt;
        while (lo < hi) {
            const uint32_t mid = (lo + hi) >> 1;
            if ((uint64_t)idx[mid] < key) lo = mid + 1; else hi = mid;
        }
        return lo;
    };
    const uint32_t a = lb((uint64_t)c << CHUNK_SHIFT), b = lb((uint64_t)(c + 1) << CHUNK_SHIFT);
    ws.tab[c * n + row] = make_uint2(a, b - a);
}

size_t sel_unpack_workspace(const flc_codec_params* prm, int64_t n, int64_t d) {
    size_t b = 0;
    carve_sel(nullptr, FLC_RANDK, n, d, std::max<int64_t>(1, std::min(prm->k, d)), &b);
    return b;
}

int sel_unpack_reduce(const flc_codec_params* prm, const void* base, int64_t ld_bytes, const void* const* ptrs,
                      int64_t n, int64_t d, const float* w, float wt, float* out, void* wsp, size_t ws_bytes,
                      hipStream_t st) {
    const int64_t K = std::max<int64_t>(1, std::min(prm->k, d));
    if (ws_bytes < sel_unpack_workspace(prm, n, d)) { set_error("flc_unpack_reduce: workspace too small"); return FLC_ERR_WORKSPACE; }
    if (d >= (int64_t)0xFFFFFFFF) { set_error("D too large for 32-bit entry indices"); return FLC_ERR_ARG; }
    SelWs ws = carve_sel(wsp, FLC_RANDK, n, d, K, nullptr);
    const int64_t C = host_chunks(d);
    dim3 g1((unsigned)std::max<int64_t>(1, std::min<int64_t>((K + 255) / 256, 64)), (unsigned)n);
    hipLaunchKernelGGL(k_unpack_lists, g1, dim3(256), 0, st, (const char*)base, ld_bytes, (const char* const*)ptrs, n,
                       ws.cap, K, ws);
    FLC_CHECK_LAUNCH("k_unpack_lists");
    hipLaunchKernelGGL(k_unpack_tab, dim3((unsigned)((C + 255) / 256), (unsigned)n), dim3(256), 0, st, n, d, ws);
    FLC_CHECK_LAUNCH("k_unpack_tab");
    const int ab = grid_stride_blocks((C + 3) / 4, 4096);
    { ProfScope _ps("k_chunk_accum", st);
    hipLaunchKernelGGL((k_chunk_accum<false>), dim3(ab), dim3(256), 0, st, n, d, ws, w, wt, out); }
    FLC_CHECK_LAUNCH("k_chunk_accum");
    return FLC_OK;
}

__global__ __launch_bounds__(256) void k_randk_dense(const float* __restrict__ x, int64_t K, const int64_t* __restrict__ idx,
                                                     float scale, float* __restrict__ out) {
    for (int64_t t = (int64_t)blockIdx.x * 256 + threadIdx.x; t < K; t += (int64_t)gridDim.x * 256) {
        const int64_t j = idx[t];
        out[j] = scale * x[j];
    }
}

int randk_dense(const flc_codec_params* prm, const flc_pattern* pat, const float* x, int64_t d, float* out,
                void* wsp, size_t ws_bytes, hipStream_t st) {
    if (d == 0) return FLC_OK;
    if (prm->k < 1 || prm->k > d) { set_error("randk: K outside [1, D]"); return FLC_ERR_ARG; }
    FLC_CHECK_HIP(hipMemsetAsync(out, 0, (size_t)d * sizeof(float), st));
    if (pat && pat->d_randk_idx) {
        int g = (int)std::max<int64_t>(1, std::min<int64_t>((prm->k + 255) / 256, 1024));
        hipLaunchKernelGGL(k_randk_dense, dim3(g), dim3(256), 0, st, x, prm->k, pat->d_randk_idx, prm->randk_scale, out);
        FLC_CHECK_LAUNCH("k_randk_dense");
        return FLC_OK;
    }
    if (ws_bytes < randk_device_workspace(1, d)) { set_error("randk: workspace too small"); return FLC_ERR_WORKSPACE; }
    RkdWs ws = carve_rkd(wsp, 1, d, nullptr);
    if (int rc = randk_counts(prm, pat, 1, d, ws, st)) return rc;
    const int g = grid_stride_blocks((host_chunks(d) + 3) / 4, 4096);
    hipLaunchKernelGGL(k_randk_scatter_dev, dim3(g), dim3(256), 0, st, x, d, ws.cnt, ws.ckey, prm->randk_scale, out);
    FLC_CHECK_LAUNCH("k_randk_scatter_dev");
    return FLC_OK;
}

}
```

Measured before the change: 5910 GB/s.

## Store top-k candidate indices as 16-bit offsets within 65536-element items

When the workgroup filter and group-fold paths are used, candidate indices are written as 16-bit offsets relative to a 16-chunk item base instead of full 32-bit indices. The filter, exact-row fallback, tie resolution, negative-zero resolution and chunk accumulation all reconstruct the full index from the chunk's item base. This cuts the index write and read traffic in half and aims to lower HBM bytes in a bandwidth-bound pipeline. In exchange, tie handling must do an extra scan of the chunk table to recover item ids, and the scheme depends on NL=4 so that items line up with the 16-bit range.

```diff
diff --git a/flpytorch_amd/csrc/select.hip b/flpytorch_amd/csrc/select.hip
--- a/flpytorch_amd/csrc/select.hip
+++ b/flpytorch_amd/csrc/select.hip
@@ -111,7 +111,11 @@
     float* part;
     int64_t cap;
     uint32_t tie_hi;
+    uint32_t idx16;
 };
+
+__device__ inline uint16_t* ent_idx16(const SelWs& ws) { return reinterpret_cast<uint16_t*>(ws.ent_idx); }
+__device__ inline uint32_t item_base(int64_t c) { return (uint32_t)(c & ~(int64_t)15) << CHUNK_SHIFT; }
 
 __device__ __host__ inline uint32_t tie_pref(uint32_t ix, uint32_t hi) { return hi ? ix : ~ix; }
 __device__ __host__ inline uint32_t tie_all(uint32_t hi) { return hi ? 0u : 0xFFFFFFFFu; }
@@ -343,8 +347,9 @@
     return *p;
 #endif
 }
-template <int NT>
-__device__ void cand_select_row(int64_t row, int64_t K, SelWs ws, uint32_t* h, uint32_t* scratch) {
+template <int NT, bool IDX16 = false>
+__device__ void cand_select_row(int64_t row, int64_t K, SelWs ws, uint32_t* h, uint32_t* scratch,
+                                uint16_t* titem = nullptr, int64_t n = 0, int64_t C = 0) {
     {
         if (ws.flags[row]) return;
         const uint32_t cnt = ws.rowcnt[(row) * RCS];
@@ -411,13 +416,34 @@
                 const float qv[4] = {q.x, q.y, q.z, q.w};
 #pragma unroll
                 for (int u = 0; u < 4; ++u)
-                    if (mag_key(qv[u]) == thr) tix[atomicAdd(&scratch[0], 1u)] = idxs[i * 4 + u];
+                    if (mag_key(qv[u]) == thr) tix[atomicAdd(&scratch[0], 1u)] = IDX16 ? i * 4 + u : idxs[i * 4 + u];
             }
             for (uint32_t i = n4 * 4 + threadIdx.x; i < cnt; i += NT) {
-                if (mag_key(vals[i]) == thr) tix[atomicAdd(&scratch[0], 1u)] = idxs[i];
+                if (mag_key(vals[i]) == thr) tix[atomicAdd(&scratch[0], 1u)] = IDX16 ? i : idxs[i];
             }
             __syncthreads();
             const uint32_t m = scratch[0];
+            if (IDX16) {
+                constexpr int TB = 8;
+                for (int64_t c0 = threadIdx.x; c0 < C; c0 += (int64_t)NT * TB) {
+                    uint2 te[TB];
+#pragma unroll
+                    for (int u = 0; u < TB; ++u) {
+                        const int64_t c = c0 + (int64_t)u * NT;
+                        te[u] = c < C ? ws.tab[c * n + row] : make_uint2(0u, 0u);
+                    }
+                    for (uint32_t a = 0; a < m; ++a) {
+                        const uint32_t p = tix[a];
+#pragma unroll
+                        for (int u = 0; u < TB; ++u)
+                            if (p - te[u].x < te[u].y) titem[a] = (uint16_t)((c0 + (int64_t)u * NT) >> 4);
+                    }
+                }
+                __syncthreads();
+                const uint16_t* i16 = ent_idx16(ws) + row * ws.cap;
+                for (uint32_t a = threadIdx.x; a < m; a += NT) tix[a] = ((uint32_t)titem[a] << 16) | (uint32_t)i16[tix[a]];
+                __syncthreads();
+            }
             for (uint32_t a = threadIdx.x; a < m; a += NT) {
                 const uint32_t ia = tix[a];
                 uint32_t rank = 0;
@@ -792,8 +818,11 @@
 #ifndef FLC_TK_PROBE
 #define FLC_TK_PROBE 0
 #endif
-
-template <int POL = FLC_TK_STPOL>
+#ifndef FLC_TK_IDX16
+#define FLC_TK_IDX16 1
+#endif
+
+template <int POL = FLC_TK_STPOL, bool IDX = true>
 __device__ inline void tk_copy_out(const uint32_t* si, const uint32_t* sv, const SelWs& ws, int64_t n, int64_t row,
                                    uint32_t pos, uint32_t tot, bool fits, int lane, int64_t wslot) {
     int64_t at = row * ws.cap + pos;
@@ -809,13 +838,35 @@
         const uint4 a = reinterpret_cast<const uint4*>(si)[q];
         const uint4 b = reinterpret_cast<const uint4*>(sv)[q];
         const uint32_t off = q < nq ? q * 16u : 0x7FFFFFF0u;
-        __builtin_amdgcn_raw_buffer_store_b128(__builtin_bit_cast(u4v, a), di, off, 0, POL);
+        if (IDX) __builtin_amdgcn_raw_buffer_store_b128(__builtin_bit_cast(u4v, a), di, off, 0, POL);
         __builtin_amdgcn_raw_buffer_store_b128(__builtin_bit_cast(u4v, b), dv, off, 0, POL);
     }
     const uint32_t e = nq * 4u + (uint32_t)(lane & 3);
     const uint32_t off = lane < 3 ? e * 4u : 0x7FFFFFF0u;
-    __builtin_amdgcn_raw_buffer_store_b32(si[e], di, off, 0, POL);
+    if (IDX) __builtin_amdgcn_raw_buffer_store_b32(si[e], di, off, 0, POL);
     __builtin_amdgcn_raw_buffer_store_b32(sv[e], dv, off, 0, POL);
+}
+
+template <int POL>
+__device__ inline void tk_copy_out_idx16(const uint32_t* si, const SelWs& ws, int64_t row, uint32_t pos, uint32_t tot,
+                                         bool fits, int lane) {
+    static_assert(GCAP <= 512, "one 16-B store of 8 entries a lane covers a group");
+    const int64_t at = row * ws.cap + pos;
+    const uint32_t hd = (uint32_t)at & 1u;
+    const uint32_t nrec = (fits && FLC_TK_PROBE != 2) ? (hd + tot) * 2u : 0u;
+    const auto di = __builtin_amdgcn_make_buffer_rsrc(ent_idx16(ws) + (at - hd), (short)0, (int)nrec, 0x00020000);
+    typedef unsigned int u4v __attribute__((ext_vector_type(4)));
+    const uint32_t t = min(tot, (uint32_t)GCAP);
+    const uint32_t nb = t > hd ? (t - hd) >> 3 : 0u;
+    const uint32_t* s = si + hd + 8 * lane;
+    u4v p;
+#pragma unroll
+    for (int u = 0; u < 4; ++u) p[u] = (s[2 * u] & 0xFFFFu) | (s[2 * u + 1] << 16);
+    __builtin_amdgcn_raw_buffer_store_b128(p, di, (uint32_t)lane < nb ? hd * 4u + (uint32_t)lane * 16u : 0x7FFFFFF0u, 0, POL);
+    const bool head = lane == 7;
+    const uint32_t j = head ? 0u : hd + 8u * nb + (uint32_t)lane;
+    const bool on = head ? (hd != 0u && t != 0u) : (lane < 7 && j < t);
+    __builtin_amdgcn_raw_buffer_store_b16((unsigned short)(si[on ? j : 0u] & 0xFFFFu), di, on ? (hd + j) * 2u : 0x7FFFFFF0u, 0, POL);
 }
 
 template <int RING, int FGS, int LONE = 0>
@@ -990,11 +1041,12 @@
     asm volatile("ds_read_b32 %0, %1\n\ts_waitcnt lgkmcnt(0)" : "=&v"(v) : "v"(addr) : "memory");
     return __builtin_amdgcn_readfirstlane(v);
 }
-template <int RING, int NL>
+template <int RING, int NL, bool IDX16 = false>
 __global__ __launch_bounds__((NL + 1) * 64) __attribute__((amdgpu_waves_per_eu(FLC_TK_WG_WPE))) void k_topk_filter_fast_wg(RowSrc rows, int64_t n, int64_t r0, int64_t rn, int64_t rb, int64_t d,
                                                                         SelWs ws) {
     static_assert(16 % RING == 0, "ring must divide the 16 loads of a chunk");
     constexpr int FGS = 4;
+    static_assert(!IDX16 || FGS * NL == 16, "16-bit indices: an item is 16 chunks = 65 536 elements (item_base)");
     constexpr int SROW = GCAP + 64;
     __shared__ __attribute__((aligned(16))) uint32_t st[2][NL][2 * SROW];
     __shared__ __attribute__((aligned(16))) uint32_t hs[2][NL][4];
@@ -1068,9 +1120,12 @@
             }
             if (!(fits && allfit) && lane == 0) atomicOr(&ws.flags[row], F_OVERFLOW);
 #pragma unroll
-            for (int w = 0; w < NL; ++w)
-                tk_copy_out<FLC_TK_WG_STPOL>(st[b][w], st[b][w] + SROW, ws, n, row, base + pre[w], tot[w], fits && tot[w] <= GCAP, lane,
-                            (int64_t)blockIdx.x * NL + w);
+            for (int w = 0; w < NL; ++w) {
+                const bool gfit = fits && tot[w] <= GCAP;
+                tk_copy_out<FLC_TK_WG_STPOL, !IDX16 && FLC_TK_PROBE != 5>(st[b][w], st[b][w] + SROW, ws, n, row, base + pre[w], tot[w], gfit, lane,
+                                                                          (int64_t)blockIdx.x * NL + w);
+                if (IDX16 && FLC_TK_PROBE != 5) tk_copy_out_idx16<FLC_TK_WG_STPOL>(st[b][w], ws, row, base + pre[w], tot[w], gfit, lane);
+            }
             asm volatile("s_waitcnt lgkmcnt(0)\n\tds_write_b32 %0, %1" ::"v"(lds_addr(&fr[b])), "v"(k + 1) : "memory");
         }
         return;
@@ -1257,7 +1312,7 @@
     return before + inc - v;
 }
 
-template <bool VEC, int NT = EX_NT>
+template <bool VEC, int NT = EX_NT, bool IDX16 = false>
 __device__ void exact_row(RowSrc rows, int64_t n, int64_t row, int64_t d, int64_t K, SelWs ws, uint32_t* h,
                           uint32_t* scratch, uint32_t* wsum) {
     const int t = threadIdx.x;
@@ -1301,6 +1356,7 @@
         const uint32_t thr = prefix;
         const uint32_t tie_from = ws.tie_hi ? ties_tot - krem : 0u, tie_to = ws.tie_hi ? ties_tot : krem;
         uint32_t* oi = ws.ent_idx + row * ws.cap;
+        uint16_t* oi16 = ent_idx16(ws) + row * ws.cap;
         float* ov = ws.ent_val + row * ws.cap;
         static_assert(CHUNK % (NT * 4) == 0, "exact_row: NT * 4 must divide CHUNK");
         constexpr int SUBS = CHUNK / (NT * 4);
@@ -1342,7 +1398,12 @@
             uint32_t pos = base + ex_scan<NT>(na, wsum, atot);
 #pragma unroll
             for (int q = 0; q < 4; ++q)
-                if (adm[q]) { oi[pos] = (uint32_t)(j0 + q); ov[pos] = v[q]; ++pos; }
+                if (adm[q]) {
+                    if (IDX16) oi16[pos] = (uint16_t)((j0 + q) & 0xFFFF);
+                    else oi[pos] = (uint32_t)(j0 + q);
+                    ov[pos] = v[q];
+                    ++pos;
+                }
             base += atot;
             tie_run += etot;
             if (sb == SUBS - 1 && t == 0) ws.tab[c * n + row] = make_uint2(cbase, base - cbase);
@@ -1368,19 +1429,20 @@
     }
 }
 
-template <int NT, bool VEC>
+template <int NT, bool VEC, bool IDX16 = false>
 __global__ __launch_bounds__(NT) void k_cand_select_x(RowSrc rows, int64_t n, int64_t r0, int64_t rn, int64_t d, int64_t K,
                                                       SelWs ws) {
     __shared__ uint32_t h[HBINS];
     __shared__ uint32_t scratch[260];
     __shared__ uint32_t wsum[NT / 64];
     __shared__ uint32_t failed;
+    __shared__ uint16_t titem[IDX16 ? TIECAP : 2];
     for (int64_t row = r0 + blockIdx.x; row < r0 + rn; row += gridDim.x) {
-        cand_select_row<NT>(row, K, ws, h, scratch);
+        cand_select_row<NT, IDX16>(row, K, ws, h, scratch, titem, n, nchunks(d));
         __syncthreads();
         if (threadIdx.x == 0) failed = __atomic_load_n(&ws.flags[row], __ATOMIC_RELAXED) & (F_OVERFLOW | F_SHORT);
         __syncthreads();
-        if (failed) exact_row<VEC, NT>(rows, n, row, d, K, ws, h, scratch, wsum);
+        if (failed) exact_row<VEC, NT, IDX16>(rows, n, row, d, K, ws, h, scratch, wsum);
         __syncthreads();
     }
 }
@@ -1675,7 +1737,7 @@
 }
 
 
-template <int TS>
+template <int TS, bool IDX16 = false>
 __device__ void resolve_neg_zero(float* tl, uint32_t* rm, const SelWs& ws, int64_t c, int64_t n, uint32_t cbase,
                                  int64_t len, const float* w, int lane) {
     constexpr int NW = TS / 32;
@@ -1702,7 +1764,8 @@
         const RowMeta m = load_meta(ws, c, n, r, w);
         const uint32_t mode = m.mode, T = m.thr, cut = m.cut;
         for (uint32_t e = (uint32_t)lane; e < m.te.y; e += 64) {
-            const uint32_t ix = ws.ent_idx[r * ws.cap + m.te.x + e];
+            const uint32_t ix = IDX16 ? item_base(c) + (uint32_t)ent_idx16(ws)[r * ws.cap + m.te.x + e]
+                                      : ws.ent_idx[r * ws.cap + m.te.x + e];
             const uint32_t key = mag_key(ws.ent_val[r * ws.cap + m.te.x + e]);
             const uint32_t loc = ix - cbase;
             if (loc < (uint32_t)TS && (mode == 2u || key > T || (key == T && tie_pref(ix, ws.tie_hi) >= cut)))
@@ -1727,7 +1790,7 @@
     }
 }
 
-template <int TS>
+template <int TS, bool IDX16 = false>
 __device__ void resolve_neg_zero_g(float* tl, uint32_t* rm, const SelWs& ws, int64_t c, int64_t n, uint32_t cbase,
                                    int64_t len, const float* w, int lane) {
     constexpr int NW = TS / 32;
@@ -1759,7 +1822,8 @@
         const RowMeta m = load_meta(ws, c, n, r, w);
         const uint32_t mode = m.mode, T = m.thr, cut = m.cut;
         for (uint32_t e = (uint32_t)lane; e < m.te.y; e += 64) {
-            const uint32_t ix = ws.ent_idx[r * ws.cap + m.te.x + e];
+            const uint32_t ix = IDX16 ? item_base(c) + (uint32_t)ent_idx16(ws)[r * ws.cap + m.te.x + e]
+                                      : ws.ent_idx[r * ws.cap + m.te.x + e];
             const uint32_t key = mag_key(ws.ent_val[r * ws.cap + m.te.x + e]);
             const uint32_t loc = ix - cbase;
             if (loc < (uint32_t)TS && (mode == 2u || key > T || (key == T && tie_pref(ix, ws.tie_hi) >= cut)))
@@ -1785,7 +1849,7 @@
     }
 }
 
-template <bool ASSIGN, int TS, bool W, int WPB, int AP = AP>
+template <bool ASSIGN, int TS, bool W, int WPB, int AP = AP, bool IDX16 = false>
 __device__ __forceinline__ void chunk_accum_body(int64_t n, int64_t d, SelWs ws, const float* __restrict__ w, float wt,
                                                  float* __restrict__ out, int64_t r0, int64_t rend, int first, int last,
                                                  float (*tile)[TS], uint32_t (*zmask)[WPB == 1 ? 1 : TS / 32]) {
@@ -1799,6 +1863,8 @@
     for (int64_t t = (int64_t)blockIdx.x * WPB + wv; t < C * PARTS; t += (int64_t)gridDim.x * WPB) {
         const int64_t c = t / PARTS;
         const uint32_t cbase = (uint32_t)(c * CHUNK + (t % PARTS) * TS);
+        const uint32_t ibase = item_base(c);
+        const uint16_t* e16 = ent_idx16(ws);
         if (FLC_TILE_V4 && !ASSIGN && !first && (int64_t)cbase + TS <= d) {
             const float4* p4 = reinterpret_cast<const float4*>(ws.part + cbase);
 #pragma unroll
@@ -1819,12 +1885,15 @@
         float rv[AP][2];
         auto fetch = [&](const RowMeta& m, int q, int64_t row, int slot) {
             const uint32_t off = __builtin_amdgcn_readlane(m.te.x, q), cnt = __builtin_amdgcn_readlane(m.te.y, q);
-            const auto di = list_rsrc(ws.ent_idx + row * ws.cap + off, cnt);
+            const auto di = IDX16 ? __builtin_amdgcn_make_buffer_rsrc(const_cast<uint16_t*>(e16 + row * ws.cap + off), (short)0,
+                                                                      (int)(cnt * 2u), 0x00020000)
+                                  : list_rsrc(ws.ent_idx + row * ws.cap + off, cnt);
             const auto dv = list_rsrc(ws.ent_val + row * ws.cap + off, cnt);
 #pragma unroll
             for (int h = 0; h < 2; ++h) {
                 const uint32_t e = (uint32_t)lane + 64u * h;
-                const uint32_t x = __builtin_amdgcn_raw_buffer_load_b32(di, lane * 4, h * 256, 0);
+                const uint32_t x = IDX16 ? ibase + (uint32_t)__builtin_amdgcn_raw_buffer_load_b16(di, lane * 2, h * 128, 0)
+                                         : __builtin_amdgcn_raw_buffer_load_b32(di, lane * 4, h * 256, 0);
                 ri[slot][h] = e < cnt ? x : 0xFFFFFFFFu;
                 rv[slot][h] = __uint_as_float(__builtin_amdgcn_raw_buffer_load_b32(dv, lane * 4, h * 256, 0));
             }
@@ -1878,7 +1947,8 @@
                     fold(i_1, v_1, T, cut, mode, wi);
                     const int64_t row = i0 + q;
                     for (uint32_t e = 128u + lane; e < cnt; e += 64)
-                        fold(ws.ent_idx[row * ws.cap + off + e], ws.ent_val[row * ws.cap + off + e], T, cut, mode, wi);
+                        fold(IDX16 ? ibase + (uint32_t)e16[row * ws.cap + off + e] : ws.ent_idx[row * ws.cap + off + e],
+                             ws.ent_val[row * ws.cap + off + e], T, cut, mode, wi);
                     const RowMeta& m = (q + AP < 64) ? cur : nxt;
                     const int qq = (q + AP) & 63;
                     const uint32_t offn = __shfl(m.te.x, qq, WAVE), cntn = __shfl(m.te.y, qq, WAVE);
@@ -1888,7 +1958,8 @@
 #pragma unroll
                     for (int h = 0; h < 2; ++h) {
                         const uint32_t e = (uint32_t)lane + 64u * h;
-                        xi[h] = e < cntn ? ws.ent_idx[rown * ws.cap + offn + e] : 0xFFFFFFFFu;
+                        xi[h] = e >= cntn ? 0xFFFFFFFFu
+                                          : (IDX16 ? ibase + (uint32_t)e16[rown * ws.cap + offn + e] : ws.ent_idx[rown * ws.cap + offn + e]);
                         xv[h] = e < cntn ? ws.ent_val[rown * ws.cap + offn + e] : 0.f;
                     }
 #pragma unroll
@@ -1904,28 +1975,28 @@
             continue;
         }
         if (!ASSIGN) {
-            if (WPB == 1) resolve_neg_zero_g<TS>(tl, ws.zm + t * (TS / 32), ws, c, n, cbase, len, w, lane);
-            else resolve_neg_zero<TS>(tl, zmask[wv], ws, c, n, cbase, len, w, lane);
+            if (WPB == 1) resolve_neg_zero_g<TS, IDX16>(tl, ws.zm + t * (TS / 32), ws, c, n, cbase, len, w, lane);
+            else resolve_neg_zero<TS, IDX16>(tl, zmask[wv], ws, c, n, cbase, len, w, lane);
         }
         for (int64_t i = lane; i < len; i += 64) out[cbase + i] = ASSIGN ? tl[i] : tl[i] / wt;
     }
 }
 
-template <bool ASSIGN, int TS = CHUNK, bool W = true>
+template <bool ASSIGN, int TS = CHUNK, bool W = true, bool IDX16 = false>
 __global__ __launch_bounds__(256) void k_chunk_accum(int64_t n, int64_t d, SelWs ws, const float* __restrict__ w, float wt,
                                                      float* __restrict__ out, int64_t r0 = 0, int64_t rend = -1,
                                                      int first = 1, int last = 1) {
     __shared__ __attribute__((aligned(16))) float tile[4][TS];
     __shared__ uint32_t zmask[4][TS / 32];
-    chunk_accum_body<ASSIGN, TS, W, 4>(n, d, ws, w, wt, out, r0, rend, first, last, tile, zmask);
-}
-
-template <bool W>
+    chunk_accum_body<ASSIGN, TS, W, 4, AP, IDX16>(n, d, ws, w, wt, out, r0, rend, first, last, tile, zmask);
+}
+
+template <bool W, bool IDX16 = false>
 __global__ __launch_bounds__(64) void k_chunk_accum1(
         int64_t n, int64_t d, SelWs ws, const float* __restrict__ w, float wt, float* __restrict__ out, int64_t r0,
         int64_t rend, int first, int last) {
     extern __shared__ __attribute__((aligned(16))) float dyn_tile[];
-    chunk_accum_body<false, CHUNK, W, 1, FLC_CA_AP1>(n, d, ws, w, wt, out, r0, rend, first, last,
+    chunk_accum_body<false, CHUNK, W, 1, FLC_CA_AP1, IDX16>(n, d, ws, w, wt, out, r0, rend, first, last,
                                          reinterpret_cast<float (*)[CHUNK]>(dyn_tile), nullptr);
 }
 
@@ -3100,6 +3171,7 @@
     const int64_t C = std::max<int64_t>(host_chunks(d), 1), nn = std::max<int64_t>(n, 1);
     SelWs s;
     s.tie_hi = 0;
+    s.idx16 = 0;
     s.cap = sel_capacity(codec, d, K);
     s.tab = cv.take<uint2>((size_t)C * nn);
     s.ent_idx = cv.take<uint32_t>((size_t)nn * s.cap);
@@ -3218,6 +3290,20 @@
     return g;
 }
 
+static bool filter_wg(int shards, const float* zout) {
+    if (!(FLC_TK_WG != 0 && FLC_TK_PROBE != 1 && FLC_TK_PROBE != 3)) return false;
+    static const bool wg = [] { const char* e = tuning_env("FLC_FILTER_WG"); return !(e && atoi(e) == 0); }();
+    return wg && shards == 1 && !zout;
+}
+static int filter_group_for(int64_t n, int64_t d) { return (filter_group() == 2 || n * d < ((int64_t)64 << 20)) ? 2 : 4; }
+static bool idx16_on() {
+    static const bool v = [] {
+        const char* e = tuning_env("FLC_TK_IDX16");
+        return FLC_TK_IDX16 != 0 && FLC_TK_WG_NL == 4 && !(e && atoi(e) == 0);
+    }();
+    return v;
+}
+
 template <int FGS>
 static void launch_filter(RowSrc rows, int64_t n, int64_t r0, int64_t rn, int64_t d, SelWs ws, hipStream_t st,
                           int shards, float* zout = nullptr) {
@@ -3228,9 +3314,8 @@
         return e ? std::max<int64_t>(1, atoll(e)) : (int64_t)64;
     }();
     ProfScope _pv(FGS == 4 ? "k_topk_filter_g4" : "k_topk_filter_g2", st);
-    if constexpr (FGS == 4 && FLC_TK_WG != 0 && FLC_TK_PROBE != 1 && FLC_TK_PROBE != 3) {
-        static const bool wg = [] { const char* e = tuning_env("FLC_FILTER_WG"); return !(e && atoi(e) == 0); }();
-        if (wg && shards == 1 && !zout) {
+    if constexpr (FGS == 4) {
+        if (filter_wg(shards, zout)) {
             constexpr int NL = FLC_TK_WG_NL;
             const int64_t items = rn * ((nchunks(d) + 4 * NL - 1) / (4 * NL));
             const int gi = (int)std::max<int64_t>(1, std::min<int64_t>(items, 32768));
@@ -3238,8 +3323,12 @@
                 const char* e = tuning_env("FLC_TK_RB");
                 return e ? std::max<int64_t>(1, atoll(e)) : (int64_t)16;
             }();
-            hipLaunchKernelGGL((k_topk_filter_fast_wg<FLC_TK_WG_RING, NL>), dim3(gi), dim3((NL + 1) * 64), 0, st, rows, n, r0,
-                               rn, std::min(rbw, std::max<int64_t>(rn, 1)), d, ws);
+            if (ws.idx16)
+                hipLaunchKernelGGL((k_topk_filter_fast_wg<FLC_TK_WG_RING, NL, NL == 4>), dim3(gi), dim3((NL + 1) * 64), 0, st, rows, n, r0,
+                                   rn, std::min(rbw, std::max<int64_t>(rn, 1)), d, ws);
+            else
+                hipLaunchKernelGGL((k_topk_filter_fast_wg<FLC_TK_WG_RING, NL, false>), dim3(gi), dim3((NL + 1) * 64), 0, st, rows, n, r0,
+                                   rn, std::min(rbw, std::max<int64_t>(rn, 1)), d, ws);
             return;
         }
     }
@@ -3384,20 +3473,25 @@
                              bool first, bool last, bool exposed, hipStream_t st) {
     const int64_t C = host_chunks(d);
     ProfScope _ps("k_chunk_accum", st);
-    if (!exposed) {
-        const int ab = grid_stride_blocks(C, 16384);
-        if (w) hipLaunchKernelGGL((k_chunk_accum1<true>), dim3(ab), dim3(64), CHUNK * sizeof(float), st, n, d, ws, w, wt, out, r0, r1,
-                                  first ? 1 : 0, last ? 1 : 0);
-        else hipLaunchKernelGGL((k_chunk_accum1<false>), dim3(ab), dim3(64), CHUNK * sizeof(float), st, n, d, ws, w, wt, out, r0, r1,
-                                first ? 1 : 0, last ? 1 : 0);
-    } else {
-        constexpr int LTS = FLC_TK_LAST_TS;
-        const int ab = grid_stride_blocks((C * (CHUNK / LTS) + 3) / 4, 4096);
-        if (w) hipLaunchKernelGGL((k_chunk_accum<false, LTS, true>), dim3(ab), dim3(256), 0, st, n, d, ws, w, wt, out, r0, r1,
-                                  first ? 1 : 0, last ? 1 : 0);
-        else hipLaunchKernelGGL((k_chunk_accum<false, LTS, false>), dim3(ab), dim3(256), 0, st, n, d, ws, w, wt, out, r0, r1,
-                                first ? 1 : 0, last ? 1 : 0);
-    }
+    auto go = [&](auto i16) {
+        constexpr bool I16 = decltype(i16)::value;
+        if (!exposed) {
+            const int ab = grid_stride_blocks(C, 16384);
+            if (w) hipLaunchKernelGGL((k_chunk_accum1<true, I16>), dim3(ab), dim3(64), CHUNK * sizeof(float), st, n, d, ws, w, wt, out, r0, r1,
+                                      first ? 1 : 0, last ? 1 : 0);
+            else hipLaunchKernelGGL((k_chunk_accum1<false, I16>), dim3(ab), dim3(64), CHUNK * sizeof(float), st, n, d, ws, w, wt, out, r0, r1,
+                                    first ? 1 : 0, last ? 1 : 0);
+        } else {
+            constexpr int LTS = FLC_TK_LAST_TS;
+            const int ab = grid_stride_blocks((C * (CHUNK / LTS) + 3) / 4, 4096);
+            if (w) hipLaunchKernelGGL((k_chunk_accum<false, LTS, true, I16>), dim3(ab), dim3(256), 0, st, n, d, ws, w, wt, out, r0, r1,
+                                      first ? 1 : 0, last ? 1 : 0);
+            else hipLaunchKernelGGL((k_chunk_accum<false, LTS, false, I16>), dim3(ab), dim3(256), 0, st, n, d, ws, w, wt, out, r0, r1,
+                                    first ? 1 : 0, last ? 1 : 0);
+        }
+    };
+    if (ws.idx16) go(std::true_type{});
+    else go(std::false_type{});
     FLC_CHECK_LAUNCH("k_chunk_accum(group)");
     return FLC_OK;
 }
@@ -3551,6 +3645,8 @@
         if (!dense_k) {
             const int TG = few ? 1 : tk_tail_groups(prm, n);
             gfold = FLC_TK_GFOLD && !few && !assign && !dense_k;
+            const int fgs = filter_group_for(n, d);
+            ws.idx16 = (gfold && fgs == 4 && filter_wg(few ? CS_SH : 1, lone_assign ? out : nullptr) && idx16_on()) ? 1u : 0u;
             hipStream_t sside = st;
             TkCtx* cx = nullptr;
             std::unique_lock<std::mutex> lk;
@@ -3595,7 +3691,7 @@
                 if (split && g == 1) FLC_CHECK_HIP(hipStreamWaitEvent(st, cx->ev[TG + 2], 0));
                 { ProfScope _ps("k_topk_filter", st);
                 float* zout = lone_assign ? out : nullptr;
-                if (filter_group() == 2 || n * d < ((int64_t)64 << 20)) launch_filter<2>(rows, n, r0, rn, d, ws, st, few ? CS_SH : 1, zout);
+                if (fgs == 2) launch_filter<2>(rows, n, r0, rn, d, ws, st, few ? CS_SH : 1, zout);
                 else launch_filter<4>(rows, n, r0, rn, d, ws, st, few ? CS_SH : 1, zout); }
                 FLC_CHECK_LAUNCH("k_topk_filter");
                 if (TG > 1) {
@@ -3612,16 +3708,19 @@
                     const bool big = rn < 128 || g == TG - 1;
                     const int nt = big ? 1024 : FLC_TK_SIDE_NT;
                     const dim3 grid((unsigned)(big ? rn : grid_stride_blocks(rn, 8192)));
-                    if (big) {
-                        if (vec) hipLaunchKernelGGL((k_cand_select_x<1024, true>), grid, dim3(nt), 0, sside, rows, n, r0, rn, d, K, ws);
-                        else hipLaunchKernelGGL((k_cand_select_x<1024, false>), grid, dim3(nt), 0, sside, rows, n, r0, rn, d, K, ws);
-                    } else if (FLC_TK_SIDE_NT == 256) {
-                        if (vec) hipLaunchKernelGGL((k_cand_select_x<256, true>), grid, dim3(nt), 0, sside, rows, n, r0, rn, d, K, ws);
-                        else hipLaunchKernelGGL((k_cand_select_x<256, false>), grid, dim3(nt), 0, sside, rows, n, r0, rn, d, K, ws);
-                    } else {
-                        if (vec) hipLaunchKernelGGL((k_cand_select_x<512, true>), grid, dim3(nt), 0, sside, rows, n, r0, rn, d, K, ws);
-                        else hipLaunchKernelGGL((k_cand_select_x<512, false>), grid, dim3(nt), 0, sside, rows, n, r0, rn, d, K, ws);
-                    }
+                    auto go = [&](auto ntc, auto i16) {
+                        constexpr int NTC = decltype(ntc)::value;
+                        constexpr bool I16 = decltype(i16)::value;
+                        if (vec) hipLaunchKernelGGL((k_cand_select_x<NTC, true, I16>), grid, dim3(nt), 0, sside, rows, n, r0, rn, d, K, ws);
+                        else hipLaunchKernelGGL((k_cand_select_x<NTC, false, I16>), grid, dim3(nt), 0, sside, rows, n, r0, rn, d, K, ws);
+                    };
+                    auto gof = [&](auto ntc) {
+                        if (ws.idx16) go(ntc, std::true_type{});
+                        else go(ntc, std::false_type{});
+                    };
+                    if (big) gof(std::integral_constant<int, 1024>{});
+                    else if (FLC_TK_SIDE_NT == 256) gof(std::integral_constant<int, 256>{});
+                    else gof(std::integral_constant<int, 512>{});
                 } else if (rn < 128 || (TG > 1 && g == TG - 1))
                     hipLaunchKernelGGL(k_cand_select<1024>, dim3((unsigned)rn), dim3(1024), 0, sside, r0, rn, K, ws);
                 else if (FLC_TK_SIDE_NT == 256)
```

New measurement: 5980 GB/s (median of 6 runs). 1.2% higher.
